# gpustack/llama-box

Measured on AMD Instinct MI355X. Metric: decode tokens/sec (batch-1) + prefill tok/s, Llama-3-8B Q4_K_M, higher is better.
Workload: dtype q4_K/q6_K weights x q8_K activations (int8 dot, f32 accumulate)

## Files before the change

### include/ggml_mi355x.h

```cpp
#ifndef GGML_MI355X_H
#define GGML_MI355X_H
#include "ggml_abi.h"

#ifdef __cplusplus
extern "C" {
#endif

#define GGML_MI355X_NAME "MI355X"
#define GGML_MI355X_MAX_DEVICES 16

ggml_backend_reg_t ggml_backend_init(void);

int ggml_backend_score(void);

ggml_backend_reg_t ggml_backend_mi355x_reg(void);


typedef void (*ggml_backend_mi355x_split_rows_t)(int64_t nrows, const float * tensor_split, int n_dev, int64_t * row0);

typedef int (*ggml_backend_mi355x_tp_init_t)(ggml_backend_t backend, int rank, int world_size, const void * unique_id, size_t unique_id_size);
typedef int (*ggml_backend_mi355x_tp_p2p_export_t)(ggml_backend_t backend, int rank, int world_size, void * handle_out, size_t handle_size);
typedef int (*ggml_backend_mi355x_tp_p2p_attach_t)(ggml_backend_t backend, const void * handles, size_t handles_size);
typedef int (*ggml_backend_mi355x_tp_all_reduce_t)(ggml_backend_t backend, float * device_ptr, size_t n);
typedef int (*ggml_backend_mi355x_tp_get_unique_id_t)(void * unique_id_out, size_t unique_id_size);
typedef ggml_backend_buffer_type_t (*ggml_backend_mi355x_tp_rowpar_buffer_type_t)(int device);

typedef int (*ggml_backend_mi355x_graph_key_probe_t)(const struct ggml_cgraph * a, const struct ggml_cgraph * b, int64_t * n_words);

typedef int64_t (*ggml_backend_mi355x_decode_copy_read_t)(ggml_backend_t backend, const struct ggml_tensor * t, void * out, size_t size);

typedef int (*ggml_backend_mi355x_set_option_t)(ggml_backend_t backend, const char * key, const char * value);
typedef int64_t (*ggml_backend_mi355x_get_stat_t)(ggml_backend_t backend, const char * key);
typedef int (*ggml_backend_mi355x_timing_report_t)(ggml_backend_t backend, char * buf, size_t size, int reset);

#ifdef __cplusplus
}
#endif
#endif
```

### llama_box_amd/csrc/backend.cpp

```cpp
#include <dlfcn.h>

#include <algorithm>
#include <chrono>
#include <mutex>
#include <thread>

#include "common.h"
#include "kernels.h"

namespace mi355x {

int log_level() {
    static int lvl = [] {
        const char * e = getenv("GGML_MI355X_LOG");
        return e ? atoi(e) : 0;
    }();
    return lvl;
}

struct device_ctx {
    int device = 0;
    std::string name, description;
    ggml_backend_buffer_type buft{};
    ggml_backend_buffer_type buft_rowpar{};
    ggml_backend_buffer_type buft_host{};
};

struct reg_ctx {
    std::vector<ggml_backend_device *> devices;
};

static ggml_backend_reg g_reg;
static reg_ctx g_reg_ctx;
static std::once_flag g_reg_once;
static ggml_guid g_guid = {0x4d, 0x49, 0x33, 0x35, 0x35, 0x58, 0x2d, 0x67, 0x67, 0x6d, 0x6c, 0x2d, 0x62, 0x6b, 0x6e, 0x64};

static device_ctx * dctx(ggml_backend_dev_t dev) { return (device_ctx *) dev->context; }
int logical_device_count() { return (int) g_reg_ctx.devices.size(); }
int logical_device_ordinal(int i) { return dctx(g_reg_ctx.devices[(size_t) i])->device; }
ggml_backend_dev_t logical_device(int i) { return g_reg_ctx.devices[(size_t) i]; }

typedef ggml_backend_buffer_t (*buffer_init_fn)(ggml_backend_buffer_type_t, struct ggml_backend_buffer_i, void *, size_t);

ggml_backend_buffer_t make_backend_buffer(ggml_backend_buffer_type_t buft, const ggml_backend_buffer_i & iface, void * context, size_t size);
static ggml_backend_buffer_t make_buffer(ggml_backend_buffer_type_t buft, const ggml_backend_buffer_i & iface, void * context, size_t size) {
    return make_backend_buffer(buft, iface, context, size);
}
ggml_backend_buffer_t make_backend_buffer(ggml_backend_buffer_type_t buft, const ggml_backend_buffer_i & iface, void * context, size_t size) {
    static buffer_init_fn host_fn = (buffer_init_fn) dlsym(RTLD_DEFAULT, "ggml_backend_buffer_init");
    if (host_fn) return host_fn(buft, iface, context, size);
    return new ggml_backend_buffer{iface, buft, context, size, GGML_BACKEND_BUFFER_USAGE_ANY};
}

static void uploader_drain(int device);
static std::atomic<uint64_t> g_decode_epoch{1};
uint64_t decode_copy_epoch() { return g_decode_epoch.load(std::memory_order_acquire); }
static void decode_copy_drop(buffer_ctx * c, size_t off, size_t n) {
    if (c->shadow == nullptr) return;
    std::lock_guard<std::mutex> lk(c->sh_mtx);
    if (c->sh_valid.empty()) return;
    bool any = false;
    for (auto it = c->sh_valid.begin(); it != c->sh_valid.end();) {
        if (it->first < off + n && off < it->first + it->second) { it = c->sh_valid.erase(it); any = true; }
        else ++it;
    }
    if (any) g_decode_epoch.fetch_add(1, std::memory_order_acq_rel);
}
static void decode_copy_drop(ggml_backend_buffer_t b, const ggml_tensor * t, size_t offset, size_t size) {
    buffer_ctx * c = (buffer_ctx *) b->context;
    if (c->shadow != nullptr && t->data != nullptr) decode_copy_drop(c, (size_t) ((const char *) t->data - (const char *) c->base) + offset, size);
}
static const uint8_t * second_copy(backend_ctx * c, const ggml_tensor * w, const bool q80_panels) {
    if (!c->opt.decode_copy || w == nullptr || w->view_src != nullptr || w->data == nullptr || w->ne[2] != 1 || w->ne[3] != 1) return nullptr;
    ggml_backend_buffer_t b = w->buffer;
    if (b == nullptr || !buffer_is_ours(b) || b->usage != GGML_BACKEND_BUFFER_USAGE_WEIGHTS || buffer_is_split(b) || buffer_is_rowpar(b)) return nullptr;
    if (q80_panels ? !repack_q80_supported(w->type, w->ne[0], w->ne[1], (int64_t) w->nb[1]) : !repack_supported(w->type, w->ne[0], (int64_t) w->nb[1])) return nullptr;
    buffer_ctx * bc = (buffer_ctx *) b->context;
    if (bc->device != c->device || bc->shadow_failed) return nullptr;
    const size_t off = (size_t) ((const char *) w->data - (const char *) bc->base), bytes = (size_t) w->nb[1] * (size_t) w->ne[1];
    if (off + bytes > bc->size) return nullptr;
    std::lock_guard<std::mutex> lk(bc->sh_mtx);
    auto it = bc->sh_valid.find(off);
    if (it != bc->sh_valid.end() && it->second == bytes) return (const uint8_t *) bc->shadow + off;
    if (c->capturing) return nullptr;
    if (bc->shadow == nullptr) {
        size_t free_b = 0, total_b = 0;
        if (hipMemGetInfo(&free_b, &total_b) != hipSuccess || free_b < bc->size + ((size_t) std::max(0, c->opt.decode_copy_headroom_gib) << 30) || hipMalloc(&bc->shadow, bc->size) != hipSuccess) {
            (void) hipGetLastError();
            bc->shadow = nullptr;
            bc->shadow_failed = true;
            MI_INFO("decode copy: no room for a second copy of a %.1f GiB weights buffer on device %d — the mat-vec kernels read the block layout", (double) bc->size / (1 << 30), bc->device);
            return nullptr;
        }
    }
    if (q80_panels) launch_repack_q80_panels(c->stream, w->data, (char *) bc->shadow + off, w->ne[0], w->ne[1], (int64_t) w->nb[1]);
    else launch_repack_planes(c->stream, w->type, w->data, (char *) bc->shadow + off, w->ne[0], (int64_t) w->nb[1], 0, w->ne[1]);
    if (hipStreamSynchronize(c->stream) != hipSuccess) { (void) hipGetLastError(); return nullptr; }
    bc->sh_valid[off] = bytes;
    c->st.decode_copy_tensors++;
    c->st.decode_copy_bytes += (int64_t) bytes;
    return (const uint8_t *) bc->shadow + off;
}
const uint8_t * decode_copy(backend_ctx * c, const ggml_tensor * w) { return second_copy(c, w, false); }
const uint8_t * q80_panel_copy(backend_ctx * c, const ggml_tensor * w) { return second_copy(c, w, true); }
static void buf_free(ggml_backend_buffer_t b) {
    buffer_ctx * c = (buffer_ctx *) b->context;
    if (ip_any()) ip_host_buffer_freed(b);
    HIP_SOFT(hipSetDevice(c->device));
    uploader_drain(c->device);
    if (c->shadow) {
        HIP_SOFT(hipDeviceSynchronize());
        HIP_NOTE(hipFree(c->shadow));
        g_decode_epoch.fetch_add(1, std::memory_order_acq_rel);
    }
    HIP_NOTE(hipFree(c->base));
    delete c;
}
static void * buf_get_base(ggml_backend_buffer_t b) { return ((buffer_ctx *) b->context)->base; }
static enum ggml_status buf_init_tensor(ggml_backend_buffer_t, ggml_tensor *) { return GGML_STATUS_SUCCESS; }
static void buf_memset_tensor(ggml_backend_buffer_t b, ggml_tensor * t, uint8_t value, size_t offset, size_t size) {
    buffer_ctx * c = (buffer_ctx *) b->context;
    if (ip_any()) ip_host_access(b, true);
    HIP_SOFT(hipSetDevice(c->device));
    decode_copy_drop(b, t, offset, size);
    uploader_drain(c->device);
    HIP_SOFT(hipMemset((char *) t->data + offset, value, size));
    HIP_SOFT(hipDeviceSynchronize());
}
struct uploader {
    std::atomic<int> device{-1};
    std::atomic<bool> failed{false};
    hipStream_t stream = nullptr;
    static constexpr int NSLOT = 3;
    char * slot[NSLOT] = {nullptr, nullptr, nullptr};
    hipEvent_t ev[NSLOT] = {nullptr, nullptr, nullptr};
    bool busy[NSLOT] = {false, false, false};
    size_t slot_bytes = 0;
    int next = 0;
    hipEvent_t last = nullptr;
    std::atomic<bool> in_flight{false};
    int n_threads = 1;
    std::mutex mtx;
    uint64_t bytes = 0;
    double seconds = 0;
};
static uploader g_uploaders[GGML_MI355X_MAX_DEVICES];
static std::atomic<int> g_staged_upload{env_int("GGML_MI355X_STAGED_UPLOAD", 0)};

static void par_memcpy(char * dst, const char * src, size_t n, int n_threads) {
    if (n_threads <= 1 || n < ((size_t) 4 << 20)) { memcpy(dst, src, n); return; }
    std::vector<std::thread> th;
    const size_t per = ((n / (size_t) n_threads) + 4095) & ~(size_t) 4095;
    for (int t = 1; t < n_threads; ++t) {
        const size_t o = (size_t) t * per;
        if (o >= n) break;
        th.emplace_back([=] { memcpy(dst + o, src + o, std::min(per, n - o)); });
    }
    memcpy(dst, src, std::min(per, n));
    for (auto & x : th) x.join();
}
static uploader * uploader_for(int device) {
    if (device < 0 || device >= GGML_MI355X_MAX_DEVICES) return nullptr;
    uploader * u = &g_uploaders[device];
    if (u->failed) return nullptr;
    if (u->device == device) return u;
    if (!g_staged_upload.load(std::memory_order_relaxed)) return nullptr;
    std::lock_guard<std::mutex> init_lock(u->mtx);
    if (u->failed) return nullptr;
    if (u->device == device) return u;
    const char * e_mb = getenv("GGML_MI355X_UPLOAD_SLOT_MIB");
    const char * e_th = getenv("GGML_MI355X_UPLOAD_THREADS");
    u->slot_bytes = (size_t) std::max(1, e_mb ? atoi(e_mb) : 32) << 20;
    u->n_threads = std::max(1, std::min(16, e_th ? atoi(e_th) : 4));
    bool ok = hipStreamCreateWithFlags(&u->stream, hipStreamNonBlocking) == hipSuccess && hipEventCreateWithFlags(&u->last, hipEventDisableTiming) == hipSuccess;
    for (int i = 0; i < uploader::NSLOT && ok; ++i)
        ok = hipHostMalloc((void **) &u->slot[i], u->slot_bytes, hipHostMallocDefault) == hipSuccess && hipEventCreateWithFlags(&u->ev[i], hipEventDisableTiming) == hipSuccess;
    if (!ok) {
        (void) hipGetLastError();
        MI_INFO("staged uploads unavailable on device %d (pinned allocation failed): set_tensor falls back to hipMemcpy", device);
        for (int i = 0; i < uploader::NSLOT; ++i) {
            if (u->slot[i]) (void) hipHostFree(u->slot[i]);
            if (u->ev[i]) (void) hipEventDestroy(u->ev[i]);
            u->slot[i] = nullptr;
            u->ev[i] = nullptr;
        }
        if (u->last) (void) hipEventDestroy(u->last);
        if (u->stream) (void) hipStreamDestroy(u->stream);
        u->failed = true;
        return nullptr;
    }
    u->device = device;
    return u;
}
static void uploader_drain(int device) {
    if (device < 0 || device >= GGML_MI355X_MAX_DEVICES) return;
    uploader * u = &g_uploaders[device];
    if (u->device != device) return;
    std::lock_guard<std::mutex> lock(u->mtx);
    if (!u->in_flight) return;
    HIP_SOFT(hipStreamSynchronize(u->stream));
    for (bool & b : u->busy) b = false;
    u->in_flight = false;
}
static void uploader_join(int device, hipStream_t s) {
    if (device < 0 || device >= GGML_MI355X_MAX_DEVICES) return;
    uploader * u = &g_uploaders[device];
    if (u->device != device || !u->in_flight) return;
    std::lock_guard<std::mutex> lock(u->mtx);
    if (!u->in_flight) return;
    if (hipEventQuery(u->last) == hipSuccess) {
        for (bool & b : u->busy) b = false;
        u->in_flight = false;
        return;
    }
    (void) hipGetLastError();
    HIP_SOFT(hipStreamWaitEvent(s, u->last, 0));
}
static bool staged_upload(int device, char * dst, const char * src, size_t size) {
    uploader * u = uploader_for(device);
    if (!u) return false;
    std::lock_guard<std::mutex> lock(u->mtx);
    const auto t0 = std::chrono::steady_clock::now();
    for (size_t o = 0; o < size; o += u->slot_bytes) {
        const size_t n = std::min(u->slot_bytes, size - o);
        const int k = u->next;
        u->next = (k + 1) % uploader::NSLOT;
        if (u->busy[k] && hipEventSynchronize(u->ev[k]) != hipSuccess) return false;
        par_memcpy(u->slot[k], src + o, n, u->n_threads);
        if (hipMemcpyAsync(dst + o, u->slot[k], n, hipMemcpyHostToDevice, u->stream) != hipSuccess || hipEventRecord(u->ev[k], u->stream) != hipSuccess) {
            (void) hipGetLastError();
            (void) hipStreamSynchronize(u->stream);
            u->failed = true;
            return false;
        }
        u->busy[k] = true;
        u->in_flight = true;
    }
    if (hipEventRecord(u->last, u->stream) != hipSuccess) { (void) hipGetLastError(); (void) hipStreamSynchronize(u->stream); }
    u->bytes += size;
    u->seconds += std::chrono::duration<double>(std::chrono::steady_clock::now() - t0).count();
    return true;
}

static std::atomic<int> g_hip_failed{0};
void note_hip_failure() { g_hip_failed.store(1, std::memory_order_relaxed); }
bool hip_failed() { return g_hip_failed.load(std::memory_order_relaxed) != 0; }
void clear_hip_failure() { g_hip_failed.store(0, std::memory_order_relaxed); }

namespace {
struct mask_entry { const void * dev = nullptr; mask_stats st; uint64_t stamp = 0; };
std::mutex g_mask_mtx;
mask_entry g_masks[8];
std::atomic<uint64_t> g_mask_clock{0};
}
void note_mask_upload(const ggml_tensor * t, const void * host, size_t offset, size_t size) {
    auto forget = [&]() {
        std::lock_guard<std::mutex> lock(g_mask_mtx);
        for (mask_entry & e : g_masks)
            if (e.dev == t->data) { e.dev = nullptr; e.stamp = 0; }
    };
    bool named = false;
    for (const char * p = t->name; *p && !named; ++p) named = (p[0] == 'm' || p[0] == 'M') && (p[1] == 'a' || p[1] == 'A') && (p[2] == 's' || p[2] == 'S') && (p[3] == 'k' || p[3] == 'K');
    const bool whole = offset == 0 && t->ne[2] == 1 && t->ne[3] == 1 && (t->type == GGML_TYPE_F16 || t->type == GGML_TYPE_F32) && t->nb[1] > 0 && size % (size_t) t->nb[1] == 0 &&
                       size <= (size_t) t->nb[1] * (size_t) t->ne[1] && t->nb[0] == (t->type == GGML_TYPE_F16 ? 2u : 4u);
    if (!named || !whole || t->ne[1] < 2 || t->ne[1] > 256 || size > ((size_t) 16 << 20)) { forget(); return; }
    const int64_t n = t->ne[0], rows = (int64_t) (size / (size_t) t->nb[1]);
    if (rows < 2) { forget(); return; }
    mask_stats st;
    int64_t total = 0;
    const int64_t dense_at = rows * n / 4 + 1;
    for (int64_t r = 0; r < rows; ++r) {
        if (total >= dense_at) {
            st.rows = (int) rows;
            st.max_visible = std::max(st.max_visible, (int) n);
            total = rows * n;
            break;
        }
        int64_t vis = 0;
        if (t->type == GGML_TYPE_F16) {
            const uint16_t * m = (const uint16_t *) ((const char *) host + r * t->nb[1]);
            for (int64_t i = 0; i < n; ++i) vis += m[i] != 0xFC00u;
        } else {
            const uint32_t * m = (const uint32_t *) ((const char *) host + r * t->nb[1]);
            for (int64_t i = 0; i < n; ++i) vis += m[i] != 0xFF800000u;
        }
        total += vis;
        st.rows += vis > 0;
        st.max_visible = std::max(st.max_visible, (int) vis);
    }
    st.density = st.rows > 0 ? (float) ((double) total / ((double) st.rows * (double) n)) : 0.0f;
    std::lock_guard<std::mutex> lock(g_mask_mtx);
    mask_entry * slot = &g_masks[0];
    for (mask_entry & e : g_masks) {
        if (e.dev == t->data) { slot = &e; break; }
        if (e.stamp < slot->stamp) slot = &e;
    }
    slot->dev = t->data;
    slot->st = st;
    slot->stamp = ++g_mask_clock;
}
void forget_mask_stats(const void * dev_ptr, size_t nbytes) {
    if (g_mask_clock.load(std::memory_order_relaxed) == 0 || !dev_ptr) return;
    std::lock_guard<std::mutex> lock(g_mask_mtx);
    for (mask_entry & e : g_masks)
        if (e.stamp != 0 && (const char *) e.dev >= (const char *) dev_ptr && (const char *) e.dev < (const char *) dev_ptr + nbytes) { e.dev = nullptr; e.stamp = 0; }
}
void copy_mask_stats(const ggml_tensor * src, const ggml_tensor * dst, size_t nbytes) {
    if (g_mask_clock.load(std::memory_order_relaxed) == 0 || !src->data || !dst->data) return;
    std::lock_guard<std::mutex> lock(g_mask_mtx);
    const mask_entry * from = nullptr;
    for (const mask_entry & e : g_masks)
        if (e.stamp != 0 && e.dev == src->data) from = &e;
    for (mask_entry & e : g_masks)
        if (e.stamp != 0 && (const char *) e.dev >= (const char *) dst->data && (const char *) e.dev < (const char *) dst->data + nbytes) { e.dev = nullptr; e.stamp = 0; }
    if (!from || src->view_src || dst->view_src || src->type != dst->type || src->ne[0] != dst->ne[0] || src->ne[1] != dst->ne[1] || src->ne[2] != dst->ne[2] || src->ne[3] != dst->ne[3] ||
        src->nb[1] != dst->nb[1])
        return;
    const mask_stats st = from->st;
    mask_entry * slot = &g_masks[0];
    for (mask_entry & e : g_masks) {
        if (e.dev == dst->data) { slot = &e; break; }
        if (e.stamp < slot->stamp) slot = &e;
    }
    if (slot == from) return;
    slot->dev = dst->data;
    slot->st = st;
    slot->stamp = ++g_mask_clock;
}
bool lookup_mask_stats(const void * dev_ptr, mask_stats * out) {
    std::lock_guard<std::mutex> lock(g_mask_mtx);
    for (const mask_entry & e : g_masks)
        if (e.dev == dev_ptr && e.stamp != 0) { *out = e.st; return true; }
    return false;
}
int mask_sparse_hint(const void * dev_ptr) {
    mask_stats st;
    return dev_ptr != nullptr && lookup_mask_stats(dev_ptr, &st) && st.rows > 0 && st.density <= 0.25f ? 1 : 0;
}

static void buf_set_tensor(ggml_backend_buffer_t b, ggml_tensor * t, const void * data, size_t offset, size_t size) {
    buffer_ctx * c = (buffer_ctx *) b->context;
    if (ip_any()) ip_host_access(b, true);
    HIP_SOFT(hipSetDevice(c->device));
    note_mask_upload(t, data, offset, size);
    decode_copy_drop(b, t, offset, size);
    if (size > ((size_t) 1 << 20) && staged_upload(c->device, (char *) t->data + offset, (const char *) data, size)) return;
    uploader_drain(c->device);
    HIP_SOFT(hipMemcpy((char *) t->data + offset, data, size, hipMemcpyHostToDevice));
}
static void buf_get_tensor(ggml_backend_buffer_t b, const ggml_tensor * t, void * data, size_t offset, size_t size) {
    buffer_ctx * c = (buffer_ctx *) b->context;
    if (ip_any()) ip_host_access(b, false);
    HIP_SOFT(hipSetDevice(c->device));
    uploader_drain(c->device);
    HIP_SOFT(hipMemcpy(data, (const char *) t->data + offset, size, hipMemcpyDeviceToHost));
}
static bool buf_cpy_tensor(ggml_backend_buffer_t b, const ggml_tensor * src, ggml_tensor * dst) {
    ggml_backend_buffer_t sb = src->view_src ? src->view_src->buffer : src->buffer;
    if (!buffer_is_ours(sb)) return false;
    buffer_ctx * sc = (buffer_ctx *) sb->context;
    buffer_ctx * dc = (buffer_ctx *) b->context;
    const size_t n = ggml_abi_nbytes(src);
    copy_mask_stats(src, dst, n);
    decode_copy_drop(b, dst, 0, n);
    if (ip_any()) { ip_host_access(sb, false); ip_host_access(b, true); }
    uploader_drain(sc->device);
    if (dc->device != sc->device) uploader_drain(dc->device);
    if (sc->device == dc->device) {
        HIP_SOFT(hipSetDevice(dc->device));
        HIP_SOFT(hipMemcpy(dst->data, src->data, n, hipMemcpyDeviceToDevice));
    } else {
        HIP_SOFT(hipMemcpyPeer(dst->data, dc->device, src->data, sc->device, n));
    }
    HIP_SOFT(hipDeviceSynchronize());
    return true;
}
static void buf_clear(ggml_backend_buffer_t b, uint8_t value) {
    buffer_ctx * c = (buffer_ctx *) b->context;
    if (ip_any()) ip_host_access(b, true);
    HIP_SOFT(hipSetDevice(c->device));
    decode_copy_drop(c, 0, c->size);
    uploader_drain(c->device);
    HIP_SOFT(hipMemset(c->base, value, c->size));
    HIP_SOFT(hipDeviceSynchronize());
}
static const ggml_backend_buffer_i k_buffer_iface = {buf_free, buf_get_base, buf_init_tensor, buf_memset_tensor, buf_set_tensor,
                                                     buf_get_tensor, buf_cpy_tensor, buf_clear, nullptr};

bool buffer_is_ours(ggml_backend_buffer_t b) { return b != nullptr && b->iface.free_buffer == buf_free; }
void make_internal_buffer(ggml_backend_buffer * out, buffer_ctx * bc, int device_ordinal, bool rowpar) {
    bc->device = device_ordinal;
    bc->base = nullptr;
    bc->size = 0;
    bc->rowpar = rowpar;
    *out = ggml_backend_buffer{k_buffer_iface, nullptr, bc, 0, GGML_BACKEND_BUFFER_USAGE_COMPUTE};
}
bool buffer_is_rowpar(ggml_backend_buffer_t b) { return buffer_is_ours(b) && ((buffer_ctx *) b->context)->rowpar; }

struct buft_ctx {
    int device;
    bool rowpar;
    std::string name;
};
static const char * buft_get_name(ggml_backend_buffer_type_t buft) { return ((buft_ctx *) buft->context)->name.c_str(); }
static ggml_backend_buffer_t buft_alloc(ggml_backend_buffer_type_t buft, size_t size) {
    buft_ctx * bc = (buft_ctx *) buft->context;
    HIP_SOFT(hipSetDevice(bc->device));
    void * p = nullptr;
    hipError_t err = hipMalloc(&p, size + 256);
    if (err != hipSuccess) {
        (void) hipGetLastError();
        MI_ERR("allocating %.2f MiB on device %d: hipMalloc failed: %s", size / 1024.0 / 1024.0, bc->device, hipGetErrorString(err));
        return nullptr;
    }
    buffer_ctx * c = new buffer_ctx{bc->device, p, size, bc->rowpar};
    return make_buffer(buft, k_buffer_iface, c, size);
}
static size_t buft_alignment(ggml_backend_buffer_type_t) { return 256; }
static size_t buft_max_size(ggml_backend_buffer_type_t buft) {
    buft_ctx * bc = (buft_ctx *) buft->context;
    hipDeviceProp_t prop{};
    if (hipGetDeviceProperties(&prop, bc->device) != hipSuccess) {
        (void) hipGetLastError();
        return SIZE_MAX;
    }
    return prop.totalGlobalMem;
}
static size_t buft_alloc_size(ggml_backend_buffer_type_t, const ggml_tensor * t) {
    return (ggml_abi_nbytes(t) + 15) / 16 * 16;
}
static bool buft_is_host(ggml_backend_buffer_type_t) { return false; }
static const ggml_backend_buffer_type_i k_buft_iface = {buft_get_name, buft_alloc, buft_alignment, buft_max_size, buft_alloc_size, buft_is_host};

static std::mutex g_pinned_mtx;
static std::vector<std::pair<const char *, size_t>> g_pinned;
static bool is_pinned_range(const void * p, size_t n) {
    std::lock_guard<std::mutex> lock(g_pinned_mtx);
    for (const auto & r : g_pinned)
        if ((const char *) p >= r.first && (const char *) p + n <= r.first + r.second) return true;
    return false;
}
static void hbuf_free(ggml_backend_buffer_t b) {
    {
        std::lock_guard<std::mutex> lock(g_pinned_mtx);
        for (size_t i = 0; i < g_pinned.size(); ++i)
            if (g_pinned[i].first == (const char *) b->context) { g_pinned.erase(g_pinned.begin() + (long) i); break; }
    }
    HIP_NOTE(hipHostFree(b->context));
}
static void * hbuf_base(ggml_backend_buffer_t b) { return b->context; }
static void hbuf_memset(ggml_backend_buffer_t, ggml_tensor * t, uint8_t v, size_t off, size_t sz) { memset((char *) t->data + off, v, sz); }
static void hbuf_set(ggml_backend_buffer_t, ggml_tensor * t, const void * d, size_t off, size_t sz) { memcpy((char *) t->data + off, d, sz); }
static void hbuf_get(ggml_backend_buffer_t, const ggml_tensor * t, void * d, size_t off, size_t sz) { memcpy(d, (const char *) t->data + off, sz); }
static void hbuf_clear(ggml_backend_buffer_t b, uint8_t v) { memset(b->context, v, b->size); }
static const char * hbuft_name(ggml_backend_buffer_type_t) { return GGML_MI355X_NAME "_Host"; }
static ggml_backend_buffer_t hbuft_alloc(ggml_backend_buffer_type_t buft, size_t size) {
    void * p = nullptr;
    hipError_t err = hipHostMalloc(&p, size > 0 ? size : 1, hipHostMallocPortable | hipHostMallocMapped);
    if (err != hipSuccess) {
        (void) hipGetLastError();
        return nullptr;
    }
    ggml_backend_buffer_i iface = {hbuf_free, hbuf_base, nullptr, hbuf_memset, hbuf_set, hbuf_get, nullptr, hbuf_clear, nullptr};
    {
        std::lock_guard<std::mutex> lock(g_pinned_mtx);
        g_pinned.emplace_back((const char *) p, size > 0 ? size : 1);
    }
    return make_buffer(buft, iface, p, size);
}
static size_t hbuft_alignment(ggml_backend_buffer_type_t) { return 64; }
static bool hbuft_is_host(ggml_backend_buffer_type_t) { return true; }

static const char * be_get_name(ggml_backend_t be) { return ((backend_ctx *) be->context)->name.c_str(); }
static void be_free(ggml_backend_t be) {
    backend_ctx * c = (backend_ctx *) be->context;
    HIP_SOFT(hipSetDevice(c->device));
    HIP_SOFT(hipStreamSynchronize(c->stream));
    free_graph_cache(c);
    ip_free(c);
    tp_free(c);
    free_split_helpers(c);
    if (c->ws) HIP_NOTE(hipFree(c->ws));
    if (c->up_ring) HIP_NOTE(hipHostFree(c->up_ring));
    if (c->fa_lists) HIP_NOTE(hipFree(c->fa_lists));
    if (c->rope_tab) HIP_NOTE(hipFree(c->rope_tab));
    if (c->act_tab) HIP_NOTE(hipFree(c->act_tab));
    if (c->fa_arrive) HIP_NOTE(hipFree(c->fa_arrive));
    if (c->ss_buf) HIP_NOTE(hipFree(c->ss_buf));
    HIP_SOFT(hipStreamDestroy(c->stream));
    delete c;
    delete be;
}
void flush_uploads(backend_ctx * c) {
    if (c->up_pending.n == 0) return;
    launch_upload_multi(c->stream, c->up_pending);
    c->up_pending.n = 0;
}
static void be_set_tensor_async(ggml_backend_t be, ggml_tensor * t, const void * data, size_t offset, size_t size) {
    backend_ctx * c = (backend_ctx *) be->context;
    if (ip_any()) ip_host_access(t->view_src ? t->view_src->buffer : t->buffer, true);
    HIP_SOFT(hipSetDevice(c->device));
    note_mask_upload(t, data, offset, size);
    {
        ggml_backend_buffer_t tb = t->view_src ? t->view_src->buffer : t->buffer;
        if (tb && buffer_is_ours(tb) && ((buffer_ctx *) tb->context)->shadow) decode_copy_drop(tb, t, offset, size);
    }
    constexpr size_t SMALL = 64 * 1024, RING = 4u << 20;
    if (size > 0 && size <= SMALL && c->opt.small_uploads) {
        if (!c->up_ring) {
            if (hipHostMalloc((void **) &c->up_ring, RING, hipHostMallocDefault) == hipSuccess) c->up_cap = RING;
            else { (void) hipGetLastError(); c->up_ring = nullptr; c->opt.small_uploads = false; }
        }
        if (c->up_ring) {
            size_t at = (c->up_head + 255) & ~(size_t) 255;
            if (at + size > c->up_cap) {
                flush_uploads(c);
                HIP_SOFT(hipStreamSynchronize(c->stream));
                at = 0;
            }
            memcpy(c->up_ring + at, data, size);
            c->up_head = at + size;
            if (c->up_pending.n == 8) flush_uploads(c);
            c->up_pending.seg[c->up_pending.n++] = {(char *) t->data + offset, c->up_ring + at, size};
            return;
        }
    }
    flush_uploads(c);
    uploader_join(c->device, c->stream);
    HIP_SOFT(hipMemcpyAsync((char *) t->data + offset, data, size, hipMemcpyHostToDevice, c->stream));
}
static void be_get_tensor_async(ggml_backend_t be, const ggml_tensor * t, void * data, size_t offset, size_t size) {
    backend_ctx * c = (backend_ctx *) be->context;
    if (ip_any()) ip_host_access(t->view_src ? t->view_src->buffer : t->buffer, false);
    HIP_SOFT(hipSetDevice(c->device));
    flush_uploads(c);
    uploader_join(c->device, c->stream);
    if (c->opt.small_downloads && size > 0 && size <= ((size_t) 8 << 20) && is_pinned_range(data, size)) {
        launch_upload_small(c->stream, data, (const char *) t->data + offset, size);
        c->st.kernel_downloads++;
        return;
    }
    HIP_SOFT(hipMemcpyAsync(data, (const char *) t->data + offset, size, hipMemcpyDeviceToHost, c->stream));
}
static bool be_is_ours(ggml_backend_t be);
static bool be_cpy_tensor_async(ggml_backend_t be_src, ggml_backend_t be_dst, const ggml_tensor * src, ggml_tensor * dst) {
    if (!be_is_ours(be_src) || !be_is_ours(be_dst)) return false;
    ggml_backend_buffer_t sb = src->view_src ? src->view_src->buffer : src->buffer;
    ggml_backend_buffer_t db = dst->view_src ? dst->view_src->buffer : dst->buffer;
    if (!buffer_is_ours(sb) || !buffer_is_ours(db)) return false;
    backend_ctx * cs = (backend_ctx *) be_src->context;
    backend_ctx * cd = (backend_ctx *) be_dst->context;
    flush_uploads(cs);
    if (cd != cs) flush_uploads(cd);
    const size_t n = ggml_abi_nbytes(src);
    copy_mask_stats(src, dst, n);
    if (((buffer_ctx *) db->context)->shadow) decode_copy_drop(db, dst, 0, n);
    if (ip_any()) { ip_host_access(sb, false); ip_host_access(db, true); }
    uploader_join(cs->device, cs->stream);
    if (cd->device != cs->device) uploader_drain(cd->device);
    if (cs->device == cd->device) {
        HIP_SOFT(hipSetDevice(cs->device));
        HIP_SOFT(hipMemcpyAsync(dst->data, src->data, n, hipMemcpyDeviceToDevice, cs->stream));
    } else {
        HIP_SOFT(hipSetDevice(cs->device));
        HIP_SOFT(hipMemcpyPeerAsync(dst->data, cd->device, src->data, cs->device, n, cs->stream));
    }
    if (be_src != be_dst) {
        hipEvent_t ev;
        HIP_NOTE(hipEventCreateWithFlags(&ev, hipEventDisableTiming));
        HIP_SOFT(hipEventRecord(ev, cs->stream));
        HIP_SOFT(hipSetDevice(cd->device));
        HIP_SOFT(hipStreamWaitEvent(cd->stream, ev, 0));
        HIP_NOTE(hipEventDestroy(ev));
    }
    return true;
}
static void be_synchronize(ggml_backend_t be) {
    backend_ctx * c = (backend_ctx *) be->context;
    HIP_SOFT(hipSetDevice(c->device));
    flush_uploads(c);
    uploader_drain(c->device);
    HIP_SOFT(hipStreamSynchronize(c->stream));
}
static enum ggml_status be_graph_compute(ggml_backend_t be, ggml_cgraph * g) {
    backend_ctx * c = (backend_ctx *) be->context;
    if (hipSetDevice(c->device) != hipSuccess) return GGML_STATUS_FAILED;
    flush_uploads(c);
    uploader_join(c->device, c->stream);
    return graph_compute(c, g);
}
static void be_event_record(ggml_backend_t be, ggml_backend_event_t ev) {
    backend_ctx * c = (backend_ctx *) be->context;
    flush_uploads(c);
    HIP_SOFT(hipEventRecord((hipEvent_t) ev->context, c->stream));
}
static void be_event_wait(ggml_backend_t be, ggml_backend_event_t ev) {
    backend_ctx * c = (backend_ctx *) be->context;
    flush_uploads(c);
    HIP_SOFT(hipStreamWaitEvent(c->stream, (hipEvent_t) ev->context, 0));
}
static const ggml_backend_i k_backend_iface = {
    be_get_name, be_free, be_set_tensor_async, be_get_tensor_async, be_cpy_tensor_async, be_synchronize,
     nullptr,  nullptr,  nullptr,  nullptr,
    be_graph_compute, be_event_record, be_event_wait,
#if GGML_ABI_HAS_GRAPH_OPTIMIZE
    nullptr,
#endif
};
static bool be_is_ours(ggml_backend_t be) { return be != nullptr && be->iface.get_name == be_get_name; }
static ggml_backend_t dev_init_backend(ggml_backend_dev_t dev, const char *);
ggml_backend_t internal_backend(int logical) {
    if (logical < 0 || logical >= logical_device_count()) return nullptr;
    return dev_init_backend(logical_device(logical), nullptr);
}

static const char * dev_get_name(ggml_backend_dev_t dev) { return dctx(dev)->name.c_str(); }
static const char * dev_get_description(ggml_backend_dev_t dev) { return dctx(dev)->description.c_str(); }
static void dev_get_memory(ggml_backend_dev_t dev, size_t * free, size_t * total) {
    *free = 0;
    *total = 0;
    HIP_NOTE(hipSetDevice(dctx(dev)->device));
    HIP_NOTE(hipMemGetInfo(free, total));
}
static enum ggml_backend_dev_type dev_get_type(ggml_backend_dev_t) { return GGML_BACKEND_DEVICE_TYPE_GPU; }
static void dev_get_props(ggml_backend_dev_t dev, ggml_backend_dev_props * props) {
    props->name = dev_get_name(dev);
    props->description = dev_get_description(dev);
    props->type = GGML_BACKEND_DEVICE_TYPE_GPU;
    dev_get_memory(dev, &props->memory_free, &props->memory_total);
    props->caps = { true,  true,  false,  true};
}
static ggml_backend_t dev_init_backend(ggml_backend_dev_t dev, const char *) {
    device_ctx * d = dctx(dev);
    if (hipSetDevice(d->device) != hipSuccess) { (void) hipGetLastError(); MI_ERR("init_backend: device %d cannot be made current", d->device); return nullptr; }
    backend_ctx * c = new backend_ctx();
    c->device = d->device;
    c->name = d->name;
    if (hipStreamCreateWithFlags(&c->stream, hipStreamNonBlocking) != hipSuccess) {
        (void) hipGetLastError();
        MI_ERR("init_backend: no stream on device %d", d->device);
        delete c;
        return nullptr;
    }
    {
        static const bool preload = env_flag("GGML_MI355X_PRELOAD", true);
        static std::mutex pre_mtx;
        static bool preloaded[64] = {false};
        std::lock_guard<std::mutex> lk(pre_mtx);
        if (preload && d->device >= 0 && d->device < 64 && !preloaded[d->device]) {
            preload_kernel_files(c->stream);
            if (hipStreamSynchronize(c->stream) != hipSuccess) { (void) hipGetLastError(); MI_ERR("init_backend: kernel preload failed on device %d", d->device); }
            preloaded[d->device] = true;
        }
    }
    c->fa_lists_bytes = (size_t) 8 << 20;
    if (hipMalloc((void **) &c->fa_lists, c->fa_lists_bytes) != hipSuccess) { (void) hipGetLastError(); c->fa_lists = nullptr; c->fa_lists_bytes = 0; }
    if (hipMalloc((void **) &c->rope_tab, backend_ctx::rope_tab_floats * sizeof(float)) != hipSuccess) { (void) hipGetLastError(); c->rope_tab = nullptr; }
    if (hipMalloc((void **) &c->fa_arrive, backend_ctx::fa_arrive_slots * sizeof(unsigned)) != hipSuccess || hipMemset(c->fa_arrive, 0, backend_ctx::fa_arrive_slots * sizeof(unsigned)) != hipSuccess) {
        (void) hipGetLastError();
        c->fa_arrive = nullptr;
    }
    options_from_env(c->opt);
    c->ssm_fuse = env_flag("GGML_MI355X_SSM_FUSE", true);
    if (hipMalloc((void **) &c->ss_buf, 256 * sizeof(double)) != hipSuccess) {
        (void) hipGetLastError();
        c->ss_buf = nullptr;
    }
    return new ggml_backend{&g_guid, k_backend_iface, dev, c};
}
static ggml_backend_buffer_type_t dev_get_buffer_type(ggml_backend_dev_t dev) { return &dctx(dev)->buft; }
static ggml_backend_buffer_type_t dev_get_host_buffer_type(ggml_backend_dev_t dev) { return &dctx(dev)->buft_host; }
static bool dev_supports_op(ggml_backend_dev_t, const ggml_tensor * op) { return supports_op(op); }
static bool dev_supports_buft(ggml_backend_dev_t dev, ggml_backend_buffer_type_t buft) {
    if (buft_is_split(buft)) return logical_device(split_buft_main_device(buft)) == dev;
    if (buft->iface.get_name != buft_get_name) return false;
    return ((buft_ctx *) buft->context)->device == dctx(dev)->device;
}
static bool dev_offload_op(ggml_backend_dev_t, const ggml_tensor * op) {
    const int64_t batch = op->op == GGML_OP_MUL_MAT ? op->ne[1] : 0;
    return batch >= 32;
}
static ggml_backend_event_t dev_event_new(ggml_backend_dev_t dev) {
    HIP_SOFT(hipSetDevice(dctx(dev)->device));
    hipEvent_t ev;
    if (hipEventCreateWithFlags(&ev, hipEventDisableTiming) != hipSuccess) {
        (void) hipGetLastError();
        return nullptr;
    }
    return new ggml_backend_event{dev, ev};
}
static void dev_event_free(ggml_backend_dev_t, ggml_backend_event_t ev) {
    HIP_NOTE(hipEventDestroy((hipEvent_t) ev->context));
    delete ev;
}
static void dev_event_synchronize(ggml_backend_dev_t, ggml_backend_event_t ev) { HIP_SOFT(hipEventSynchronize((hipEvent_t) ev->context)); }
static const ggml_backend_device_i k_device_iface = {
    dev_get_name, dev_get_description, dev_get_memory, dev_get_type, dev_get_props, dev_init_backend, dev_get_buffer_type,
    dev_get_host_buffer_type,  nullptr, dev_supports_op, dev_supports_buft, dev_offload_op,
    dev_event_new, dev_event_free, dev_event_synchronize,
};

static ggml_backend_feature g_features[] = {{"ARCH", "gfx950"}, {"WAVE", "64"}, {"GRAPHS", "1"}, {"RCCL_TP", "1"}, {nullptr, nullptr}};
static ggml_backend_feature * get_features(ggml_backend_reg_t) { return g_features; }

static int api_tp_init(ggml_backend_t be, int rank, int world, const void * uid, size_t n) {
    if (!be_is_ours(be)) return -1;
    return tp_init((backend_ctx *) be->context, rank, world, uid, n);
}
static int api_tp_get_unique_id(void * out, size_t n) { return tp_get_unique_id(out, n); }
static int api_tp_p2p_export(ggml_backend_t be, int rank, int world, void * handle_out, size_t n) {
    if (!be_is_ours(be)) return -1;
    return tp_p2p_export((backend_ctx *) be->context, rank, world, handle_out, n);
}
static int api_tp_all_reduce(ggml_backend_t be, float * device_ptr, size_t n) {
    if (!be_is_ours(be)) return -1;
    backend_ctx * c = (backend_ctx *) be->context;
    if (!tp_active(c)) return -2;
    HIP_TRY(hipSetDevice(c->device), -3);
    return tp_all_reduce(c, device_ptr, n) ? 0 : -4;
}
static int api_tp_p2p_attach(ggml_backend_t be, const void * handles, size_t n) {
    if (!be_is_ours(be)) return -1;
    return tp_p2p_attach((backend_ctx *) be->context, handles, n);
}
static ggml_backend_buffer_type_t api_split_buffer_type(int main_device, const float * tensor_split) { return split_buffer_type(main_device, tensor_split); }
static void api_split_rows(int64_t nrows, const float * tensor_split, int n_dev, int64_t * row0) { split_rows(nrows, tensor_split, n_dev, nrows % 256 == 0 ? 256 : 64, row0); }
static ggml_backend_buffer_type_t api_tp_rowpar_buft(int device) {
    if (device < 0 || device >= (int) g_reg_ctx.devices.size()) return nullptr;
    return &dctx(g_reg_ctx.devices[device])->buft_rowpar;
}
static int api_graph_key_probe(const ggml_cgraph * a, const ggml_cgraph * b, int64_t * n_words) {
    std::vector<uint64_t> key;
    graph_key_build(a, key);
    if (n_words) *n_words = (int64_t) key.size();
    return graph_key_equals(b, key) ? 1 : 0;
}
static int64_t api_decode_copy_read(ggml_backend_t be, const ggml_tensor * t, void * out, size_t size) {
    if (!be_is_ours(be) || t == nullptr) return -1;
    backend_ctx * c = (backend_ctx *) be->context;
    if (hipSetDevice(c->device) != hipSuccess) return -1;
    uploader_join(c->device, c->stream);
    const uint8_t * p = t->type == GGML_TYPE_Q8_0 ? q80_panel_copy(c, t) : decode_copy(c, t);
    if (!p) return 0;
    const size_t bytes = (size_t) t->nb[1] * (size_t) t->ne[1];
    if (out == nullptr || size < bytes) return (int64_t) bytes;
    if (hipStreamSynchronize(c->stream) != hipSuccess || hipMemcpy(out, p, bytes, hipMemcpyDeviceToHost) != hipSuccess) { (void) hipGetLastError(); return -1; }
    return (int64_t) bytes;
}
static int api_set_option(ggml_backend_t be, const char * key, const char * value) {
    if (!be_is_ours(be)) return -1;
    backend_ctx * c = (backend_ctx *) be->context;
    const std::string k = key;
    const int v = atoi(value);
    if (!options_set(c->opt, key, v)) {
        if (k == "tp_p2p") { if (!tp_p2p_enable(c, v != 0)) return -2; }
        else if (k == "tp_p2p_reset") { if (!tp_p2p_reset(c)) return -2; }
        else if (k == "clear_failure") { if (v) clear_hip_failure(); }
        else if (k == "staged_upload") g_staged_upload.store(v != 0);
        else if (k == "ssm_fuse") c->ssm_fuse = v != 0;
        else return -1;
    }
    HIP_SOFT(hipStreamSynchronize(c->stream));
    free_graph_cache(c);
    return 0;
}
static int64_t api_get_stat(ggml_backend_t be, const char * key) {
    if (!be_is_ours(be)) return -1;
    backend_ctx * c = (backend_ctx *) be->context;
    const std::string k = key;
    if (const int64_t * p = stats_find(c->st, key)) return *p;
    if (k == "graph_cache_size") return (int64_t) c->graphs.size();
    if (k == "p2p_timeouts") return tp_p2p_timeouts(c);
    if (k.rfind("ip_", 0) == 0) return ip_stat(c, key);
    if (k == "staged_upload_bytes") return (int64_t) g_uploaders[c->device].bytes;
    if (k == "staged_upload_us") return (int64_t) (g_uploaders[c->device].seconds * 1e6);
    return -1;
}
static int api_timing_report(ggml_backend_t be, char * buf, size_t size, int reset) {
    if (!be_is_ours(be) || !buf || size == 0) return -1;
    backend_ctx * c = (backend_ctx *) be->context;
    HIP_SOFT(hipStreamSynchronize(c->stream));
    for (auto & pe : c->pending_events) {
        float ms = 0;
        HIP_NOTE(hipEventElapsedTime(&ms, pe.second.first, pe.second.second));
        c->timing[pe.first].total_ms += ms;
        c->timing[pe.first].count += 1;
        HIP_NOTE(hipEventDestroy(pe.second.first));
        HIP_NOTE(hipEventDestroy(pe.second.second));
    }
    c->pending_events.clear();
    std::string out;
    for (auto & kv : c->timing) {
        if (kv.first.rfind("bytes:", 0) == 0) continue;
        auto itb = c->timing.find("bytes:" + kv.first);
        char line[256];
        snprintf(line, sizeof(line), "%s %lld %.6f %.0f\n", kv.first.c_str(), (long long) kv.second.count, kv.second.total_ms,
                 itb == c->timing.end() ? 0.0 : itb->second.total_ms);
        out += line;
    }
    snprintf(buf, size, "%s", out.c_str());
    if (reset) c->timing.clear();
    return 0;
}

static const char * reg_get_name(ggml_backend_reg_t) { return GGML_MI355X_NAME; }
static size_t reg_get_device_count(ggml_backend_reg_t) { return g_reg_ctx.devices.size(); }
static ggml_backend_dev_t reg_get_device(ggml_backend_reg_t, size_t i) { return i < g_reg_ctx.devices.size() ? g_reg_ctx.devices[i] : nullptr; }
static void * reg_get_proc_address(ggml_backend_reg_t, const char * name) {
    const std::string n = name;
    if (n == "ggml_backend_get_features") return (void *) get_features;
    if (n == "ggml_backend_mi355x_tp_init") return (void *) api_tp_init;
    if (n == "ggml_backend_mi355x_tp_get_unique_id") return (void *) api_tp_get_unique_id;
    if (n == "ggml_backend_mi355x_tp_p2p_export") return (void *) api_tp_p2p_export;
    if (n == "ggml_backend_mi355x_tp_p2p_attach") return (void *) api_tp_p2p_attach;
    if (n == "ggml_backend_mi355x_tp_all_reduce") return (void *) api_tp_all_reduce;
    if (n == "ggml_backend_mi355x_tp_rowpar_buffer_type") return (void *) api_tp_rowpar_buft;
    if (n == "ggml_backend_mi355x_set_option") return (void *) api_set_option;
    if (n == "ggml_backend_mi355x_decode_copy_read") return (void *) api_decode_copy_read;
    if (n == "ggml_backend_mi355x_get_stat") return (void *) api_get_stat;
    if (n == "ggml_backend_mi355x_timing_report") return (void *) api_timing_report;
    if (n == "ggml_backend_split_buffer_type") return (void *) api_split_buffer_type;
    if (n == "ggml_backend_mi355x_split_rows") return (void *) api_split_rows;
    if (n == "ggml_backend_mi355x_graph_key_probe") return (void *) api_graph_key_probe;
    return nullptr;
}
static const ggml_backend_reg_i k_reg_iface = {reg_get_name, reg_get_device_count, reg_get_device, reg_get_proc_address};

static int count_gfx950() {
    int n = 0;
    if (hipGetDeviceCount(&n) != hipSuccess) {
        (void) hipGetLastError();
        return 0;
    }
    int ok = 0;
    for (int i = 0; i < n; ++i) {
        hipDeviceProp_t prop;
        if (hipGetDeviceProperties(&prop, i) == hipSuccess && strncmp(prop.gcnArchName, "gfx950", 6) == 0) ok++;
    }
    return ok;
}

static void init_reg() {
    int n = 0;
    if (hipGetDeviceCount(&n) != hipSuccess) {
        (void) hipGetLastError();
        n = 0;
    }
    const int fake = std::max(1, env_int("GGML_MI355X_FAKE_DEVICES", 1));
    for (int ii = 0; ii < n * fake && (int) g_reg_ctx.devices.size() < GGML_MI355X_MAX_DEVICES; ++ii) {
        const int i = ii / fake;
        hipDeviceProp_t prop;
        if (hipGetDeviceProperties(&prop, i) != hipSuccess) continue;
        if (strncmp(prop.gcnArchName, "gfx950", 6) != 0) {
            MI_INFO("skipping HIP device %d (%s): not gfx950", i, prop.gcnArchName);
            continue;
        }
        device_ctx * d = new device_ctx();
        d->device = i;
        d->name = std::string(GGML_MI355X_NAME) + std::to_string(g_reg_ctx.devices.size());
        d->description = prop.name;
        ggml_backend_device * dev = new ggml_backend_device{k_device_iface, &g_reg, d};
        d->buft = {k_buft_iface, dev, new buft_ctx{i, false, d->name}};
        d->buft_rowpar = {k_buft_iface, dev, new buft_ctx{i, true, d->name + "_RowPar"}};
        d->buft_host = {{hbuft_name, hbuft_alloc, hbuft_alignment, nullptr, nullptr, hbuft_is_host}, dev, nullptr};
        g_reg_ctx.devices.push_back(dev);
    }
    g_reg = {GGML_BACKEND_API_VERSION, k_reg_iface, &g_reg_ctx};
}

static bool op_numbering_matches_host() {
    typedef const char * (*op_name_fn)(int);
    op_name_fn host_name = (op_name_fn) dlsym(RTLD_DEFAULT, "ggml_op_name");
    if (!host_name) {
        MI_INFO("ggml_op_name is not resolvable in this process: operator numbering of include/ggml_abi.h not verified against the host");
        return true;
    }
    static const struct { int op; const char * name; } k_expect[] = {
        {GGML_OP_NONE, "NONE"}, {GGML_OP_DUP, "DUP"}, {GGML_OP_ADD, "ADD"}, {GGML_OP_SUB, "SUB"}, {GGML_OP_MUL, "MUL"}, {GGML_OP_DIV, "DIV"},
        {GGML_OP_ARGMAX, "ARGMAX"}, {GGML_OP_NORM, "NORM"}, {GGML_OP_RMS_NORM, "RMS_NORM"}, {GGML_OP_MUL_MAT, "MUL_MAT"}, {GGML_OP_MUL_MAT_ID, "MUL_MAT_ID"}, {GGML_OP_SCALE, "SCALE"},
        {GGML_OP_CPY, "CPY"}, {GGML_OP_CONT, "CONT"}, {GGML_OP_RESHAPE, "RESHAPE"}, {GGML_OP_VIEW, "VIEW"}, {GGML_OP_PERMUTE, "PERMUTE"},
        {GGML_OP_TRANSPOSE, "TRANSPOSE"}, {GGML_OP_GET_ROWS, "GET_ROWS"}, {GGML_OP_SET_ROWS, "SET_ROWS"}, {GGML_OP_SOFT_MAX, "SOFT_MAX"},
        {GGML_OP_ROPE, "ROPE"}, {GGML_OP_FLASH_ATTN_EXT, "FLASH_ATTN_EXT"}, {GGML_OP_UNARY, "UNARY"}, {GGML_OP_GLU, "GLU"},
    };
    bool ok = true;
    for (const auto & e : k_expect) {
        const char * got = host_name(e.op);
        if (!got || strcmp(got, e.name) != 0) {
            MI_ERR("operator numbering mismatch: this library was built with %s = %d, the host calls op %d \"%s\" — rebuild against the host's ggml.h (tools/abi_dump.c prints both tables)",
                   e.name, e.op, e.op, got ? got : "(null)");
            ok = false;
        }
    }
    return ok;
}

}

extern "C" {

__attribute__((visibility("default"))) ggml_backend_reg_t ggml_backend_mi355x_reg(void) {
    std::call_once(mi355x::g_reg_once, mi355x::init_reg);
    return &mi355x::g_reg;
}

__attribute__((visibility("default"))) ggml_backend_reg_t ggml_backend_init(void) {
    ggml_backend_reg_t reg = ggml_backend_mi355x_reg();
    if (mi355x::g_reg_ctx.devices.empty()) {
        MI_ERR("no gfx950 (MI355X) device visible: backend not registered");
        return nullptr;
    }
    static const bool ops_ok = mi355x::op_numbering_matches_host();
    if (!ops_ok) return nullptr;
    return reg;
}

__attribute__((visibility("default"))) int ggml_backend_score(void) { return mi355x::count_gfx950() > 0 ? 100 : 0; }
}
```

### llama_box_amd/csrc/common.h

```cpp
#pragma once
#include <hip/hip_runtime.h>
#include <hip/hip_ext.h>

#include <cstdint>
#include <cstdio>
#include <cstdlib>
#include <cstring>
#include <atomic>
#include <map>
#include <mutex>
#include <string>
#include <unordered_map>
#include <vector>

#include "../../include/ggml_mi355x.h"
#include "options.h"

#define MI_LOG(level, ...)                                    \
    do {                                                      \
        if ((level) <= mi355x::log_level()) {                 \
            fprintf(stderr, "ggml-mi355x: " __VA_ARGS__);     \
            fprintf(stderr, "\n");                            \
        }                                                     \
    } while (0)
#define MI_ERR(...) MI_LOG(0, __VA_ARGS__)
#define MI_INFO(...) MI_LOG(1, __VA_ARGS__)
#define MI_DBG(...) MI_LOG(2, __VA_ARGS__)

#define HIP_CHECK(expr)                                                                                         \
    do {                                                                                                        \
        hipError_t err_ = (expr);                                                                               \
        if (err_ != hipSuccess) {                                                                               \
            fprintf(stderr, "ggml-mi355x: HIP error %d (%s) at %s:%d: %s\n", (int) err_, hipGetErrorString(err_), __FILE__, __LINE__, #expr); \
            abort();                                                                                            \
        }                                                                                                       \
    } while (0)

#define HIP_SOFT(expr)                                                                                          \
    do {                                                                                                        \
        hipError_t err_ = (expr);                                                                               \
        if (err_ != hipSuccess) {                                                                               \
            (void) hipGetLastError();                                                                           \
            fprintf(stderr, "ggml-mi355x: HIP error %d (%s) at %s:%d: %s — graph_compute will report failure from here on\n", (int) err_, \
                    hipGetErrorString(err_), __FILE__, __LINE__, #expr);                                        \
            mi355x::note_hip_failure();                                                                         \
        }                                                                                                       \
    } while (0)

#define HIP_NOTE(expr)                                                                                          \
    do {                                                                                                        \
        hipError_t err_ = (expr);                                                                               \
        if (err_ != hipSuccess) {                                                                               \
            (void) hipGetLastError();                                                                           \
            fprintf(stderr, "ggml-mi355x: HIP error %d (%s) at %s:%d: %s (ignored: no tensor data involved)\n", (int) err_, hipGetErrorString(err_), __FILE__, __LINE__, #expr); \
        }                                                                                                       \
    } while (0)

#define HIP_TRY(expr, ret)                                                                                      \
    do {                                                                                                        \
        hipError_t err_ = (expr);                                                                               \
        if (err_ != hipSuccess) {                                                                               \
            (void) hipGetLastError();                                                                           \
            fprintf(stderr, "ggml-mi355x: HIP error %d (%s) at %s:%d: %s\n", (int) err_, hipGetErrorString(err_), __FILE__, __LINE__, #expr); \
            return ret;                                                                                         \
        }                                                                                                       \
    } while (0)

namespace mi355x {

int log_level();
void note_hip_failure();
bool hip_failed();
void clear_hip_failure();

struct upload_seg { char * dst; const char * src; size_t n; };
struct upload_batch { upload_seg seg[8]; int n; };

struct q8k_dev {
    int8_t qs[256];
    uint16_t bsums[16];
    int16_t bs32[8];
    float d;
    float pad[3];
};
static_assert(sizeof(q8k_dev) == 320, "q8k_dev");
struct q80_dev {
    int8_t qs[32];
    float d;
};
static_assert(sizeof(q80_dev) == 36, "q80_dev");
struct q81_dev {
    int8_t qs[32];
    float d;
    float s;
};
static_assert(sizeof(q81_dev) == 40, "q81_dev");

struct backend_ctx;

struct tp_state;
struct split_helper;
struct ip_engine;

struct cached_graph {
    hipGraph_t graph = nullptr;
    hipGraphExec_t exec = nullptr;
    int seen = 0;
    uint64_t last_use = 0;
    int64_t allreduces = 0;
    int n_nodes = 0;
    int fa_form = 0;
    bool early_failed = false;
    std::vector<uint64_t> key;
};

struct timing_slot {
    double total_ms = 0;
    int64_t count = 0;
};

struct backend_ctx {
    int device = 0;
    hipStream_t stream = nullptr;
    std::string name;
    options opt;
    stats st;
    void * ws = nullptr;
    size_t ws_size = 0;
    const void * q8_src = nullptr;
    int q8_kind = 0;
    size_t q8_bytes = 0;
    uint64_t q8_epoch = 0;
    std::unordered_map<uint64_t, cached_graph> graphs;
    cached_graph * last_graph = nullptr;
    std::vector<uint64_t> key_scratch;
    uint64_t tick = 0;
    uint64_t decode_epoch = 0;
    bool capturing = false;
    bool ssm_fuse = true;
    bool mm_q5_major = false;
    tp_state * tp = nullptr;
    ip_engine * ip = nullptr;
    std::vector<split_helper *> split_helpers;
    hipEvent_t split_ready = nullptr;
    char * up_ring = nullptr;
    size_t up_cap = 0, up_head = 0;
    upload_batch up_pending{};
    double * ss_buf = nullptr;
    unsigned * fa_arrive = nullptr;
    static constexpr int fa_arrive_slots = 16384;
    float * rope_tab = nullptr;
    static constexpr int rope_tab_floats = 4096 * 256;
    uint16_t * act_tab = nullptr;
    int * fa_lists = nullptr;
    size_t fa_lists_bytes = 0;
    std::map<std::string, timing_slot> timing;
    std::vector<std::pair<std::string, std::pair<hipEvent_t, hipEvent_t>>> pending_events;
};

inline bool ensure_dyn_lds(const void * kernel, size_t bytes, std::atomic<uint32_t> & done) {
    int dev = 0;
    if (hipGetDevice(&dev) != hipSuccess || dev < 0 || dev >= 32) dev = 0;
    const uint32_t bit = 1u << dev;
    if (done.load(std::memory_order_acquire) & bit) return true;
    if (hipFuncSetAttribute(kernel, hipFuncAttributeMaxDynamicSharedMemorySize, (int) bytes) != hipSuccess) {
        (void) hipGetLastError();
        MI_ERR("hipFuncSetAttribute(MaxDynamicSharedMemorySize = %zu) failed on device %d", bytes, dev);
        return false;
    }
    done.fetch_or(bit, std::memory_order_release);
    return true;
}

void flush_uploads(backend_ctx * c);

struct buffer_ctx {
    int device = 0;
    void * base = nullptr;
    size_t size = 0;
    bool rowpar = false;
    void * shadow = nullptr;
    bool shadow_failed = false;
    std::mutex sh_mtx;
    std::unordered_map<size_t, size_t> sh_valid;
};
const uint8_t * decode_copy(backend_ctx * c, const ggml_tensor * w);
const uint8_t * q80_panel_copy(backend_ctx * c, const ggml_tensor * w);
uint64_t decode_copy_epoch();
bool buffer_is_ours(ggml_backend_buffer_t b);
bool buffer_is_rowpar(ggml_backend_buffer_t b);
ggml_backend_buffer_t make_backend_buffer(ggml_backend_buffer_type_t buft, const ggml_backend_buffer_i & iface, void * context, size_t size);
int logical_device_count();
int logical_device_ordinal(int i);
ggml_backend_dev_t logical_device(int i);

struct split_tensor_info {
    int n_dev;
    int kind;
    int64_t row0[GGML_MI355X_MAX_DEVICES + 1];
    void * slice[GGML_MI355X_MAX_DEVICES];
    size_t row_bytes;
    size_t slice_row_bytes[GGML_MI355X_MAX_DEVICES];
};
void split_rows(int64_t nrows, const float * tensor_split, int n_dev, int64_t granule, int64_t * row0);
ggml_backend_buffer_type_t split_buffer_type(int main_device, const float * tensor_split);
bool buft_is_split(ggml_backend_buffer_type_t buft);
int split_buft_main_device(ggml_backend_buffer_type_t buft);
bool buffer_is_split(ggml_backend_buffer_t b);
const split_tensor_info * split_info(const ggml_tensor * t);
bool split_mul_mat_supported(const ggml_tensor * op);
bool run_split_mul_mat(backend_ctx * c, const ggml_tensor * w, const ggml_tensor * b, ggml_tensor * dst);
bool run_split_rowpar(backend_ctx * c, const ggml_tensor * w, const ggml_tensor * b, ggml_tensor * dst, const ggml_tensor * add);
bool split_ffn_applies(const ggml_tensor * wg, const ggml_tensor * wu, const ggml_tensor * wd);
bool run_split_ffn(backend_ctx * c, const ggml_tensor * wg, const ggml_tensor * wu, const ggml_tensor * wd, const ggml_tensor * x, ggml_tensor * dst, const ggml_tensor * add);
void free_split_helpers(backend_ctx * c);

bool supports_op(const ggml_tensor * op);
enum ggml_status graph_compute(backend_ctx * ctx, ggml_cgraph * g);
void free_graph_cache(backend_ctx * ctx);
bool graph_key_equals(const ggml_cgraph * g, const std::vector<uint64_t> & key);
void graph_key_build(const ggml_cgraph * g, std::vector<uint64_t> & key);

struct ip_engine;
enum ggml_status ip_graph_compute(backend_ctx * ctx, ggml_cgraph * g, bool * handled);
void ip_free(backend_ctx * ctx);
int64_t ip_stat(const backend_ctx * ctx, const char * key);
void ip_host_access(ggml_backend_buffer_t b, bool write);
void ip_host_buffer_freed(ggml_backend_buffer_t b);
bool ip_any();

struct buffer_ctx;
void make_internal_buffer(ggml_backend_buffer * out, buffer_ctx * bc, int device_ordinal, bool rowpar);
ggml_backend_t internal_backend(int logical_device);

struct mask_stats {
    int rows = 0;
    int max_visible = 0;
    float density = 1.0f;
};
void note_mask_upload(const ggml_tensor * t, const void * host, size_t offset, size_t size);
bool lookup_mask_stats(const void * dev_ptr, mask_stats * out);
void forget_mask_stats(const void * dev_ptr, size_t nbytes);
void copy_mask_stats(const ggml_tensor * src, const ggml_tensor * dst, size_t nbytes);
int mask_sparse_hint(const void * dev_ptr);

int tp_init(backend_ctx * ctx, int rank, int world, const void * uid, size_t uid_size);
int tp_get_unique_id(void * out, size_t size);
bool tp_active(const backend_ctx * ctx);
int tp_p2p_export(backend_ctx * ctx, int rank, int world, void * handle_out, size_t size);
int tp_p2p_attach(backend_ctx * ctx, const void * handles, size_t size);
int64_t tp_p2p_timeouts(backend_ctx * ctx);
int tp_attach_local(backend_ctx * const * ctxs, int n);
bool tp_p2p_enable(backend_ctx * ctx, bool on);
bool tp_p2p_reset(backend_ctx * ctx);
bool tp_check(backend_ctx * ctx);
bool tp_all_reduce(backend_ctx * ctx, float * ptr, size_t n);
bool tp_all_reduce_fused(backend_ctx * ctx, float * ptr, size_t n, const float * add, float * out, double * ss_out, int * ss_n);
void tp_free(backend_ctx * ctx);

}
```

### llama_box_amd/csrc/graph.cpp

```cpp
#include <algorithm>
#include <chrono>
#include <cmath>

#include "kernels.h"

namespace mi355x {

static bool is_kq23_type(int t) { return t == GGML_TYPE_Q2_K || t == GGML_TYPE_Q3_K; }
static bool is_iq4xs_type(int t) { return t == GGML_TYPE_IQ4_XS; }
struct wtype_info {
    int type;
    const char * tag;
    int act;
    int align;
    bool prologue;
};
static const wtype_info k_wtypes[] = {
    {GGML_TYPE_Q4_K, "q4_K", GGML_TYPE_Q8_K, 0, true},
    {GGML_TYPE_Q5_K, "q5_K", GGML_TYPE_Q8_K, 0, true},
    {GGML_TYPE_Q6_K, "q6_K", GGML_TYPE_Q8_K, 0, true},
    {GGML_TYPE_Q8_0, "q8_0", GGML_TYPE_Q8_0, 0, true},
    {GGML_TYPE_Q4_0, "q4_0", GGML_TYPE_Q8_0, 2, false},
    {GGML_TYPE_Q4_1, "q4_1", GGML_TYPE_Q8_1, 4, false},
    {GGML_TYPE_Q5_0, "q5_0", GGML_TYPE_Q8_0, 2, false},
// ... 2019 lines not shown
                    }
                    return 1;
                }
            }
            timed_scope ts(c, "get_rows", (double) ggml_abi_nbytes(n));
            launch_get_rows(s, TD(a), TD(b), TD(n));
            c->st.kernel_launches++;
            return 1;
        }
        case GGML_OP_SET_ROWS: {
            timed_scope ts(c, "set_rows", (double) ggml_abi_nbytes(a));
            if (n->type == GGML_TYPE_Q8_0) launch_set_rows_q8_0(s, TD(a), TD(b), TD(n));
            else if (kv_store_type(n->type)) {
                int j = i + 1;
                while (j < g->n_nodes && (st.done[j] || is_view_op(g->nodes[j]))) ++j;
                const ggml_tensor * n2 = j < g->n_nodes ? g->nodes[j] : nullptr;
                if (fuse && n2 && n2->op == GGML_OP_SET_ROWS && kv_store_type(n2->type) && n2->src[0]->type == GGML_TYPE_F32 && n2->src[1]->type == GGML_TYPE_I64 &&
                    n2->src[0] != n && !ranges_overlap(n2->src[0], n) && !ranges_overlap(n2, n) && supports_op(n2)) {
                    launch_set_rows_kv_pair(s, TD(a), TD(b), TD(n), TD(n2->src[0]), TD(n2->src[1]), TD(n2));
                    mark_done(st, j);
                    c->st.fused_nodes++;
                } else {
                    launch_set_rows_kv(s, TD(a), TD(b), TD(n));
                }
            }
            else launch_set_rows(s, TD(a), TD(b), TD(n));
            c->st.kernel_launches++;
            return 1;
        }
        case GGML_OP_SOFT_MAX: {
            const tdesc md = b ? TD(b) : TD(a);
            if (fuse && c->opt.softmax_mm && n->ne[1] == 1 && !n->src[2] && ggml_abi_op_param_f32(n, 1) == 0.0f && a->type == GGML_TYPE_F32 && ggml_abi_is_contiguous(a) &&
                single_use(st, n)) {
                int j = -1;
                for (int k = i + 1; k < std::min(g->n_nodes, i + 8) && j < 0; ++k) {
                    if (st.done[k]) continue;
                    const ggml_tensor * t = g->nodes[k];
                    if (t->op == GGML_OP_MUL_MAT && t->src[1] == n) j = k;
                    else if (!is_view_op(t)) break;
                }
                if (j >= 0) {
                    const ggml_tensor * mm = g->nodes[j];
                    const ggml_tensor * v = mm->src[0];
                    if (v->type == GGML_TYPE_F16 && !buffer_is_split(v->buffer) && ggml_abi_is_contiguous(mm) && !ranges_overlap(mm, a) && !(b && ranges_overlap(mm, b))) {
                        int cont_at = -1;
                        const ggml_tensor * cont = nullptr;
                        static const bool elide_on = env_flag("GGML_MI355X_ELIDE_CONT", true);
                        if (elide_on && use_count(st, mm) == 1 && !(mm->flags & GGML_TENSOR_FLAG_OUTPUT)) {
                            const ggml_tensor * cur = mm;
                            for (int k = j + 1; k < std::min(g->n_nodes, j + 6); ++k) {
                                const ggml_tensor * t = g->nodes[k];
                                if (st.done[k]) continue;
                                if (is_view_op(t) && t->src[0] == cur && t->data == mm->data && use_count(st, t) == 1 && !(t->flags & GGML_TENSOR_FLAG_OUTPUT)) { cur = t; continue; }
                                if ((t->op == GGML_OP_CONT || t->op == GGML_OP_CPY || t->op == GGML_OP_DUP) && t->src[0] == cur && cur != mm && t->type == mm->type && ggml_abi_is_contiguous(cur) &&
                                    ggml_abi_is_contiguous(t) && ggml_abi_nelements(t) == ggml_abi_nelements(mm) && !ranges_overlap(t, a) && !ranges_overlap(t, v) && !(b && ranges_overlap(t, b)) &&
                                    !ranges_overlap(t, mm)) {
                                    cont = t;
                                    cont_at = k;
                                }
                                break;
                            }
                        }
                        tdesc out = TD(mm);
                        if (cont) out.data = (char *) cont->data;
                        timed_scope ts(c, "soft_max_mul_mat_f", (double) ggml_abi_nbytes(v) + (double) ggml_abi_nbytes(n));
                        if (launch_soft_max_mul_mat_f16(s, TD(v), TD(a), b ? &md : nullptr, out, ggml_abi_op_param_f32(n, 0))) {
                            mark_done(st, j);
                            if (cont) { mark_done(st, cont_at); c->st.fused_nodes++; c->st.elided_conts++; }
                            c->st.kernel_launches++;
                            c->st.fused_nodes++;
                            return 1;
                        }
                    }
                }
            }
            timed_scope ts(c, "soft_max", (double) ggml_abi_nbytes(n) * 2);
            launch_soft_max(s, TD(a), b ? &md : nullptr, n->src[2] ? (const float *) n->src[2]->data : nullptr, TD(n), ggml_abi_op_param_f32(n, 0), ggml_abi_op_param_f32(n, 1));
            c->st.kernel_launches++;
            return 1;
        }
        case GGML_OP_ROPE: {
            if (fuse && try_fuse_rope_store(st, i)) return 1;
            const rope_params p = rope_params_of(n, true);
            timed_scope ts(c, "rope", (double) ggml_abi_nbytes(n) * 2);
            launch_rope(s, TD(a), TD(b), n->src[2] ? (const float *) n->src[2]->data : nullptr, TD(n), p);
            c->st.kernel_launches++;
            return 1;
        }
        case GGML_OP_FLASH_ATTN_EXT: {
            const ggml_tensor * k = n->src[1];
            const ggml_tensor * v = n->src[2];
            const ggml_tensor * m = n->src[3];
            fattn_params p;
            p.scale = ggml_abi_op_param_f32(n, 0);
            p.max_bias = ggml_abi_op_param_f32(n, 1);
            p.logit_softcap = ggml_abi_op_param_f32(n, 2);
            const tdesc qd = TD(a);
            tdesc kd = TD(k), vd = TD(v);
            bool imaged = fa_route(n) == 3;
            bool native_kv = false;
            if (imaged) {
                fattn_params probe{};
                probe.logit_softcap = ggml_abi_op_param_f32(n, 2);
                probe.max_bias = ggml_abi_op_param_f32(n, 1);
                probe.n_splits = 1;
                native_kv = fattn_native_kv_ok(qd, kd, vd, probe);
                if (native_kv) {
                    imaged = false;
                    c->st.kv_native_nodes++;
                }
            }
            if (imaged) {
                char * img = (char *) c->ws + st.aux_off + fa_image_offset(qd, kd, vd);
                timed_scope ts(c, "kv_image_f16", (double) (ggml_abi_nbytes(k) + ggml_abi_nbytes(v)));
                launch_kv_images_f16(s, kd, vd, img);
                c->st.kernel_launches++;
                c->st.kv_image_nodes++;
            }
            const tdesc md0 = m ? TD(m) : qd;
            p.mask_sparse = fa_mask_hint(n);
            p.n_splits = std::min(64, c->opt.fa_splits > 0 ? c->opt.fa_splits : fattn_pick_splits(qd, kd, m ? &md0 : nullptr, p.mask_sparse));
            p.kv_type = (imaged || native_kv) ? (int) GGML_TYPE_F16 : (int) k->type;
            p.dq = native_kv ? 1 : 0;
            if (c->opt.fa_self_merge && c->fa_arrive) {
                p.arrive = c->fa_arrive;
                p.arrive_slots = backend_ctx::fa_arrive_slots;
            }
            const tdesc md = m ? TD(m) : qd;
            timed_scope ts(c, "flash_attn", (double) (k->ne[1] * k->ne[2] * k->ne[0] * 2 * 2));
            if (c->fa_lists) {
                const int tile = fattn_list_tile(qd, kd, m ? &md : nullptr, p, c->fa_lists_bytes);
                if (tile > 0) {
                    if (st.fa_list_mask != m->data || st.fa_list_tile != tile) {
                        launch_fattn_tile_scan(s, md, (int) a->ne[1], (int) k->ne[1], tile, c->fa_lists);
                        c->st.kernel_launches++;
                        st.fa_list_mask = m->data;
                        st.fa_list_tile = tile;
                    }
                    p.lists = c->fa_lists;
                    c->st.fa_list_launches++;
                } else if (m && a->ne[1] >= fattn_mma_min_q() && a->ne[3] == 1 && m->ne[3] == 1 && m->type == GGML_TYPE_F16 && (m->nb[1] % 8) == 0 && !(((uintptr_t) m->data) & 7) &&
                           (k->ne[1] % 4) == 0 && fattn_vis_bytes(qd, kd) <= c->fa_lists_bytes && flash_attn_mma_applies(qd, kd, &md, n->src[4] ? (const float *) n->src[4]->data : nullptr, TD(n), p)) {
                    if (st.fa_list_mask != m->data || st.fa_list_tile != -1) {
                        launch_fattn_vis_scan(s, md, (int) a->ne[1], (int) k->ne[1], (uint8_t *) c->fa_lists);
                        c->st.kernel_launches++;
                        st.fa_list_mask = m->data;
                        st.fa_list_tile = -1;
                    }
                    p.tile_vis = (const uint8_t *) c->fa_lists;
                }
            }
            if (fuse && c->opt.fa_wo && !native_kv && c->opt.prologue && c->opt.fa_splits == 0 && a->ne[1] == 1 && a->ne[3] == 1 && !p.lists && !p.tile_vis && use_count(st, n) == 1 &&
                !(n->flags & GGML_TENSOR_FLAG_OUTPUT) && ggml_abi_is_contiguous(n) && (((uintptr_t) n->data) & 15) == 0) {
                const int S = fattn_fat_splits(qd, kd, m ? &md : nullptr, n->src[4] ? (const float *) n->src[4]->data : nullptr, p);
                int j = i + 1;
                const ggml_tensor * view = nullptr;
                while (j < g->n_nodes && (st.done[j] || is_view_op(g->nodes[j]))) {
                    if (!st.done[j] && g->nodes[j]->src[0] == (view ? view : n) && g->nodes[j]->data == n->data) view = g->nodes[j];
                    ++j;
                }
                const ggml_tensor * mm = j < g->n_nodes ? g->nodes[j] : nullptr;
                const ggml_tensor * w = mm ? mm->src[0] : nullptr;
                const bool kq = w && (w->type == GGML_TYPE_Q4_K || w->type == GGML_TYPE_Q5_K || w->type == GGML_TYPE_Q6_K || w->type == GGML_TYPE_Q8_0) && w->ne[2] == 1 && w->ne[3] == 1 &&
                                rows_contig(w) && (w->ne[0] % 256) == 0 && !buffer_is_split(w->buffer);
                if (S > 0 && view && mm && mm->op == GGML_OP_MUL_MAT && mm->src[1] == view && kq && w->ne[0] == n->ne[0] * n->ne[1] && ggml_abi_nelements(view) == w->ne[0] &&
                    use_count(st, view) == 1 && !(view->flags & GGML_TENSOR_FLAG_OUTPUT) && ggml_abi_is_contiguous(mm) && mm->type == GGML_TYPE_F32 &&
                    !(tp_active(c) && weight_is_rowpar(w))) {
                    p.n_splits = S;
                    p.fat = 1;
                    timed_scope ts(c, "flash_attn_fat", (double) (k->ne[1] * k->ne[2] * k->ne[0] * 2 * 2));
                    g_fa_form = 0;
                    launch_flash_attn(s, qd, kd, vd, m ? &md : nullptr, nullptr, TD(n), p, (char *) c->ws + st.aux_off);
                    c->st.fa_form = g_fa_form;
                    st.fa_wo.b = view;
                    st.fa_wo.fa = n;
                    st.fa_wo.part = (const float *) ((char *) c->ws + st.aux_off);
                    st.fa_wo.splits = S;
                    c->st.kernel_launches++;
                    c->st.fused_nodes++;
                    return 1;
                }
            }
            const ggml_tensor * q8_reader = nullptr;
            if (fuse && c->opt.prologue && a->ne[1] > 1 &&
                (a->ne[1] <= 128 || (p.n_splits >= 2 && fattn_combine_rows_applies((int) k->ne[0], a->ne[1], a->ne[2], a->ne[3], p.n_splits, n->src[4] ? (const float *) n->src[4]->data : nullptr))) &&
                use_count(st, n) == 1 && !(n->flags & GGML_TENSOR_FLAG_OUTPUT) && ggml_abi_is_contiguous(n)) {
                for (int k = i + 1; k < std::min(g->n_nodes, i + 4) && !q8_reader; ++k) {
                    const ggml_tensor * t = g->nodes[k];
                    if ((t->op == GGML_OP_RESHAPE || t->op == GGML_OP_VIEW) && t->src[0] == n && t->data == n->data && ggml_abi_is_contiguous(t) && t->ne[0] == n->ne[0] * n->ne[1] &&
                        t->ne[1] == n->ne[2] && quant_consumers_only(st, k, t) &&
                        fattn_q8_out_ok(qd, kd, m ? &md : nullptr, n->src[4] ? (const float *) n->src[4]->data : nullptr, TD(n), p))
                        q8_reader = t;
                }
            }
            if (q8_reader) p.q8_out = (char *) c->ws + st.act_off;
            g_fa_form = 0;
            launch_flash_attn(s, qd, kd, vd, m ? &md : nullptr, n->src[4] ? (const float *) n->src[4]->data : nullptr, TD(n), p, (char *) c->ws + st.aux_off);
            c->st.fa_form = g_fa_form;
            if (q8_reader) {
                mark_q8_cache(st, q8_reader);
                c->st.fused_nodes++;
            }
            c->st.kernel_launches += p.n_splits > 1 ? 2 : 1;
            return 1;
        }
        case GGML_OP_ARGMAX:
            launch_argmax(s, TD(a), TD(n));
            c->st.kernel_launches++;
            return 1;
        case GGML_OP_CONCAT: {
            timed_scope ts(c, "concat", (double) ggml_abi_nbytes(n) * 2);
            if (!launch_concat(s, TD(a), TD(b), TD(n), n->op_params[0])) return -1;
            c->st.kernel_launches++;
            return 1;
        }
        case GGML_OP_SSM_CONV: {
            const ssm_conv_act f = (fuse && c->ssm_fuse) ? find_ssm_conv_act(st, i) : ssm_conv_act{nullptr, n, 0};
            timed_scope ts(c, f.absorbed ? "ssm_conv_bias_silu" : "ssm_conv", (double) ggml_abi_nbytes(a) + (double) ggml_abi_nbytes(n));
            if (!launch_ssm_conv(s, TD(a), TD(b), TD(f.out), f.bias ? (const float *) f.bias->data : nullptr)) return -1;
            c->st.kernel_launches++;
            c->st.fused_nodes += f.absorbed;
            return 1 + f.absorbed;
        }
        case GGML_OP_SSM_SCAN: {
            timed_scope ts(c, "ssm_scan", (double) (ggml_abi_nelements(n) - ggml_abi_nelements(b)) * 8);
            if (!launch_ssm_scan(s, TD(a), TD(b), TD(n->src[2]), TD(n->src[3]), TD(n->src[4]), TD(n->src[5]), TD(n->src[6]), TD(n))) return -1;
            c->st.kernel_launches++;
            return 1;
        }
        default:
            MI_ERR("graph_compute: unsupported op %d (node %d '%s')", (int) n->op, i, n->name);
            return -1;
    }
}

static bool run_nodes(backend_ctx * c, ggml_cgraph * g, const ws_plan & wp) {
    exec_state st{};
    st.c = c;
    st.g = g;
    st.aux_off = wp.act_bytes;
    st.uses.reserve((size_t) g->n_nodes * 2);
    for (int i = 0; i < g->n_nodes; ++i)
        for (int s = 0; s < GGML_MAX_SRC; ++s)
            if (g->nodes[i]->src[s]) st.uses[g->nodes[i]->src[s]]++;
    c->q8_src = nullptr;
    st.done.assign((size_t) g->n_nodes, 0);
    for (int i = 0; i < g->n_nodes;) {
        ggml_tensor * n = g->nodes[i];
        if (ggml_abi_nelements(n) == 0 || st.done[i]) { i++; continue; }
        st.ooo.clear();
        const int used = run_node(st, i);
        if (used < 0) return false;
        for (int k = 0; k < used; ++k)
            if (!is_view_op(g->nodes[i + k]) && g->nodes[i + k]->data) forget_mask_stats(g->nodes[i + k]->data, ggml_abi_nbytes(g->nodes[i + k]));
        if (!st.q8_fresh && c->q8_src) {
            const char * q0 = (const char *) c->q8_src, * q1 = q0 + c->q8_bytes;
            auto hits = [&](const ggml_tensor * t) {
                if (is_view_op(t) || !t->data) return false;
                const char * t0 = (const char *) t->data;
                return t0 < q1 && q0 < t0 + ggml_abi_nbytes(t);
            };
            bool hit = false;
            for (int k = 0; k < used && !hit; ++k) hit = hits(g->nodes[i + k]);
            for (size_t k = 0; k < st.ooo.size() && !hit; ++k) hit = hits(g->nodes[st.ooo[k]]);
            if (hit) c->q8_src = nullptr;
        }
        st.q8_fresh = false;
        i += used;
    }
    return hipGetLastError() == hipSuccess;
}

static_assert(offsetof(ggml_tensor, ne) == offsetof(ggml_tensor, buffer) + 8 && offsetof(ggml_tensor, nb) == offsetof(ggml_tensor, ne) + 32 &&
              offsetof(ggml_tensor, op) == offsetof(ggml_tensor, nb) + 32 && offsetof(ggml_tensor, op_params) == offsetof(ggml_tensor, op) + 4 &&
              offsetof(ggml_tensor, flags) == offsetof(ggml_tensor, op_params) + 64 && offsetof(ggml_tensor, src) == offsetof(ggml_tensor, flags) + 4 &&
              offsetof(ggml_tensor, buffer) % 8 == 0 && offsetof(ggml_tensor, src) % 8 == 0,
              "graph key: {buffer, ne, nb, op, op_params, flags} must be one padding-free run of ggml_tensor");
static constexpr size_t KEY_NODE_RUN = (offsetof(ggml_tensor, src) - offsetof(ggml_tensor, buffer)) / 8;
static constexpr size_t KEY_SRC_RUN = (offsetof(ggml_tensor, op) - offsetof(ggml_tensor, buffer)) / 8;

template <class Put>
static inline bool walk_key(const ggml_cgraph * g, Put && put) {
    uint64_t w[2];
    w[0] = (uint64_t) (uint32_t) g->n_nodes;
    if (!put(w, 1)) return false;
    for (int i = 0; i < g->n_nodes; ++i) {
        const ggml_tensor * n = g->nodes[i];
        uint32_t present = 0;
        for (int s = 0; s < GGML_MAX_SRC; ++s) present |= n->src[s] ? 1u << s : 0u;
        const bool hinted = n->op == GGML_OP_FLASH_ATTN_EXT || n->op == GGML_OP_SOFT_MAX;
        w[0] = (uint64_t) (uint32_t) n->type | (uint64_t) present << 32 | (uint64_t) (hinted ? fa_mask_hint(n) : 0) << 48;
        w[1] = (uint64_t) (uintptr_t) n->data;
        if (!put(w, 2) || !put(&n->buffer, KEY_NODE_RUN)) return false;
        for (int s = 0; s < GGML_MAX_SRC; ++s) {
            const ggml_tensor * t = n->src[s];
            if (!t) continue;
            w[0] = (uint64_t) (uint32_t) t->type;
            w[1] = (uint64_t) (uintptr_t) t->data;
            if (!put(w, 2) || !put(&t->buffer, KEY_SRC_RUN)) return false;
        }
    }
    return true;
}
static bool key_equals(const ggml_cgraph * g, const std::vector<uint64_t> & key) {
    const uint64_t * at = key.data(), * const end = at + key.size();
    const bool same = walk_key(g, [&](const void * p, size_t n) {
        if ((size_t) (end - at) < n || memcmp(at, p, n * 8) != 0) return false;
        at += n;
        return true;
    });
    return same && at == end;
}
static void key_build(const ggml_cgraph * g, std::vector<uint64_t> & key) {
    key.clear();
    key.reserve((size_t) g->n_nodes * 48);
    walk_key(g, [&](const void * p, size_t n) {
        const size_t at = key.size();
        key.resize(at + n);
        memcpy(key.data() + at, p, n * 8);
        return true;
    });
}
bool graph_key_equals(const ggml_cgraph * g, const std::vector<uint64_t> & key) { return key_equals(g, key); }
void graph_key_build(const ggml_cgraph * g, std::vector<uint64_t> & key) { key_build(g, key); }
static uint64_t key_hash(const std::vector<uint64_t> & key) {
    uint64_t h[4] = {0x9E3779B97F4A7C15ull, 0xC2B2AE3D27D4EB4Full, 0x165667B19E3779F9ull, 0x27D4EB2F165667C5ull};
    auto fold = [](uint64_t a, uint64_t v) {
        const unsigned __int128 m = (unsigned __int128) (a ^ v) * 0xD6E8FEB86659FD93ull;
        return (uint64_t) m ^ (uint64_t) (m >> 64);
    };
    size_t i = 0;
    for (; i + 4 <= key.size(); i += 4)
        for (int l = 0; l < 4; ++l) h[l] = fold(h[l], key[i + l]);
    for (; i < key.size(); ++i) h[0] = fold(h[0], key[i]);
    return fold(fold(fold(h[0], h[1]), h[2]), h[3] ^ key.size());
}

void free_graph_cache(backend_ctx * c) {
    for (auto & kv : c->graphs) {
        if (kv.second.exec) (void) hipGraphExecDestroy(kv.second.exec);
        if (kv.second.graph) (void) hipGraphDestroy(kv.second.graph);
    }
    c->graphs.clear();
    c->last_graph = nullptr;
}

enum ggml_status graph_compute(backend_ctx * c, ggml_cgraph * g) {
    if (g->n_nodes == 0) return GGML_STATUS_SUCCESS;
    if (hip_failed()) {
        MI_ERR("graph_compute: refused — an earlier HIP call of the data path failed (see the log above)");
        return GGML_STATUS_FAILED;
    }
    if (!tp_check(c)) return GGML_STATUS_FAILED;
    const auto t_enter = std::chrono::steady_clock::now();
    struct host_clock {
        backend_ctx * c;
        std::chrono::steady_clock::time_point t0;
        ~host_clock() { c->st.graph_compute_host_ns += std::chrono::duration_cast<std::chrono::nanoseconds>(std::chrono::steady_clock::now() - t0).count(); }
    } clock{c, t_enter};
    c->tick++;
    c->st.fa_form = 0;
    {
        const uint64_t ep = decode_copy_epoch();
        if (ep != c->decode_epoch) {
            if (!c->graphs.empty()) {
                (void) hipStreamSynchronize(c->stream);
                free_graph_cache(c);
            }
            c->decode_epoch = ep;
        }
    }
    auto replay = [&](cached_graph & cg) {
        cg.last_use = c->tick;
        cg.seen++;
        const auto t0 = std::chrono::steady_clock::now();
        c->st.graph_key_host_ns += std::chrono::duration_cast<std::chrono::nanoseconds>(t0 - t_enter).count();
        if (hipGraphLaunch(cg.exec, c->stream) != hipSuccess) {
            (void) hipGetLastError();
            return GGML_STATUS_FAILED;
        }
        c->st.graph_launch_host_ns += std::chrono::duration_cast<std::chrono::nanoseconds>(std::chrono::steady_clock::now() - t0).count();
        c->st.graph_launches++;
        c->st.allreduces += cg.allreduces;
        c->st.fa_form = cg.fa_form;
        return GGML_STATUS_SUCCESS;
    };
    const bool may_replay = c->opt.graphs && !c->opt.timing && g->n_nodes >= 8;
    if (may_replay && c->last_graph && c->last_graph->exec && key_equals(g, c->last_graph->key)) {
        c->st.graph_key_fast_hits++;
        return replay(*c->last_graph);
    }
    {
        bool handled = false;
        const enum ggml_status st_ip = ip_graph_compute(c, g, &handled);
        if (handled) return st_ip;
    }
    const ws_plan wp = plan_ws(c, g);
    if (!ensure_ws(c, wp.act_bytes + wp.aux_bytes + 256)) return GGML_STATUS_ALLOC_FAILED;
    if (!ensure_act_tables(c, g)) return GGML_STATUS_ALLOC_FAILED;
    bool has_split = false;
    for (int i = 0; i < g->n_nodes && !has_split; ++i) has_split = g->nodes[i]->op == GGML_OP_MUL_MAT && buffer_is_split(g->nodes[i]->src[0]->buffer);
    static const bool split_graphs = env_flag("GGML_MI355X_SPLIT_GRAPHS", false);
    const bool want_graph = may_replay && (!has_split || split_graphs);
    if (!want_graph) {
        c->st.eager_graphs++;
        return run_nodes(c, g, wp) ? GGML_STATUS_SUCCESS : GGML_STATUS_FAILED;
    }
    key_build(g, c->key_scratch);
    uint64_t fp = key_hash(c->key_scratch);
    auto it = c->graphs.find(fp);
    while (it != c->graphs.end() && it->second.key != c->key_scratch) {
        c->st.graph_key_collisions++;
        fp = fp * 0x9E3779B97F4A7C15ull + 1;
        it = c->graphs.find(fp);
    }
    if (it == c->graphs.end()) {
        if (c->graphs.size() > 64) {
            for (auto jt = c->graphs.begin(); jt != c->graphs.end();) {
                if (jt->second.last_use + 256 < c->tick) {
                    if (jt->second.exec) (void) hipGraphExecDestroy(jt->second.exec);
                    if (jt->second.graph) (void) hipGraphDestroy(jt->second.graph);
                    if (c->last_graph == &jt->second) c->last_graph = nullptr;
                    jt = c->graphs.erase(jt);
                    c->st.graph_evictions++;
                } else {
                    ++jt;
                }
            }
        }
        it = c->graphs.emplace(fp, cached_graph()).first;
        it->second.key = c->key_scratch;
        it->second.last_use = c->tick;
    }
    cached_graph & cg = it->second;
    static const bool early_on = env_flag("GGML_MI355X_EARLY_CAPTURE", true);
    const bool early = early_on && cg.seen == 0 && !cg.early_failed && c->last_graph && c->last_graph != &cg && c->last_graph->exec && c->last_graph->n_nodes == g->n_nodes &&
                       c->last_graph->last_use + 1 == c->tick && !has_split && !tp_active(c);
    cached_graph * const prev = early ? c->last_graph : nullptr;
    cg.n_nodes = g->n_nodes;
    c->last_graph = &cg;
    if (cg.exec) return replay(cg);
    cg.last_use = c->tick;
    cg.seen++;
    if (!early && (cg.seen < 2 || cg.seen > 1000000)) {
        c->st.eager_graphs++;
        return run_nodes(c, g, wp) ? GGML_STATUS_SUCCESS : GGML_STATUS_FAILED;
    }
    const bool shadow = early && c->opt.shadow_capture != 0;
    auto now_ns = [] { return std::chrono::duration_cast<std::chrono::nanoseconds>(std::chrono::steady_clock::now().time_since_epoch()).count(); };
    int64_t t_mark = now_ns();
    if (shadow && !run_nodes(c, g, wp)) return GGML_STATUS_FAILED;
    if (shadow) c->st.graph_shadow_eager_ns += now_ns() - t_mark;
    const stats st_step = c->st;
    struct shadow_stats {
        backend_ctx * c; const stats & keep; bool on;
        ~shadow_stats() {
            if (!on) return;
            stats s = keep;
            s.graph_captures = c->st.graph_captures; s.graph_early_captures = c->st.graph_early_captures; s.graph_shadow_captures = c->st.graph_shadow_captures;
            s.graph_exec_updates = c->st.graph_exec_updates; s.graph_exec_update_failures = c->st.graph_exec_update_failures; s.graph_evictions = c->st.graph_evictions;
            s.graph_capture_walk_ns = c->st.graph_capture_walk_ns; s.graph_exec_update_ns = c->st.graph_exec_update_ns;
            c->st = s;
        }
    } shadow_guard{c, st_step, shadow};
    t_mark = now_ns();
    if (hipStreamBeginCapture(c->stream, hipStreamCaptureModeRelaxed) != hipSuccess) {
        (void) hipGetLastError();
        if (shadow) { cg.early_failed = true; return GGML_STATUS_SUCCESS; }
        c->st.eager_graphs++;
        return run_nodes(c, g, wp) ? GGML_STATUS_SUCCESS : GGML_STATUS_FAILED;
    }
    c->capturing = true;
    const int64_t red0 = c->st.allreduces;
    const bool ok = run_nodes(c, g, wp);
    c->capturing = false;
    cg.fa_form = (int) c->st.fa_form;
    const int64_t red_captured = c->st.allreduces - red0;
    hipGraph_t graph = nullptr;
    const hipError_t e_end = hipStreamEndCapture(c->stream, &graph);
    c->st.graph_capture_walk_ns += now_ns() - t_mark;
    t_mark = now_ns();
    if (!ok || e_end != hipSuccess || graph == nullptr) {
        (void) hipGetLastError();
        if (graph) (void) hipGraphDestroy(graph);
        if (shadow) { cg.early_failed = true; return GGML_STATUS_SUCCESS; }
        if (early) {
            cg.early_failed = true;
            c->st.eager_graphs++;
            return run_nodes(c, g, wp) ? GGML_STATUS_SUCCESS : GGML_STATUS_FAILED;
        }
        MI_INFO("hipGraph capture failed (ok=%d, err=%d); running this topology eagerly from now on", (int) ok, (int) e_end);
        cg.seen = 1000001;
        c->st.eager_graphs++;
        return run_nodes(c, g, wp) ? GGML_STATUS_SUCCESS : GGML_STATUS_FAILED;
    }
    hipGraphExec_t exec = nullptr;
    if (early && c->opt.exec_update && prev && prev->exec) {
        hipGraphNode_t err_node = nullptr;
        hipGraphExecUpdateResult res = hipGraphExecUpdateError;
        const bool updated = hipGraphExecUpdate(prev->exec, graph, &err_node, &res) == hipSuccess && res == hipGraphExecUpdateSuccess && c->opt.exec_update != 2;
        if (updated) {
            exec = prev->exec;
            c->st.graph_exec_updates++;
        } else {
            (void) hipGetLastError();
            (void) hipGraphExecDestroy(prev->exec);
            c->st.graph_exec_update_failures++;
        }
        prev->exec = nullptr;
        if (prev->graph) (void) hipGraphDestroy(prev->graph);
        prev->graph = nullptr;
        prev->seen = 1;
    }
    if (exec == nullptr && (hipGraphInstantiate(&exec, graph, nullptr, nullptr, 0) != hipSuccess || exec == nullptr)) {
        (void) hipGetLastError();
        (void) hipGraphDestroy(graph);
        cg.seen = 1000001;
        if (shadow) return GGML_STATUS_SUCCESS;
        c->st.eager_graphs++;
        return run_nodes(c, g, wp) ? GGML_STATUS_SUCCESS : GGML_STATUS_FAILED;
    }
    c->st.graph_exec_update_ns += now_ns() - t_mark;
    cg.graph = graph;
    cg.exec = exec;
    cg.allreduces = red_captured;
    c->st.graph_captures++;
    c->st.graph_early_captures += early ? 1 : 0;
    if (shadow) {
        c->st.graph_shadow_captures++;
        return GGML_STATUS_SUCCESS;
    }
    if (hipGraphLaunch(cg.exec, c->stream) != hipSuccess) {
        (void) hipGetLastError();
        return GGML_STATUS_FAILED;
    }
    c->st.graph_launches++;
    return GGML_STATUS_SUCCESS;
}

}
```

### llama_box_amd/csrc/kernels.h

```cpp
#pragma once
#include "common.h"

namespace mi355x {

struct tdesc {
    char * data;
    int64_t ne[4];
    int64_t nb[4];
    int type;
};
inline tdesc TD(const ggml_tensor * t) {
    tdesc d;
    d.data = (char *) t->data;
    for (int i = 0; i < 4; ++i) {
        d.ne[i] = t->ne[i];
        d.nb[i] = (int64_t) t->nb[i];
    }
    d.type = (int) t->type;
    return d;
}

size_t quantized_act_bytes(int kind, int64_t K, int64_t rows);
void launch_quantize_act(hipStream_t s, int kind, const tdesc & src, void * dst);
#define MI_ACT_Q80_PANEL 1008
void launch_quantize_q80_panel(hipStream_t s, const tdesc & src, void * dst);
#define MI_ACT_Q81_PANEL 1009
bool rms_norm_q80_panel_ok(const tdesc & src, const float * w);
void launch_rms_norm_mul_q80_panel(hipStream_t s, const tdesc & src, float eps, const float * w, void * q80_panel);
bool swiglu_q80_panel_ok(const tdesc & a, const tdesc * b, int64_t nc, int swapped);
void launch_swiglu_q80_panel(hipStream_t s, const tdesc & a, const tdesc * b, int64_t nc, int swapped, void * q80_panel);

struct mmvq_args {
    const uint8_t * W;
    const uint8_t * W2;
    int64_t w_nb1;
    int type;
    int K, N;
    int ncols;
    const void * act;
    float * dst;
    int64_t dst_stride;
    const float * add;
    int64_t add_stride;
    const float * add2;
    int64_t add2_stride;
    const float * x;
    const float * norm_w;
    float eps;
    const float * fa_part;
    int fa_splits;
    float * x_out;
    float * norm_out;
    int balance_tail;
    double * ss_out;
    const double * ss_in;
    int ss_n;
    const uint8_t * Wp;
    const uint8_t * W2p;
};
int launch_mmvq_ss_count(const mmvq_args & a);
#define FA_REC 132
void launch_mmvq(hipStream_t s, const mmvq_args & a, int rows_per_wave);
struct launch_probe {
    hipEvent_t e0 = nullptr, e1 = nullptr;
    bool armed = false, used = false;
};
extern thread_local launch_probe g_launch_probe;
#define MI_LAUNCH_PROBED(kernel, grid, block, lds, stream, ...)                                                                  \
    do {                                                                                                                         \
        if (g_launch_probe.armed && !g_launch_probe.used) {                                                                      \
            hipExtLaunchKernelGGL(kernel, grid, block, lds, stream, g_launch_probe.e0, g_launch_probe.e1, 0, __VA_ARGS__);       \
            g_launch_probe.used = true;                                                                                          \
        } else {                                                                                                                 \
            hipLaunchKernelGGL(kernel, grid, block, lds, stream, __VA_ARGS__);                                                   \
        }                                                                                                                        \
    } while (0)

struct mmid_args {
    const uint8_t * W;
    int64_t w_nb1, w_nb2;
    int type;
    int K, N, n_expert;
    const char * ids;
    int64_t ids_nb1;
    int n_used, n_tokens;
    int b_rows;
    const void * act;
    const char * x;
    int64_t x_nb1, x_nb2;
    float * dst;
    int64_t dst_nb1, dst_nb2;
};
void launch_mmid(hipStream_t s, const mmid_args & a);

struct qkv_seg {
    const uint8_t * W;
    int64_t w_nb1;
    int N;
    uint8_t alt;
    uint8_t rope;
    uint8_t store;
    uint8_t kvt;
    const float * bias;
    char * out;
    int64_t row_stride;
};
struct qkv_args {
    qkv_seg seg[3];
    int nseg, K;
    const float * x;
    const float * norm_w;
    float eps;
    float * norm_out;
    int head_dim, neox;
    const int32_t * pos;
    const float * freq_factors;
    float theta_scale, freq_scale, ext_factor, attn_factor, corr0, corr1;
    const int64_t * slot;
    const float * rope_tab;
    int wg_a;
    int wv_a;
    int planes;
    const double * ss_in;
    int ss_n;
};
#define P2P_SLOT_FLOATS 65536
#define P2P_MAX_BLOCKS 32
#define P2P_MAX_RANKS 16
struct p2p_args {
    float * data;
    int n;
    int rank, world;
    char * mbox[P2P_MAX_RANKS];
    unsigned * state;
    unsigned max_spins;
    unsigned * err_host;
    const float * add;
    float * out;
    double * ss_out;
};
void launch_p2p_all_reduce(hipStream_t s, const p2p_args & a);
int p2p_all_reduce_blocks(int n);
bool qkv_types_supported(int type_a, int type_b);
void launch_qkv(hipStream_t s, const qkv_args & a, int type_a, int type_b);

void launch_mul_mat_f(hipStream_t s, const tdesc & src0, const tdesc & src1, const tdesc & dst, float * ws = nullptr, size_t ws_bytes = 0);
size_t mul_mat_f_workspace_bytes(const tdesc & src0, const tdesc & src1);
enum { MI_BF16_DOT = 0, MI_BF16_MMV = 1, MI_BF16_MMV_COLS = 2, MI_BF16_MMA16 = 3, MI_BF16_MMA = 4 };
int mul_mat_bf16_form(const tdesc & src0, const tdesc & src1, const tdesc & dst, int force, int max_cols);
const char * mul_mat_bf16_class(int form, int64_t n_cols);
int mul_mat_bf16_launches(int form, const tdesc & src0, const tdesc & src1);
void launch_mul_mat_bf16(hipStream_t s, const tdesc & src0, const tdesc & src1, const tdesc & dst, int form = -1, bool nt = MI_BF16_NT != 0, void * ws = nullptr, size_t ws_bytes = 0);
size_t mul_mat_bf16_workspace_bytes(const tdesc & src0, const tdesc & src1);
size_t attn_nf_list_scratch_bytes(const tdesc & q, const tdesc & k, int * dq_out);
bool launch_attn_nf_list(hipStream_t s, const tdesc & q, const tdesc & k, const tdesc & v, const tdesc & mask, const tdesc & dst, const int * lists, int list_stride,
                         float * scratch, size_t scratch_bytes, float scale, void * q8_out = nullptr );
bool launch_soft_max_mul_mat_f16(hipStream_t s, const tdesc & a, const tdesc & kq, const tdesc * mask, const tdesc & d, float scale);

bool mmq_supported(int type, int64_t K, int64_t N, int64_t M);
size_t mmq_workspace_bytes(int type, int64_t K, int64_t N, int64_t M, bool skinny);
bool mmq_skinny_mix_ok(const int * types, const int64_t * N, const int64_t * w_nb1, int n, int64_t K, int64_t M);
struct mmq_mat_desc { const uint8_t * W; int64_t w_nb1; int N; float * dst; int64_t dst_stride; const float * add; int64_t add_stride;
                      int type = 0; };
struct mmq_epi {
    int kind[3];
    char * out[3];
    int64_t nb1[3], nb2[3];
    const int32_t * pos;
    const float * ff;
    const int64_t * idx;
    const int64_t * v_idx;
    const float * tab;
    float theta_scale, freq_scale, ext_factor, attn_factor, corr0, corr1;
    int head_dim, n_dims;
};
int launch_mmq_i8_multi(hipStream_t s, int type, int n_mat, const mmq_mat_desc * mats, int K, int M, const void * act_q8k, int force_bn, int ksplit, float * part, bool reduce = true, bool skinny = false,
                        const mmq_epi * epi = nullptr );
void launch_splitk_reduce_mats(hipStream_t s, int n_mat, const mmq_mat_desc * mats, const float * part, int ks, int M);
bool mmq_i8_supported(int type, int64_t K, int64_t N, int64_t M);
int mmq_pick_ksplit(int64_t K, int64_t N, int64_t M, bool skinny, int type);
void launch_splitk_reduce(hipStream_t s, const float * part, int ks, int M, int N, float * dst, int64_t dst_stride, const float * add, int64_t add_stride);
int launch_mmq_i8(hipStream_t s, int type, const uint8_t * W, int64_t w_nb1, int K, int N, int M, const void * act_q8k, float * dst, int64_t dst_stride, int force_bn,
                   int ksplit, float * part, const float * add , int64_t add_stride, bool reduce = true, bool skinny = false, const mmq_epi * epi = nullptr);
bool mmq_skinny_supported(int type, int64_t K, int64_t N, int64_t M, int64_t w_nb1);
int mmq_skinny_ksplit(int64_t K, int64_t n_total);
bool mmq_q80_supported(int type, int64_t K, int64_t N, int64_t M);
void launch_mmq_q80(hipStream_t s, const uint8_t * W, const uint8_t * W_panels, int64_t w_nb1, int K, int N, int M, const void * act_q80, float * dst, int64_t dst_stride, const float * add, int64_t add_stride);
bool mmq_q80_skinny_supported(int type, int64_t K, int64_t N, int64_t M);
struct mmq80s_desc { const uint8_t * W; const uint8_t * W_panels; int64_t w_nb1; int N; float * dst; int64_t dst_stride; const float * add; int64_t add_stride; };
void launch_mmq_q80_skinny_multi(hipStream_t s, int n, const mmq80s_desc * mats, int K, int M, const void * act_q80_panel);
void launch_mmq_q80_skinny(hipStream_t s, const uint8_t * W, const uint8_t * W_panels, int64_t w_nb1, int K, int N, int M, const void * act_q80_panel, float * dst, int64_t dst_stride, const float * add, int64_t add_stride);
inline bool is_l32_type(int t) { return t == GGML_TYPE_Q4_0 || t == GGML_TYPE_Q4_1 || t == GGML_TYPE_Q5_0 || t == GGML_TYPE_Q5_1 || t == GGML_TYPE_IQ4_NL; }
int mmq_l32_form(int type, int64_t K, int64_t N, int64_t M);
void launch_mmq_l32(hipStream_t s, int type, int form, const uint8_t * W, int64_t w_nb1, int K, int N, int M, const void * act, float * dst, int64_t dst_stride, const float * add, int64_t add_stride);
void launch_mmq(hipStream_t s, int type, const uint8_t * W, int64_t w_nb1, int K, int N, int M, const void * act_q8k, float * dst, int64_t dst_stride, int ksplit, float * part);

void launch_rms_norm(hipStream_t s, const tdesc & src, const tdesc & dst, float eps, const tdesc * mul_w );
void launch_binary(hipStream_t s, int op, const tdesc & a, const tdesc & b, const tdesc & dst);
void launch_scale(hipStream_t s, const tdesc & src, const tdesc & dst, float scale, float bias);
void launch_unary(hipStream_t s, int uop, const tdesc & src, const tdesc & dst);
void launch_swiglu(hipStream_t s, const tdesc & a, const tdesc * b, const tdesc & dst, int swapped);
struct splitk_src { const float * part; int ks; int64_t mn; const float * add; int64_t add_stride; float * out; int64_t out_stride; };
void launch_splitk_rms_norm_mul_quantize(hipStream_t s, const splitk_src & sk, int rows, int K, const float * w, float eps, void * dst);
void launch_rms_norm_mul_quantize(hipStream_t s, const tdesc & x, const float * w, float eps, void * dst_q8k);
void launch_swiglu_quantize(hipStream_t s, const tdesc & a, const tdesc * b, int64_t nc, int swapped, void * dst_q8k);
void launch_cpy(hipStream_t s, const tdesc & src, const tdesc & dst);
void launch_get_rows(hipStream_t s, const tdesc & src, const tdesc & idx, const tdesc & dst);
void launch_set_rows(hipStream_t s, const tdesc & src, const tdesc & idx, const tdesc & dst);
void launch_cpy_q8_0(hipStream_t s, const void * src, void * dst, int64_t n_values, bool to_q8);
void launch_set_rows_q8_0(hipStream_t s, const tdesc & src, const tdesc & idx, const tdesc & dst);
bool kv_type_is_block(int type);
bool kv_store_type(int type);
bool kv_image_type(int type);
void launch_set_rows_kv(hipStream_t s, const tdesc & src, const tdesc & idx, const tdesc & dst);
void launch_set_rows_kv_pair(hipStream_t s, const tdesc & a0, const tdesc & i0, const tdesc & d0, const tdesc & a1, const tdesc & i1, const tdesc & d1);
void launch_cpy_kv(hipStream_t s, int type, const void * src, void * dst, int64_t n_values, bool to_type);
size_t kv_image_bytes(const tdesc & t);
tdesc kv_image_desc(const tdesc & t, void * image);
void launch_kv_images_f16(hipStream_t s, tdesc & k, tdesc & v, void * image);
void launch_argmax(hipStream_t s, const tdesc & src, const tdesc & dst);
#define MI_ARGSORT_MAX_COLS 1024
void launch_argsort(hipStream_t s, const tdesc & src, const tdesc & dst, int descending);
void launch_sum_rows(hipStream_t s, const tdesc & src, const tdesc & dst);
void launch_clamp(hipStream_t s, const tdesc & src, const tdesc & dst, float lo, float hi);
void launch_upload_multi(hipStream_t s, const upload_batch & b);
void launch_upload_small(hipStream_t s, void * dst, const void * pinned_src, size_t n);
void launch_copy2d(hipStream_t s, void * dst, size_t dpitch, const void * src, size_t spitch, size_t width, size_t height);
void launch_rebase_row_index(hipStream_t s, int64_t * dst, const int64_t * src, int64_t n_tok, int64_t full, int64_t ext, int64_t o0, int64_t n_ctx);
struct reduce_parts { const float * part[GGML_MI355X_MAX_DEVICES]; int n; };
void launch_reduce_parts(hipStream_t s, const reduce_parts & p, const float * add, float * dst, int64_t n);
void launch_norm(hipStream_t s, const tdesc & src, const tdesc & dst, float eps, const float * mul_w, const float * add_b);
bool launch_gelu(hipStream_t s, int unary_op, const tdesc & src, const tdesc & dst, const uint16_t * act_tab);
bool launch_glu(hipStream_t s, int glu_op, const tdesc & a, const tdesc * b, const tdesc & d, int swapped, const uint16_t * act_tab);


struct rope_params {
    int n_dims, mode, n_ctx_orig;
    float freq_base, freq_scale, ext_factor, attn_factor, beta_fast, beta_slow;
    int sections[4];
};
void rope_host_consts(const rope_params & p, float & theta_scale, float & corr0, float & corr1);
void launch_rope_table(hipStream_t s, const int32_t * pos, const float * ff, const rope_params & p, int n_tok, float * tab);
void launch_step_head(hipStream_t s, const tdesc * a, const tdesc * idx, const tdesc * d, const float * cp_src, void * cp_dst, int64_t cp_n,
                      const int32_t * pos, const float * ff, const rope_params * p, int n_tok, float * tab);
struct rope_store_args {
    const char * q_src; char * q_dst; const char * k_src; const char * v_src;
    int64_t q_nb1, q_nb2, qd_nb1, qd_nb2, k_nb1, k_nb2, v_nb1, v_nb2;
    char * k_cache; char * v_cache;
    int64_t kc_nb1, vc_nb1;
    const int64_t * idx;
    const int64_t * v_idx;
    const int32_t * pos;
    const float * ff;
    rope_params p;
    float theta_scale, corr0, corr1;
    int nh, nkv, head_dim;
    struct { const float * part; int64_t mn; const float * bias; int n; } sk[3];
    int ks;
};
void launch_rope_qk_store(hipStream_t s, rope_store_args a, int n_tokens);
bool rope_qk_store_vec_ok(const rope_store_args & a, int n_tokens);
void launch_rope_qk_store_vec(hipStream_t s, const rope_store_args & a, int n_tokens, const float * tab);
void launch_rope(hipStream_t s, const tdesc & src, const tdesc & pos, const float * freq_factors, const tdesc & dst, const rope_params & p);
void launch_soft_max(hipStream_t s, const tdesc & src, const tdesc * mask, const float * sinks, const tdesc & dst, float scale, float max_bias);

struct fattn_params {
    float scale, max_bias, logit_softcap;
    int n_splits;
    int fat = 0;
    int kv_type;
    int dq = 0;
    const int * lists = nullptr;
    void * q8_out = nullptr;
    unsigned * arrive = nullptr;
    int arrive_slots = 0;
    const uint8_t * tile_vis = nullptr;
    int mask_sparse = 0;
};
bool attn_nf_mma_applies(const tdesc & q, const tdesc & k, const tdesc & vt, const tdesc & mask);
size_t attn_nf_mma_ws_bytes(const tdesc & q, int n_splits);
void launch_attn_nf_mma(hipStream_t s, const tdesc & q, const tdesc & k, const tdesc & vt, const tdesc & mask, const tdesc & dst, float scale, int n_splits, const uint8_t * tile_vis, void * workspace,
                        void * q8_out = nullptr);
bool fattn_native_kv_ok(const tdesc & q, const tdesc & k, const tdesc & v, const fattn_params & p);
bool fattn_combine_rows_applies(int D, int64_t n_q, int64_t n_head, int64_t n_batch, int n_splits, const float * sinks);
size_t fattn_vis_bytes(const tdesc & q, const tdesc & k);
void launch_fattn_vis_scan(hipStream_t s, const tdesc & mask, int n_q, int n_kv, uint8_t * vis);
int fattn_list_tile(const tdesc & q, const tdesc & k, const tdesc * mask, const fattn_params & p, size_t lists_bytes);
void launch_fattn_tile_scan(hipStream_t s, const tdesc & mask, int n_q, int n_kv, int tile, int * lists);
size_t fattn_workspace_bytes(const tdesc & q, const tdesc & k, const tdesc & v, int n_splits, int kv_type);
int fattn_mma_min_q();
bool flash_attn_mma_applies(const tdesc & q, const tdesc & k, const tdesc * mask, const float * sinks, const tdesc & dst, const fattn_params & p);
int fattn_pick_splits(const tdesc & q, const tdesc & k, const tdesc * mask = nullptr, int mask_sparse = 0);
bool fattn_prefers_lists(const tdesc & q, const tdesc * mask, int mask_sparse);
int fattn_fat_splits(const tdesc & q, const tdesc & k, const tdesc * mask, const float * sinks, const fattn_params & p);
bool fattn_q8_out_ok(const tdesc & q, const tdesc & k, const tdesc * mask, const float * sinks, const tdesc & dst, const fattn_params & p);
void launch_flash_attn(hipStream_t s, const tdesc & q, const tdesc & k, const tdesc & v, const tdesc * mask, const float * sinks,
                       const tdesc & dst, const fattn_params & p, void * workspace);
bool launch_flash_attn_mma(hipStream_t s, const tdesc & q, const tdesc & k, const tdesc & v, const tdesc * mask, const float * sinks, const tdesc & dst,
                           const fattn_params & p, void * workspace);
int fattn_mma_pick_splits(const tdesc & q, const tdesc & k);
void launch_flash_attn_combine(hipStream_t s, int D, const float * ws, const float * sinks, const tdesc & dst, int n_q, int n_head, int n_batch, int n_splits, void * q8_out = nullptr);
enum {
    FA_FORM_K_SPLIT = 1, FA_FORM_K_DEC = 2, FA_FORM_K_MMA = 3,
    FA_FORM_MODE_PLAIN = 0, FA_FORM_MODE_SKIP = 1, FA_FORM_MODE_LIST = 2,
    FA_FORM_KV_F16 = 0, FA_FORM_KV_Q8_0 = 1, FA_FORM_KV_BLOCK = 2, FA_FORM_KV_Q8_IMAGE = 3,
    FA_FORM_TAIL_NONE = 0, FA_FORM_TAIL_COMBINE = 1, FA_FORM_TAIL_COMBINE_ROWS = 2, FA_FORM_TAIL_SELF_MERGE = 3, FA_FORM_TAIL_MERGE2 = 4, FA_FORM_TAIL_FAT = 5,
    FA_FORM_D256_BIT = 16,
};
static inline int fa_form_code(int kernel, int mode, int waves, int kv, int D, int tail) {
    if (D == 256) kernel |= 1 << FA_FORM_D256_BIT;
    return kernel | (mode << 4) | (waves << 6) | (kv << 10) | ((D == 128 ? 1 : 0) << 12) | (tail << 13);
}
extern thread_local int g_fa_form;

bool repack_supported(int type, int64_t K, int64_t nb1);
void launch_repack_planes(hipStream_t s, int type, const void * src, void * dst, int64_t K, int64_t nb1, int64_t r0, int64_t n_rows);
bool repack_q80_supported(int type, int64_t K, int64_t N, int64_t nb1);
void launch_repack_q80_panels(hipStream_t s, const void * src, void * dst, int64_t K, int64_t N, int64_t nb1);

bool launch_concat(hipStream_t s, const tdesc & a, const tdesc & b, const tdesc & dst, int dim);
bool launch_ssm_conv(hipStream_t s, const tdesc & sx, const tdesc & c, const tdesc & dst, const float * bias);
bool launch_ssm_scan(hipStream_t s, const tdesc & st, const tdesc & x, const tdesc & dt, const tdesc & A, const tdesc & B, const tdesc & C, const tdesc & ids, const tdesc & dst);

#define MI_TU_TOUCH(name) \
    __global__ void k_tu_touch_##name() {} \
    void tu_touch_##name(hipStream_t s) { hipLaunchKernelGGL(k_tu_touch_##name, dim3(1), dim3(64), 0, s); }
void tu_touch_quantize(hipStream_t s);
void tu_touch_mmvq(hipStream_t s);
void tu_touch_qkv(hipStream_t s);
void tu_touch_mmf(hipStream_t s);
void tu_touch_mmbf(hipStream_t s);
void tu_touch_attn_nf(hipStream_t s);
void tu_touch_mmq(hipStream_t s);
void tu_touch_mmq_i8(hipStream_t s);
void tu_touch_mmq_skinny(hipStream_t s);
void tu_touch_mmq_q80(hipStream_t s);
void tu_touch_ops(hipStream_t s);
void tu_touch_ops_act(hipStream_t s);
void tu_touch_fattn(hipStream_t s);
void tu_touch_fattn_mma(hipStream_t s);
void tu_touch_tp_p2p(hipStream_t s);
void tu_touch_kv_types(hipStream_t s);
void tu_touch_repack(hipStream_t s);
void tu_touch_mmid(hipStream_t s);
void tu_touch_ssm(hipStream_t s);
inline void preload_kernel_files(hipStream_t s) {
    tu_touch_kv_types(s);
    tu_touch_repack(s);
    tu_touch_quantize(s);
    tu_touch_mmvq(s);
    tu_touch_mmid(s);
    tu_touch_qkv(s);
    tu_touch_mmf(s);
    tu_touch_mmbf(s);
    tu_touch_attn_nf(s);
    tu_touch_mmq(s);
    tu_touch_mmq_i8(s);
    tu_touch_mmq_skinny(s);
    tu_touch_mmq_q80(s);
    tu_touch_ops(s);
    tu_touch_ops_act(s);
    tu_touch_fattn(s);
    tu_touch_fattn_mma(s);
    tu_touch_tp_p2p(s);
    tu_touch_ssm(s);
}

}
```

### llama_box_amd/csrc/ops.hip

```cpp
#include <algorithm>

#include "dev_util.h"
#include "kernels.h"
#include "kv_dequant.h"

namespace mi355x {

__device__ __forceinline__ double block_sum_d(double v, double * sh) {
    v = wave_sum_d(v);
    const int lane = threadIdx.x & 63, wave = threadIdx.x >> 6;
    __syncthreads();
    if (lane == 0) sh[wave] = v;
    __syncthreads();
    double t = 0.0;
    const int nw = blockDim.x >> 6;
    for (int i = 0; i < nw; ++i) t += sh[i];
    return t;
}
__device__ __forceinline__ float block_max_f(float v, float * sh) {
    v = wave_max(v);
    const int lane = threadIdx.x & 63, wave = threadIdx.x >> 6;
    __syncthreads();
    if (lane == 0) sh[wave] = v;
    __syncthreads();
// ... 664 lines not shown
        if (slot < a.nh) {
            const float * src = (const float *) (a.q_src + slot * a.q_nb1 + t * a.q_nb2);
            float * dst = (float *) (a.q_dst + slot * a.qd_nb1 + t * a.qd_nb2);
            for (int i0 = a.p.n_dims + lane; i0 < a.head_dim; i0 += 64) dst[i0] = ld(0, src, slot, i0);
        } else if (slot < a.nh + a.nkv) {
            const int h = slot - a.nh;
            const float * src = (const float *) (a.k_src + h * a.k_nb1 + t * a.k_nb2);
            uint16_t * dst = (uint16_t *) (a.k_cache + row * a.kc_nb1) + (int64_t) h * a.head_dim;
            for (int i0 = a.p.n_dims + lane; i0 < a.head_dim; i0 += 64) dst[i0] = f2h(ld(1, src, h, i0));
        } else {
            const int h = slot - a.nh - a.nkv;
            const float * src = (const float *) (a.v_src + h * a.v_nb1 + t * a.v_nb2);
            if (a.v_idx) {
                const int64_t * ix = a.v_idx + ((int64_t) t * a.nkv + h) * a.head_dim;
                for (int i0 = lane; i0 < a.head_dim; i0 += 64) ((uint16_t *) a.v_cache)[ix[i0]] = f2h(ld(2, src, h, i0));
            } else {
                uint16_t * dst = (uint16_t *) (a.v_cache + row * a.vc_nb1) + (int64_t) h * a.head_dim;
                for (int i0 = lane; i0 < a.head_dim; i0 += 64) dst[i0] = f2h(ld(2, src, h, i0));
            }
        }
    }
}
template <bool NEOX>
__global__ void __launch_bounds__(256) k_rope_qk_store_vec(const rope_store_args a, const float * __restrict__ tab) {
    const int64_t t = blockIdx.x;
    const int tid = threadIdx.x, hd = a.head_dim, half = hd >> 1;
    const int64_t row = a.idx[t];
    const int cph = NEOX ? hd / 8 : hd / 4;
    const int n_rot = (a.nh + a.nkv) * cph, n_v = a.nkv * (hd / 4);
    constexpr int MAXC = 6;
    for (int c0 = 0; c0 < n_rot + n_v; c0 += 256 * MAXC) {
        float4 lo[MAXC], hi[MAXC], cs[MAXC], cs2[MAXC];
#pragma unroll
        for (int k = 0; k < MAXC; ++k) {
            const int c = c0 + tid + 256 * k;
            if (c < n_rot) {
                const int slot = c / cph, j = c - slot * cph;
                const float * src = slot < a.nh ? (const float *) (a.q_src + (int64_t) slot * a.q_nb1 + t * a.q_nb2) : (const float *) (a.k_src + (int64_t) (slot - a.nh) * a.k_nb1 + t * a.k_nb2);
                lo[k] = *(const float4 *) (src + 4 * j);
                if (NEOX) {
                    hi[k] = *(const float4 *) (src + half + 4 * j);
                    cs[k] = *(const float4 *) (tab + ((size_t) t * half + 4 * j) * 2);
                    cs2[k] = *(const float4 *) (tab + ((size_t) t * half + 4 * j + 2) * 2);
                } else {
                    cs[k] = *(const float4 *) (tab + ((size_t) t * half + 2 * j) * 2);
                }
            } else if (c < n_rot + n_v) {
                const int cv = c - n_rot, h = cv / (hd / 4), j = cv - h * (hd / 4);
                lo[k] = *(const float4 *) ((const float *) (a.v_src + (int64_t) h * a.v_nb1 + t * a.v_nb2) + 4 * j);
            }
        }
#pragma unroll
        for (int k = 0; k < MAXC; ++k) {
            const int c = c0 + tid + 256 * k;
            if (c < n_rot) {
                const int slot = c / cph, j = c - slot * cph;
                float4 o0, o1;
                if (NEOX) {
                    o0 = make_float4(lo[k].x * cs[k].x - hi[k].x * cs[k].y, lo[k].y * cs[k].z - hi[k].y * cs[k].w, lo[k].z * cs2[k].x - hi[k].z * cs2[k].y, lo[k].w * cs2[k].z - hi[k].w * cs2[k].w);
                    o1 = make_float4(lo[k].x * cs[k].y + hi[k].x * cs[k].x, lo[k].y * cs[k].w + hi[k].y * cs[k].z, lo[k].z * cs2[k].y + hi[k].z * cs2[k].x, lo[k].w * cs2[k].w + hi[k].w * cs2[k].z);
                } else {
                    o0 = make_float4(lo[k].x * cs[k].x - lo[k].y * cs[k].y, lo[k].x * cs[k].y + lo[k].y * cs[k].x, lo[k].z * cs[k].z - lo[k].w * cs[k].w, lo[k].z * cs[k].w + lo[k].w * cs[k].z);
                    o1 = o0;
                }
                if (slot < a.nh) {
                    float * dst = (float *) (a.q_dst + (int64_t) slot * a.qd_nb1 + t * a.qd_nb2);
                    *(float4 *) (dst + 4 * j) = o0;
                    if (NEOX) *(float4 *) (dst + half + 4 * j) = o1;
                } else {
                    uint16_t * dst = (uint16_t *) (a.k_cache + row * a.kc_nb1) + (int64_t) (slot - a.nh) * hd;
                    *(uint2 *) (dst + 4 * j) = make_uint2((uint32_t) f2h(o0.x) | ((uint32_t) f2h(o0.y) << 16), (uint32_t) f2h(o0.z) | ((uint32_t) f2h(o0.w) << 16));
                    if (NEOX) *(uint2 *) (dst + half + 4 * j) = make_uint2((uint32_t) f2h(o1.x) | ((uint32_t) f2h(o1.y) << 16), (uint32_t) f2h(o1.z) | ((uint32_t) f2h(o1.w) << 16));
                }
            } else if (c < n_rot + n_v) {
                const int cv = c - n_rot, h = cv / (hd / 4), j = cv - h * (hd / 4);
                if (a.v_idx) {
                    const int64_t * ix = a.v_idx + ((int64_t) t * a.nkv + h) * hd + 4 * j;
                    const int64_t i0 = ix[0], i1 = ix[1], i2 = ix[2], i3 = ix[3];
                    uint16_t * vc = (uint16_t *) a.v_cache;
                    vc[i0] = f2h(lo[k].x);
                    vc[i1] = f2h(lo[k].y);
                    vc[i2] = f2h(lo[k].z);
                    vc[i3] = f2h(lo[k].w);
                } else {
                    uint16_t * dst = (uint16_t *) (a.v_cache + row * a.vc_nb1) + (int64_t) h * hd;
                    *(uint2 *) (dst + 4 * j) = make_uint2((uint32_t) f2h(lo[k].x) | ((uint32_t) f2h(lo[k].y) << 16), (uint32_t) f2h(lo[k].z) | ((uint32_t) f2h(lo[k].w) << 16));
                }
            }
        }
    }
}
bool rope_qk_store_vec_ok(const rope_store_args & a, int n_tokens) {
    static const bool on = env_flag("GGML_MI355X_ROPE_VEC", true);
    if (!on || n_tokens < 33 || a.ks > 1 || a.sk[0].part || a.sk[1].part || a.sk[2].part) return false;
    if ((a.p.mode & ~GGML_ROPE_TYPE_NEOX) != 0 || a.p.n_dims != a.head_dim || (a.head_dim % 8) != 0) return false;
    auto al16 = [](const void * p) { return (((uintptr_t) p) & 15) == 0; };
    if (!al16(a.q_src) || !al16(a.q_dst) || !al16(a.k_src) || !al16(a.v_src) || !al16(a.k_cache) || !al16(a.v_cache)) return false;
    for (int64_t v : {a.q_nb1, a.q_nb2, a.qd_nb1, a.qd_nb2, a.k_nb1, a.k_nb2, a.v_nb1, a.v_nb2})
        if (v % 16) return false;
    return (a.kc_nb1 % 8) == 0 && (a.v_idx != nullptr || (a.vc_nb1 % 8) == 0);
}
void launch_rope_qk_store_vec(hipStream_t s, const rope_store_args & a, int n_tokens, const float * tab) {
    if (a.p.mode & GGML_ROPE_TYPE_NEOX) hipLaunchKernelGGL(k_rope_qk_store_vec<true>, dim3((unsigned) n_tokens), dim3(256), 0, s, a, tab);
    else hipLaunchKernelGGL(k_rope_qk_store_vec<false>, dim3((unsigned) n_tokens), dim3(256), 0, s, a, tab);
}
void launch_rope_qk_store(hipStream_t s, rope_store_args a, int n_tokens) {
    rope_host_consts(a.p, a.theta_scale, a.corr0, a.corr1);
    const int n_all = a.nh + 2 * a.nkv;
    const int shares = n_tokens >= 256 ? 1 : std::max(1, std::min((n_all + 3) / 4, 1024 / std::max(1, n_tokens)));
    hipLaunchKernelGGL(k_rope_qk_store, dim3((unsigned) n_tokens, (unsigned) shares), dim3(256), 0, s, a);
}
void launch_rope(hipStream_t s, const tdesc & a, const tdesc & pos, const float * ff, const tdesc & d, const rope_params & p) {
    float theta_scale, c0, c1;
    rope_host_consts(p, theta_scale, c0, c1);
    dim3 grid((unsigned) a.ne[1], (unsigned) a.ne[2], (unsigned) a.ne[3]);
    if (p.mode & GGML_ROPE_TYPE_MROPE) {
        if (a.type == GGML_TYPE_F16) hipLaunchKernelGGL(k_rope_multi<true>, grid, dim3(64), 0, s, a, (const int32_t *) pos.data, ff, d, p, theta_scale, c0, c1);
        else hipLaunchKernelGGL(k_rope_multi<false>, grid, dim3(64), 0, s, a, (const int32_t *) pos.data, ff, d, p, theta_scale, c0, c1);
        return;
    }
    if (a.type == GGML_TYPE_F16) hipLaunchKernelGGL(k_rope<true>, grid, dim3(64), 0, s, a, pos, ff, d, p, theta_scale, c0, c1);
    else hipLaunchKernelGGL(k_rope<false>, grid, dim3(64), 0, s, a, pos, ff, d, p, theta_scale, c0, c1);
}

__global__ void __launch_bounds__(256) k_soft_max(const tdesc a, const tdesc m, const int has_mask, const float * __restrict__ sinks, const tdesc d,
                                                  const float scale, const float max_bias, const float m0, const float m1, const uint32_t n_head_log2) {
    __shared__ double shd[4];
    __shared__ float shf[4];
    const int64_t row = blockIdx.x;
    const int64_t i1 = row % a.ne[1], i2 = (row / a.ne[1]) % a.ne[2], i3 = row / (a.ne[1] * a.ne[2]);
    const float * x = (const float *) (a.data + i1 * a.nb[1] + i2 * a.nb[2] + i3 * a.nb[3]);
    float * y = (float *) (d.data + i1 * d.nb[1] + i2 * d.nb[2] + i3 * d.nb[3]);
    const char * mp = has_mask ? m.data + i1 * m.nb[1] + (i2 % m.ne[2]) * m.nb[2] + (i3 % m.ne[3]) * m.nb[3] : nullptr;
    const uint32_t h = (uint32_t) i2;
    const float slope = max_bias > 0.0f ? (h < n_head_log2 ? powf(m0, (float) (h + 1)) : powf(m1, (float) (2 * (h - n_head_log2) + 1))) : 1.0f;
    const int64_t n = a.ne[0];
    float mx = -INFINITY;
    for (int64_t i = threadIdx.x; i < n; i += blockDim.x) {
        float w = x[i] * scale;
        if (mp) {
            const float mv = m.type == GGML_TYPE_F16 ? h2f(((const uint16_t *) mp)[i]) : ((const float *) mp)[i];
            w += slope * mv;
        }
        y[i] = w;
        mx = fmaxf(mx, w);
    }
    mx = block_max_f(mx, shf);
    if (sinks) mx = fmaxf(mx, sinks[i2]);
    double sum = 0.0;
    for (int64_t i = threadIdx.x; i < n; i += blockDim.x) {
        const float v = expf(y[i] - mx);
        y[i] = v;
        sum += (double) v;
    }
    sum = block_sum_d(sum, shd);
    if (sinks) sum += (double) expf(sinks[i2] - mx);
    if (isnan(sum) || sum == 0.0) sum = -INFINITY;
    const float inv = (float) (1.0 / sum);
    for (int64_t i = threadIdx.x; i < n; i += blockDim.x) y[i] *= inv;
}
template <int NR>
__global__ void __launch_bounds__(256) k_soft_max_reg(const tdesc a, const tdesc m, const int has_mask, const float * __restrict__ sinks, const tdesc d,
                                                      const float scale, const float max_bias, const float m0, const float m1, const uint32_t n_head_log2) {
    __shared__ double shd[4];
    __shared__ float shf[4];
    const int64_t row = blockIdx.x;
    const int64_t i1 = row % a.ne[1], i2 = (row / a.ne[1]) % a.ne[2], i3 = row / (a.ne[1] * a.ne[2]);
    const float * x = (const float *) (a.data + i1 * a.nb[1] + i2 * a.nb[2] + i3 * a.nb[3]);
    float * y = (float *) (d.data + i1 * d.nb[1] + i2 * d.nb[2] + i3 * d.nb[3]);
    const char * mp = has_mask ? m.data + i1 * m.nb[1] + (i2 % m.ne[2]) * m.nb[2] + (i3 % m.ne[3]) * m.nb[3] : nullptr;
    const uint32_t h = (uint32_t) i2;
    const float slope = max_bias > 0.0f ? (h < n_head_log2 ? powf(m0, (float) (h + 1)) : powf(m1, (float) (2 * (h - n_head_log2) + 1))) : 1.0f;
    const int n = (int) a.ne[0];
    const bool m16 = m.type == GGML_TYPE_F16;
    float w[NR];
    float mx = -INFINITY;
#pragma unroll
    for (int j = 0; j < NR; ++j) {
        const int i = threadIdx.x + 256 * j;
        w[j] = -INFINITY;
        if (i < n) {
            float v = x[i] * scale;
            if (mp) v += slope * (m16 ? h2f(((const uint16_t *) mp)[i]) : ((const float *) mp)[i]);
            w[j] = v;
            mx = fmaxf(mx, v);
        }
    }
    mx = block_max_f(mx, shf);
    if (sinks) mx = fmaxf(mx, sinks[i2]);
    double sum = 0.0;
#pragma unroll
    for (int j = 0; j < NR; ++j) {
        if ((int) threadIdx.x + 256 * j < n) {
            w[j] = expf(w[j] - mx);
            sum += (double) w[j];
        }
    }
    sum = block_sum_d(sum, shd);
    if (sinks) sum += (double) expf(sinks[i2] - mx);
    if (isnan(sum) || sum == 0.0) sum = -INFINITY;
    const float inv = (float) (1.0 / sum);
#pragma unroll
    for (int j = 0; j < NR; ++j) {
        const int i = threadIdx.x + 256 * j;
        if (i < n) y[i] = w[j] * inv;
    }
}
void launch_soft_max(hipStream_t s, const tdesc & a, const tdesc * mask, const float * sinks, const tdesc & d, float scale, float max_bias) {
    const uint32_t n_head = (uint32_t) a.ne[2];
    const uint32_t n_head_log2 = 1u << (uint32_t) floor(log2((double) n_head));
    const float m0 = powf(2.0f, -(max_bias) / (float) n_head_log2);
    const float m1 = powf(2.0f, -(max_bias / 2.0f) / (float) n_head_log2);
    const int64_t rows = a.ne[1] * a.ne[2] * a.ne[3];
    tdesc dummy = a;
#define SM_REG(NR) hipLaunchKernelGGL(k_soft_max_reg<NR>, dim3((unsigned) rows), dim3(256), 0, s, a, mask ? *mask : dummy, mask ? 1 : 0, sinks, d, scale, max_bias, m0, m1, n_head_log2)
    if (a.nb[0] == 4 && d.nb[0] == 4 && a.ne[0] <= 256 * 32) {
        if (a.ne[0] <= 256 * 4) SM_REG(4);
        else if (a.ne[0] <= 256 * 12) SM_REG(12);
        else SM_REG(32);
        return;
    }
#undef SM_REG
    hipLaunchKernelGGL(k_soft_max, dim3((unsigned) rows), dim3(256), 0, s, a, mask ? *mask : dummy, mask ? 1 : 0, sinks, d, scale, max_bias, m0, m1, n_head_log2);
}

__global__ void __launch_bounds__(64) k_set_rows_q8_0(const tdesc a, const tdesc idx, const tdesc d) {
    const int lane = threadIdx.x;
    const int64_t chunks = (a.ne[0] + 255) / 256;
    const int64_t gid = blockIdx.x;
    const int64_t row = gid / chunks, ch = gid - row * chunks;
    const int64_t i01 = row % a.ne[1], i02 = (row / a.ne[1]) % a.ne[2], i03 = row / (a.ne[1] * a.ne[2]);
    const int64_t i12 = i03 % idx.ne[2], i11 = i02 % idx.ne[1];
    const int64_t r = *(const int64_t *) (idx.data + i01 * idx.nb[0] + i11 * idx.nb[1] + i12 * idx.nb[2]);
    const bool live = ch * 256 + lane * 4 < a.ne[0];
    const float4 x = live ? ((const float4 *) (a.data + i01 * a.nb[1] + i02 * a.nb[2] + i03 * a.nb[3]))[ch * 64 + lane] : make_float4(0.f, 0.f, 0.f, 0.f);
    const float v[4] = {x.x, x.y, x.z, x.w};
    float amax = fmaxf(fmaxf(fabsf(v[0]), fabsf(v[1])), fmaxf(fabsf(v[2]), fabsf(v[3])));
    amax = fmaxf(amax, dpp_f32<MI_DPP_QUAD_XOR1>(amax));
    amax = fmaxf(amax, dpp_f32<MI_DPP_QUAD_XOR2>(amax));
    amax = fmaxf(amax, dpp_f32<MI_DPP_HALF_MIRROR>(amax));
    const float dd = amax / 127.0f;
    const float id = dd != 0.0f ? 1.0f / dd : 0.0f;
    uint32_t packed = 0;
#pragma unroll
    for (int k = 0; k < 4; ++k) packed |= (uint32_t) ((int) roundf(v[k] * id) & 0xFF) << (8 * k);
    char * blk = d.data + r * d.nb[1] + i02 * d.nb[2] + i03 * d.nb[3] + (ch * 8 + (lane >> 3)) * 34;
    if (!live) return;
    uint16_t * qs = (uint16_t *) (blk + 2 + 4 * (lane & 7));
    qs[0] = (uint16_t) (packed & 0xFFFF);
    qs[1] = (uint16_t) (packed >> 16);
    if ((lane & 7) == 0) *(uint16_t *) blk = f2h(dd);
}
void launch_set_rows_q8_0(hipStream_t s, const tdesc & a, const tdesc & idx, const tdesc & d) {
    const int64_t blocks = ((a.ne[0] + 255) / 256) * a.ne[1] * a.ne[2] * a.ne[3];
    hipLaunchKernelGGL(k_set_rows_q8_0, dim3((unsigned) blocks), dim3(64), 0, s, a, idx, d);
}

__global__ void __launch_bounds__(256) k_cpy_q8_0_f32(const char * __restrict__ src, float * __restrict__ dst, const int64_t n4) {
    const int64_t i = (int64_t) blockIdx.x * 256 + threadIdx.x;
    if (i >= n4) return;
    const char * blk = src + (i >> 3) * 34;
    const float d = h2f(ld16(blk));
    const uint32_t qs = ld32_a2(blk + 2 + 4 * (i & 7));
    ((float4 *) dst)[i] = make_float4(d * (float) (int8_t) qs, d * (float) (int8_t) (qs >> 8), d * (float) (int8_t) (qs >> 16), d * (float) (int8_t) (qs >> 24));
}
__global__ void __launch_bounds__(256) k_cpy_f32_q8_0(const float * __restrict__ src, char * __restrict__ dst, const int64_t n4) {
    const int64_t i = (int64_t) blockIdx.x * 256 + threadIdx.x;
    const bool live = i < n4;
    const float4 x = live ? ((const float4 *) src)[i] : make_float4(0.f, 0.f, 0.f, 0.f);
    const float v[4] = {x.x, x.y, x.z, x.w};
    float amax = fmaxf(fmaxf(fabsf(v[0]), fabsf(v[1])), fmaxf(fabsf(v[2]), fabsf(v[3])));
    amax = fmaxf(amax, dpp_f32<MI_DPP_QUAD_XOR1>(amax));
    amax = fmaxf(amax, dpp_f32<MI_DPP_QUAD_XOR2>(amax));
    amax = fmaxf(amax, dpp_f32<MI_DPP_HALF_MIRROR>(amax));
    const float dd = amax / 127.0f;
    const float id = dd != 0.0f ? 1.0f / dd : 0.0f;
    uint32_t packed = 0;
#pragma unroll
    for (int k = 0; k < 4; ++k) packed |= (uint32_t) ((int) roundf(v[k] * id) & 0xFF) << (8 * k);
    if (!live) return;
    char * blk = dst + (i >> 3) * 34;
    uint16_t * qs = (uint16_t *) (blk + 2 + 4 * (i & 7));
    qs[0] = (uint16_t) (packed & 0xFFFF);
    qs[1] = (uint16_t) (packed >> 16);
    if ((i & 7) == 0) *(uint16_t *) blk = f2h(dd);
}
void launch_cpy_q8_0(hipStream_t s, const void * src, void * dst, int64_t n, bool to_q8) {
    const int64_t n4 = n / 4;
    const unsigned grid = (unsigned) ((n4 + 255) / 256);
    if (to_q8) hipLaunchKernelGGL(k_cpy_f32_q8_0, dim3(grid), dim3(256), 0, s, (const float *) src, (char *) dst, n4);
    else hipLaunchKernelGGL(k_cpy_q8_0_f32, dim3(grid), dim3(256), 0, s, (const char *) src, (float *) dst, n4);
}

__global__ void __launch_bounds__(256) k_upload_small(char * __restrict__ dst, const char * __restrict__ src, const size_t n, const int vec) {
    const size_t i = (size_t) blockIdx.x * 256 + threadIdx.x;
    if (vec == 16) {
        if (i * 16 < n) ((uint4 *) dst)[i] = ((const uint4 *) src)[i];
    } else if (vec == 4) {
        if (i * 4 < n) ((uint32_t *) dst)[i] = ((const uint32_t *) src)[i];
    } else {
        if (i < n) dst[i] = src[i];
    }
}
void launch_upload_small(hipStream_t s, void * dst, const void * pinned_src, size_t n) {
    const uintptr_t al = (uintptr_t) dst | (uintptr_t) pinned_src | (uintptr_t) n;
    const int vec = (al & 15) == 0 ? 16 : ((al & 3) == 0 ? 4 : 1);
    const size_t items = (n + vec - 1) / vec;
    hipLaunchKernelGGL(k_upload_small, dim3((unsigned) ((items + 255) / 256)), dim3(256), 0, s, (char *) dst, (const char *) pinned_src, n, vec);
}

__global__ void __launch_bounds__(256) k_upload_multi(const upload_batch b) {
    const upload_seg sg = b.seg[blockIdx.y];
    const uintptr_t al = (uintptr_t) sg.dst | (uintptr_t) sg.src | (uintptr_t) sg.n;
    for (size_t i = (size_t) blockIdx.x * 256 + threadIdx.x;; i += (size_t) gridDim.x * 256) {
        if ((al & 15) == 0) {
            if (i * 16 >= sg.n) break;
            ((uint4 *) sg.dst)[i] = ((const uint4 *) sg.src)[i];
        } else if ((al & 3) == 0) {
            if (i * 4 >= sg.n) break;
            ((uint32_t *) sg.dst)[i] = ((const uint32_t *) sg.src)[i];
        } else {
            if (i >= sg.n) break;
            sg.dst[i] = sg.src[i];
        }
    }
}
void launch_upload_multi(hipStream_t s, const upload_batch & b) {
    size_t most = 0;
    for (int i = 0; i < b.n; ++i) most = std::max(most, b.seg[i].n);
    const unsigned gx = (unsigned) std::min<size_t>(16, (most / 16 + 255) / 256 + 1);
    hipLaunchKernelGGL(k_upload_multi, dim3(gx, (unsigned) b.n), dim3(256), 0, s, b);
}

__global__ void __launch_bounds__(256) k_copy2d(char * __restrict__ dst, const size_t dpitch, const char * __restrict__ src, const size_t spitch, const size_t width, const int vec) {
    const size_t row = blockIdx.y;
    char * d = dst + row * dpitch;
    const char * s = src + row * spitch;
    for (size_t i = (size_t) blockIdx.x * 256 + threadIdx.x;; i += (size_t) gridDim.x * 256) {
        if (vec == 16) {
            if (i * 16 >= width) break;
            ((uint4 *) d)[i] = ((const uint4 *) s)[i];
        } else if (vec == 2) {
            if (i * 2 >= width) break;
            ((uint16_t *) d)[i] = ((const uint16_t *) s)[i];
        } else {
            if (i >= width) break;
            d[i] = s[i];
        }
    }
}
void launch_copy2d(hipStream_t s, void * dst, size_t dpitch, const void * src, size_t spitch, size_t width, size_t height) {
    if (width == 0 || height == 0) return;
    const uintptr_t al = (uintptr_t) dst | (uintptr_t) src | (uintptr_t) dpitch | (uintptr_t) spitch | (uintptr_t) width;
    const int vec = (al & 15) == 0 ? 16 : ((al & 1) == 0 ? 2 : 1);
    const size_t items = (width + vec - 1) / vec;
    const unsigned gx = (unsigned) std::min<size_t>(64, (items + 255) / 256);
    for (size_t r0 = 0; r0 < height; r0 += 65535) {
        const size_t h = std::min<size_t>(65535, height - r0);
        hipLaunchKernelGGL(k_copy2d, dim3(gx, (unsigned) h), dim3(256), 0, s, (char *) dst + r0 * dpitch, dpitch, (const char *) src + r0 * spitch, spitch, width, vec);
    }
}

__global__ void __launch_bounds__(256) k_rebase_row_index(int64_t * __restrict__ dst, const int64_t * __restrict__ src, const int64_t n_tok, const int64_t full, const int64_t ext,
                                                         const int64_t o0, const int64_t n_ctx) {
    const int64_t e = (int64_t) blockIdx.x * 256 + threadIdx.x;
    if (e >= n_tok * ext) return;
    const int64_t i = e / ext, j = e - i * ext;
    dst[e] = src[i * full + o0 + j] - o0 * n_ctx;
}
void launch_rebase_row_index(hipStream_t s, int64_t * dst, const int64_t * src, int64_t n_tok, int64_t full, int64_t ext, int64_t o0, int64_t n_ctx) {
    const int64_t n = n_tok * ext;
    if (n <= 0) return;
    hipLaunchKernelGGL(k_rebase_row_index, dim3((unsigned) ((n + 255) / 256)), dim3(256), 0, s, dst, src, n_tok, full, ext, o0, n_ctx);
}

template <bool DESC> __device__ __forceinline__ bool argsort_before(const float va, const int ia, const float vb, const int ib, const int n) {
    const bool pa = ia >= n, pb = ib >= n;
    if (pa || pb) return pa == pb ? ia < ib : pb;
    if (va != vb) return DESC ? va > vb : va < vb;
    return ia < ib;
}
template <bool DESC> __global__ void __launch_bounds__(256) k_argsort(const tdesc a, const tdesc d, const int npad) {
    __shared__ float sv[MI_ARGSORT_MAX_COLS];
    __shared__ int si[MI_ARGSORT_MAX_COLS];
    const int n = (int) a.ne[0];
    const int64_t r = blockIdx.x;
    const int64_t i1 = r % a.ne[1], i2 = (r / a.ne[1]) % a.ne[2], i3 = r / (a.ne[1] * a.ne[2]);
    const float * x = (const float *) (a.data + i1 * a.nb[1] + i2 * a.nb[2] + i3 * a.nb[3]);
    int32_t * y = (int32_t *) (d.data + i1 * d.nb[1] + i2 * d.nb[2] + i3 * d.nb[3]);
    for (int i = threadIdx.x; i < npad; i += 256) {
        sv[i] = i < n ? x[i] : 0.0f;
        si[i] = i;
    }
    __syncthreads();
    for (int k = 2; k <= npad; k <<= 1) {
        for (int j = k >> 1; j > 0; j >>= 1) {
            for (int t = threadIdx.x; t < (npad >> 1); t += 256) {
                const int lo = ((t & ~(j - 1)) << 1) | (t & (j - 1)), hi = lo | j;
                const float vl = sv[lo], vh = sv[hi];
                const int il = si[lo], ih = si[hi];
                const bool up = (lo & k) == 0;
                if (argsort_before<DESC>(vh, ih, vl, il, n) == up) {
                    sv[lo] = vh; sv[hi] = vl;
                    si[lo] = ih; si[hi] = il;
                }
            }
            __syncthreads();
        }
    }
    for (int i = threadIdx.x; i < n; i += 256) y[i] = si[i];
}
void launch_argsort(hipStream_t s, const tdesc & a, const tdesc & d, int descending) {
    const int64_t rows = a.ne[1] * a.ne[2] * a.ne[3];
    if (a.ne[0] < 1 || a.ne[0] > MI_ARGSORT_MAX_COLS) { MI_ERR("launch_argsort: rows of %lld values", (long long) a.ne[0]); abort(); }
    int npad = 1;
    while (npad < a.ne[0]) npad <<= 1;
    if (descending) hipLaunchKernelGGL(k_argsort<true>, dim3((unsigned) rows), dim3(256), 0, s, a, d, npad);
    else hipLaunchKernelGGL(k_argsort<false>, dim3((unsigned) rows), dim3(256), 0, s, a, d, npad);
}

__global__ void __launch_bounds__(256) k_sum_rows(const tdesc a, const tdesc d, const int64_t rows) {
    const int lane = threadIdx.x & 63;
    const int64_t r = (int64_t) blockIdx.x * 4 + (threadIdx.x >> 6);
    if (r >= rows) return;
    const int64_t i1 = r % a.ne[1], i2 = (r / a.ne[1]) % a.ne[2], i3 = r / (a.ne[1] * a.ne[2]);
    const float * x = (const float *) (a.data + i1 * a.nb[1] + i2 * a.nb[2] + i3 * a.nb[3]);
    double sum = 0.0;
    for (int64_t i = lane; i < a.ne[0]; i += 64) sum += (double) x[i];
    sum = wave_sum_d(sum);
    if (lane == 0) *(float *) (d.data + i1 * d.nb[1] + i2 * d.nb[2] + i3 * d.nb[3]) = (float) sum;
}
void launch_sum_rows(hipStream_t s, const tdesc & a, const tdesc & d) {
    const int64_t rows = a.ne[1] * a.ne[2] * a.ne[3];
    hipLaunchKernelGGL(k_sum_rows, dim3((unsigned) ((rows + 3) / 4)), dim3(256), 0, s, a, d, rows);
}

__global__ void __launch_bounds__(256) k_clamp(const float * x, float * y, const int64_t n, const float lo, const float hi) {
    for (int64_t i = (int64_t) blockIdx.x * blockDim.x + threadIdx.x; i < n; i += (int64_t) gridDim.x * blockDim.x) {
        const float v = x[i];
        const float m = v < hi ? v : hi;
        y[i] = m > lo ? m : lo;
    }
}
void launch_clamp(hipStream_t s, const tdesc & a, const tdesc & d, float lo, float hi) {
    const int64_t n = a.ne[0] * a.ne[1] * a.ne[2] * a.ne[3];
    const unsigned grid = (unsigned) std::min<int64_t>((n + 255) / 256, 2048);
    hipLaunchKernelGGL(k_clamp, dim3(grid), dim3(256), 0, s, (const float *) a.data, (float *) d.data, n, lo, hi);
}

MI_TU_TOUCH(ops)

}
```

### llama_box_amd/csrc/tp_inproc.cpp

```cpp
#include <algorithm>
#include <condition_variable>
#include <deque>
#include <list>
#include <mutex>
#include <thread>
#include <unordered_map>

#include "common.h"
#include "kernels.h"

namespace mi355x {

static constexpr int MAXD = GGML_MI355X_MAX_DEVICES;

struct sdesc {
    int kind = 0;
    int dim = 0;
    int64_t off[MAXD + 1] = {0};
};
static bool same_off(const sdesc & a, const sdesc & b, int n) {
    for (int i = 0; i <= n; ++i)
        if (a.off[i] != b.off[i]) return false;
    return true;
}
// ... 658 lines not shown
        }
        case GGML_OP_GET_ROWS: case GGML_OP_RMS_NORM: case GGML_OP_SCALE: case GGML_OP_UNARY: case GGML_OP_CPY: case GGML_OP_DUP: case GGML_OP_ARGMAX:
            return all_replicated();
        default:
            return A.fail("an op the engine has no rule for", t);
    }
}

struct rewriter {
    ip_engine * E;
    ip_plan * P;
    analysis * A;
    int dev;
    std::unordered_map<const ggml_tensor *, ggml_tensor *> done;
    std::unordered_map<const ggml_tensor *, ggml_tensor *> vidx_done;
    bool ok = true;
};
static void contiguous_strides(ggml_tensor * c) {
    c->nb[0] = ggml_abi_type_size(c->type);
    c->nb[1] = c->nb[0] * (size_t) (c->ne[0] / ggml_abi_blck_size(c->type));
    c->nb[2] = c->nb[1] * (size_t) c->ne[1];
    c->nb[3] = c->nb[2] * (size_t) c->ne[2];
}
static char * mirror_addr(rewriter & R, const ggml_tensor * t, bool kv) {
    const int mi = mirror_of(R.E, root_buffer(t));
    if (mi < 0 || !mirror_ready(R.E, mi, kv)) { R.ok = false; return nullptr; }
    const ip_mirror & m = R.E->mirrors[(size_t) mi];
    return m.base[R.dev] + ((char *) t->data - m.host_base);
}
static ggml_tensor * clone_of(rewriter & R, const ggml_tensor * t);
static ggml_tensor * new_clone(rewriter & R, const ggml_tensor * t) {
    R.P->store[R.dev].push_back(*t);
    ggml_tensor * c = &R.P->store[R.dev].back();
    c->extra = nullptr;
    c->buffer = &R.E->buf_plain[R.dev];
    for (int s = 0; s < GGML_MAX_SRC; ++s) c->src[s] = nullptr;
    c->view_src = nullptr;
    return c;
}
static ggml_tensor * clone_leaf(rewriter & R, const ggml_tensor * t) {
    const sdesc & sd = R.A->d[t];
    ggml_tensor * c = new_clone(R, t);
    const int d = R.dev;
    if (buffer_is_split(t->buffer)) {
        const split_tensor_info * info = split_info(t);
        const int64_t ext = sd.off[d + 1] - sd.off[d];
        if (info->kind == 0) {
            c->ne[1] = ext;
            c->nb[1] = info->row_bytes;
        } else {
            c->ne[0] = ext;
            c->nb[1] = info->slice_row_bytes[d];
            c->buffer = &R.E->buf_rowpar[d];
        }
        c->nb[2] = c->nb[1] * (size_t) c->ne[1];
        c->nb[3] = c->nb[2];
        c->data = info->slice[d];
        return c;
    }
    if (sd.kind == 1) {
        const int64_t ext = sd.off[d + 1] - sd.off[d];
        c->ne[sd.dim] = ext;
        contiguous_strides(c);
        c->data = mirror_addr(R, t, true);
        return c;
    }
    if (is_weight(t)) {
        c->data = replica_of(R.E, d, t);
        if (!c->data) R.ok = false;
        return c;
    }
    c->data = mirror_addr(R, t, false);
    return c;
}
static ggml_tensor * clone_of(rewriter & R, const ggml_tensor * t) {
    auto it = R.done.find(t);
    if (it != R.done.end()) return it->second;
    ggml_tensor * c = nullptr;
    if (t->op == GGML_OP_NONE) {
        c = clone_leaf(R, t);
        R.done[t] = c;
        return c;
    }
    const sdesc & sd = R.A->d[t];
    const int d = R.dev;
    c = new_clone(R, t);
    R.done[t] = c;
    for (int s = 0; s < GGML_MAX_SRC; ++s)
        if (t->src[s]) c->src[s] = clone_of(R, t->src[s]);
    if (t->view_src) c->view_src = clone_of(R, t->view_src);
    const int64_t ext = sd.kind == 1 ? sd.off[d + 1] - sd.off[d] : 0;
    switch (t->op) {
        case GGML_OP_RESHAPE:
            if (sd.kind == 1) { c->ne[sd.dim] = ext; contiguous_strides(c); }
            c->data = c->src[0]->data;
            break;
        case GGML_OP_PERMUTE:
            for (int i = 0; i < 4; ++i) { c->ne[t->op_params[i]] = c->src[0]->ne[i]; c->nb[t->op_params[i]] = c->src[0]->nb[i]; }
            c->data = c->src[0]->data;
            break;
        case GGML_OP_TRANSPOSE:
            c->ne[0] = c->src[0]->ne[1]; c->ne[1] = c->src[0]->ne[0]; c->nb[0] = c->src[0]->nb[1]; c->nb[1] = c->src[0]->nb[0];
            c->ne[2] = c->src[0]->ne[2]; c->ne[3] = c->src[0]->ne[3]; c->nb[2] = c->src[0]->nb[2]; c->nb[3] = c->src[0]->nb[3];
            c->data = c->src[0]->data;
            break;
        case GGML_OP_VIEW:
            if (sd.kind == 1) {
                c->ne[2] = ext;
                c->nb[1] = c->src[0]->nb[1];
                c->nb[3] = c->nb[2] * (size_t) c->ne[2];
            }
            c->data = (char *) (c->view_src ? c->view_src->data : c->src[0]->data) + t->view_offs;
            break;
        case GGML_OP_SET_ROWS:
            if (t->ne[0] == 1 && sd.kind == 1) {
                c->ne[1] = ext;
                contiguous_strides(c);
                auto vi = R.A->vidx.find(t->src[1]);
                if (vi != R.A->vidx.end()) {
                    ggml_tensor *& ix = R.vidx_done[t->src[1]];
                    if (!ix) {
                        ix = new_clone(R, t->src[1]);
                        ix->ne[0] = vi->second.n_tok * (vi->second.off[d + 1] - vi->second.off[d]);
                        ix->ne[1] = ix->ne[2] = ix->ne[3] = 1;
                        contiguous_strides(ix);
                        ix->data = nullptr;
                    }
                    c->src[1] = ix;
                }
            } else {
                for (int i = 0; i < 4; ++i) { c->ne[i] = c->view_src->ne[i]; c->nb[i] = c->view_src->nb[i]; }
            }
            c->data = c->view_src->data;
            break;
        default:
            if (sd.kind == 1) { c->ne[sd.dim] = ext; contiguous_strides(c); }
            c->data = mirror_addr(R, t, false);
            break;
    }
    if ((t->op == GGML_OP_ADD || t->op == GGML_OP_SUB || t->op == GGML_OP_MUL || t->op == GGML_OP_DIV) && sd.kind == 1 && R.A->d[t->src[1]].kind == 0) {
        ggml_tensor * b = new_clone(R, t->src[1]);
        b->ne[0] = ext;
        contiguous_strides(b);
        b->data = (char *) c->src[1]->data + (size_t) sd.off[d] * sizeof(float);
        c->src[1] = b;
    }
    return c;
}

static ip_plan * build_plan(ip_engine * E, const ggml_cgraph * g) {
    E->plans.emplace_back();
    ip_plan * P = &E->plans.back();
    graph_key_build(g, P->key);
    E->plans_built++;
    analysis A;
    A.E = E;
    A.g = g;
    A.n = E->n_dev;
    bool any_split = false;
    for (int i = 0; i < g->n_nodes; ++i) {
        const ggml_tensor * t = g->nodes[i];
        if (!analyse_node(A, t)) {
            MI_INFO("in-process tensor parallel declines a graph of %d nodes: %s (node %d '%s'); it runs node by node on the main device", g->n_nodes, A.why, i, A.where ? A.where->name : "?");
            P->declined = true;
            return P;
        }
        any_split = any_split || (t->op == GGML_OP_MUL_MAT && buffer_is_split(t->src[0]->buffer));
    }
    if (!any_split) { P->declined = true; return P; }
    for (auto & kv : A.d) {
        const ggml_tensor * t = kv.first;
        if (t->op != GGML_OP_NONE || kv.second.kind != 1 || buffer_is_split(t->buffer)) continue;
        bool known = false;
        for (const ip_kv_tensor & k : E->kv) known = known || k.host_ptr == (char *) t->data;
        if (known) continue;
        const int mi = mirror_of(E, root_buffer(t));
        if (mi < 0) { P->declined = true; return P; }
        ip_kv_tensor k;
        k.host_ptr = (char *) t->data;
        k.dim = kv.second.dim;
        k.type = t->type;
        k.ne0 = t->ne[0];
        k.rows = t->ne[1];
        k.host_row_bytes = t->nb[1];
        for (int i = 0; i <= E->n_dev; ++i) k.off[i] = kv.second.off[i];
        k.mirror = mi;
        E->kv.push_back(k);
        if (E->mirrors[(size_t) mi].kv && E->mirrors[(size_t) mi].state == 0) E->mirrors[(size_t) mi].state = 2;
    }
    for (int d = 0; d < E->n_dev; ++d) {
        rewriter R;
        R.E = E;
        R.P = P;
        R.A = &A;
        R.dev = d;
        for (int i = 0; i < g->n_nodes && R.ok; ++i) P->nodes[d].push_back(clone_of(R, g->nodes[i]));
        if (!R.ok) {
            MI_ERR("in-process tensor parallel: building device %d's graph failed (memory for a mirror or a replica?)", E->ordinal[d]);
            P->declined = true;
            return P;
        }
        for (auto & vd : R.vidx_done) {
            const analysis::vidx_t & v = A.vidx[vd.first];
            ip_rebase * rb = nullptr;
            const int mi = mirror_of(E, root_buffer(vd.first));
            if (mi < 0) { P->declined = true; return P; }
            const size_t moff = (size_t) ((char *) vd.first->data - E->mirrors[(size_t) mi].host_base);
            for (ip_rebase & x : P->rebases)
                if (x.mirror == mi && x.moff == moff) rb = &x;
            if (!rb) {
                P->rebases.emplace_back();
                rb = &P->rebases.back();
                rb->mirror = mi;
                rb->moff = moff;
                rb->n_tok = v.n_tok;
                rb->full = v.full;
                rb->n_ctx = v.n_ctx;
                for (int k = 0; k <= E->n_dev; ++k) rb->off[k] = v.off[k];
                int64_t widest = 0;
                for (int k = 0; k < E->n_dev; ++k) widest = std::max(widest, v.off[k + 1] - v.off[k]);
                rb->stage_off = P->stage_bytes;
                P->stage_bytes += ((size_t) (v.n_tok * widest) * 8 + 255) & ~(size_t) 255;
            }
            rb->clones[d].push_back(vd.second);
        }
        ggml_cgraph & cg = P->graph[d];
        memset(&cg, 0, sizeof(cg));
        cg.size = (int) P->nodes[d].size();
        cg.n_nodes = (int) P->nodes[d].size();
        cg.nodes = P->nodes[d].data();
        if (d != 0) continue;
        for (auto & kv : R.done) {
            const ggml_tensor * t = kv.first;
            if (t->op != GGML_OP_NONE || buffer_is_split(t->buffer) || is_weight(t) || A.d[t].kind != 0) continue;
            const int mi = mirror_of(E, root_buffer(t));
            if (mi < 0 || E->mirrors[(size_t) mi].kv) continue;
            P->inputs.push_back({mi, (size_t) ((char *) t->data - E->mirrors[(size_t) mi].host_base), ggml_abi_nbytes(t)});
        }
    }
    for (int i = 0; i < g->n_nodes; ++i) {
        const ggml_tensor * t = g->nodes[i];
        const sdesc & sd = A.d[t];
        if (!(t->flags & GGML_TENSOR_FLAG_OUTPUT) || sd.kind == 0) continue;
        if (sd.dim != 0 || t->type != GGML_TYPE_F32 || !ggml_abi_is_contiguous(t)) { P->declined = true; return P; }
        ip_output o;
        o.node = i;
        o.host_ptr = (char *) t->data;
        o.ne0 = t->ne[0];
        o.cols = ggml_abi_nelements(t) / t->ne[0];
        for (int k = 0; k <= E->n_dev; ++k) o.off[k] = sd.off[k];
        o.stage_off = P->stage_bytes;
        int64_t widest = 0;
        for (int k = 0; k < E->n_dev; ++k) widest = std::max(widest, sd.off[k + 1] - sd.off[k]);
        P->stage_bytes += ((size_t) widest * (size_t) o.cols * 4 + 255) & ~(size_t) 255;
        P->outputs.push_back(o);
        for (int d = 0; d < E->n_dev; ++d) P->nodes[d][(size_t) i]->data = nullptr;
    }
    return P;
}

static bool ensure_stage(ip_engine * E, size_t need) {
    if (need <= E->stage_size) return true;
    for (int d = 0; d < E->n_dev; ++d) {
        if (hipSetDevice(E->ordinal[d]) != hipSuccess) { (void) hipGetLastError(); return false; }
        (void) hipStreamSynchronize(E->ctx[d]->stream);
        if (E->stage[d]) (void) hipFree(E->stage[d]);
        E->stage[d] = nullptr;
        if (hipMalloc((void **) &E->stage[d], need + (1u << 20)) != hipSuccess) { (void) hipGetLastError(); (void) hipSetDevice(E->main->device); return false; }
        free_graph_cache(E->ctx[d]);
    }
    E->stage_size = need + (1u << 20);
    (void) hipSetDevice(E->main->device);
    return true;
}

static enum ggml_status prepare_device(ip_engine * E, ip_plan * P, int d) {
    backend_ctx * w = E->ctx[d];
    HIP_TRY(hipSetDevice(E->ordinal[d]), GGML_STATUS_FAILED);
    if (d != E->main_dev) {
        HIP_TRY(hipStreamWaitEvent(w->stream, E->ev_in, 0), GGML_STATUS_FAILED);
        for (const ip_input & in : P->inputs) {
            const ip_mirror & m = E->mirrors[(size_t) in.mirror];
            launch_copy2d(w->stream, m.base[d] + in.off, in.bytes, m.host_base + in.off, in.bytes, in.bytes, 1);
        }
    }
    for (const ip_rebase & rb : P->rebases) {
        const ip_mirror & m = E->mirrors[(size_t) rb.mirror];
        launch_rebase_row_index(w->stream, (int64_t *) (E->stage[d] + rb.stage_off), (const int64_t *) (m.base[d] + rb.moff), rb.n_tok, rb.full, rb.off[d + 1] - rb.off[d], rb.off[d], rb.n_ctx);
    }
    return hipGetLastError() == hipSuccess ? GGML_STATUS_SUCCESS : GGML_STATUS_FAILED;
}
static enum ggml_status launch_device(ip_engine * E, ip_plan * P, int d) {
    backend_ctx * w = E->ctx[d];
    HIP_TRY(hipSetDevice(E->ordinal[d]), GGML_STATUS_FAILED);
    static const bool graphs_ok = env_flag("GGML_MI355X_SPLIT_GRAPHS", true);
    const bool graphs_was = w->opt.graphs;
    w->opt.graphs = graphs_was && graphs_ok;
    static const char * dbg_order = getenv("GGML_MI355X_DBG_SUBMIT_ORDER");
    if (dbg_order && E->threaded) {
        const int my = dbg_order[0] == 'd' ? E->n_dev - 1 - d : (dbg_order[0] == 'm' ? (d == E->main_dev ? 0 : E->n_dev - d) : d);
        std::unique_lock<std::mutex> lk(E->turn_m);
        E->turn_cv.wait(lk, [&] { return E->turn == my; });
    }
    const enum ggml_status st = graph_compute(w, &P->graph[d]);
    if (dbg_order && E->threaded) {
        std::lock_guard<std::mutex> lk(E->turn_m);
        E->turn++;
        E->turn_cv.notify_all();
    }
    w->opt.graphs = graphs_was;
    return st;
}
static void worker_main(ip_engine * E, int d) {
    ip_worker * W = E->workers[d];
    std::unique_lock<std::mutex> lk(W->m);
    for (;;) {
        W->cv.wait(lk, [&] { return W->job != nullptr || W->quit; });
        if (W->quit) return;
        ip_plan * P = W->job;
        lk.unlock();
        enum ggml_status st = prepare_device(E, P, d);
        W->prepared.store(E->epoch, std::memory_order_release);
        if (st == GGML_STATUS_SUCCESS) st = launch_device(E, P, d);
        lk.lock();
        W->result = st;
        W->job = nullptr;
        W->cv.notify_all();
    }
}

static enum ggml_status run_plan(ip_engine * E, ip_plan * P, const ggml_cgraph * g) {
    backend_ctx * c = E->main;
    struct guard { int dev; ~guard() { if (hipSetDevice(dev) != hipSuccess) (void) hipGetLastError(); } } restore{c->device};
    if (!(E->opt_seen == c->opt)) {
        for (int d = 0; d < E->n_dev; ++d) {
            if (d == E->main_dev) continue;
            if (hipSetDevice(E->ordinal[d]) == hipSuccess) (void) hipStreamSynchronize(E->ctx[d]->stream);
            E->ctx[d]->opt = c->opt;
            free_graph_cache(E->ctx[d]);
        }
        E->opt_seen = c->opt;
        (void) hipSetDevice(c->device);
    }
    if (!ensure_stage(E, P->stage_bytes)) return GGML_STATUS_ALLOC_FAILED;
    (void) g;
    for (const ip_output & o : P->outputs)
        for (int d = 0; d < E->n_dev; ++d) P->nodes[d][(size_t) o.node]->data = E->stage[d] + o.stage_off;
    for (const ip_rebase & rb : P->rebases)
        for (int d = 0; d < E->n_dev; ++d)
            for (ggml_tensor * ix : rb.clones[d]) ix->data = E->stage[d] + rb.stage_off;
    for (size_t mi = 0; mi < E->mirrors.size(); ++mi) {
        ip_mirror & m = E->mirrors[mi];
        if (!m.kv) continue;
        if (m.state == 2) {
            HIP_TRY(hipStreamSynchronize(c->stream), GGML_STATUS_FAILED);
            if (!kv_move(E, (int) mi, false)) return GGML_STATUS_FAILED;
        }
        m.state = 1;
    }
    HIP_TRY(hipSetDevice(c->device), GGML_STATUS_FAILED);
    HIP_TRY(hipEventRecord(E->ev_in, c->stream), GGML_STATUS_FAILED);
    enum ggml_status st = GGML_STATUS_SUCCESS;
    E->epoch++;
    E->input_copies += (int64_t) P->inputs.size() * (E->n_dev - 1);
    E->turn = 0;
    if (E->threaded) {
        for (int d = 0; d < E->n_dev; ++d) {
            if (d == E->main_dev) continue;
            ip_worker * W = E->workers[d];
            std::lock_guard<std::mutex> lk(W->m);
            W->job = P;
            W->cv.notify_all();
        }
    }
    for (int d = 0; d < E->n_dev; ++d) {
        if (d == E->main_dev) continue;
        if (E->threaded) {
            while (E->workers[d]->prepared.load(std::memory_order_acquire) != E->epoch) std::this_thread::yield();
        } else if (st == GGML_STATUS_SUCCESS) {
            st = prepare_device(E, P, d);
        }
    }
    if (st == GGML_STATUS_SUCCESS) st = prepare_device(E, P, E->main_dev);
    if (st == GGML_STATUS_SUCCESS) {
        E->running = true;
        st = launch_device(E, P, E->main_dev);
        E->running = false;
    }
    if (st == GGML_STATUS_SUCCESS) HIP_TRY(hipEventRecord(E->ev_done[E->main_dev], c->stream), GGML_STATUS_FAILED);
    for (int d = 0; d < E->n_dev; ++d) {
        if (d == E->main_dev) continue;
        if (E->threaded) {
            ip_worker * W = E->workers[d];
            std::unique_lock<std::mutex> lk(W->m);
            W->cv.wait(lk, [&] { return W->job == nullptr; });
            if (W->result != GGML_STATUS_SUCCESS) st = W->result;
        } else if (st == GGML_STATUS_SUCCESS) {
            st = launch_device(E, P, d);
        }
    }
    for (int d = 0; d < E->n_dev && st == GGML_STATUS_SUCCESS; ++d) {
        backend_ctx * w = E->ctx[d];
        HIP_TRY(hipSetDevice(E->ordinal[d]), GGML_STATUS_FAILED);
        if (!P->outputs.empty() && d != E->main_dev) HIP_TRY(hipStreamWaitEvent(w->stream, E->ev_done[E->main_dev], 0), GGML_STATUS_FAILED);
        for (const ip_output & o : P->outputs) {
            const int64_t ext = o.off[d + 1] - o.off[d];
            launch_copy2d(w->stream, o.host_ptr + (size_t) o.off[d] * 4, (size_t) o.ne0 * 4, E->stage[d] + o.stage_off, (size_t) ext * 4, (size_t) ext * 4, (size_t) o.cols);
            E->output_copies++;
        }
        if (d != E->main_dev) HIP_TRY(hipEventRecord(E->ev_done[d], w->stream), GGML_STATUS_FAILED);
    }
    HIP_TRY(hipSetDevice(c->device), GGML_STATUS_FAILED);
    if (st == GGML_STATUS_SUCCESS)
        for (int d = 0; d < E->n_dev; ++d)
            if (d != E->main_dev) HIP_TRY(hipStreamWaitEvent(c->stream, E->ev_done[d], 0), GGML_STATUS_FAILED);
    if (st != GGML_STATUS_SUCCESS) {
        for (int d = 0; d < E->n_dev; ++d)
            if (hipSetDevice(E->ordinal[d]) == hipSuccess) (void) hipStreamSynchronize(E->ctx[d]->stream);
        (void) hipGetLastError();
    }
    E->graphs++;
    return st;
}

enum ggml_status ip_graph_compute(backend_ctx * c, ggml_cgraph * g, bool * handled) {
    *handled = false;
    static const bool on = env_flag("GGML_MI355X_SPLIT_TP", true);
    if (!on || c->capturing) return GGML_STATUS_SUCCESS;
    ip_engine * E = c->ip;
    if (E && (E->dead || E->running)) return GGML_STATUS_SUCCESS;
    ip_plan * P = nullptr;
    if (E && E->last && graph_key_equals(g, E->last->key)) {
        P = E->last;
    } else {
        const ggml_tensor * w = nullptr;
        for (int i = 0; i < g->n_nodes && !w; ++i)
            if (g->nodes[i]->op == GGML_OP_MUL_MAT && buffer_is_split(g->nodes[i]->src[0]->buffer)) w = g->nodes[i]->src[0];
        if (!w) {
            if (E) {
                for (int i = 0; i < g->n_nodes; ++i) {
                    const ggml_tensor * t = g->nodes[i];
                    if (root_buffer(t)) ip_host_access(root_buffer(t), true);
                    for (int s = 0; s < GGML_MAX_SRC; ++s)
                        if (t->src[s] && root_buffer(t->src[s])) ip_host_access(root_buffer(t->src[s]), false);
                }
            }
            return GGML_STATUS_SUCCESS;
        }
        if (!E) {
            const split_tensor_info * info = split_info(w);
            const int main_dev = split_buft_main_device(w->buffer->buft);
            if (!info || main_dev < 0 || main_dev >= info->n_dev || logical_device_ordinal(main_dev) != c->device) return GGML_STATUS_SUCCESS;
            E = c->ip = engine_new(c, info->n_dev, main_dev);
            if (!E || E->dead) return GGML_STATUS_SUCCESS;
        }
        std::vector<uint64_t> key;
        graph_key_build(g, key);
        for (ip_plan & p : E->plans)
            if (p.key == key) { P = &p; break; }
        if (!P) {
            if (E->plans.size() > 48) {
                for (auto it = E->plans.begin(); it != E->plans.end();) {
                    if (&*it != E->last && it->last_use + 64 < E->tick) it = E->plans.erase(it);
                    else ++it;
                }
            }
            P = build_plan(E, g);
        }
    }
    E->tick++;
    P->last_use = E->tick;
    if (P->declined) {
        E->declined++;
        for (size_t mi = 0; mi < E->mirrors.size(); ++mi)
            if (E->mirrors[mi].kv) ip_host_access(E->mirrors[mi].host, true);
        return GGML_STATUS_SUCCESS;
    }
    E->last = P;
    *handled = true;
    return run_plan(E, P, g);
}

}
```

Baseline: 590.0.

## Park graph replay and fuse the logits download into a tail-copy graph

Result: no change. 593.4 (median of 6 runs) (+0.6%).

```diff
diff --git a/include/ggml_mi355x.h b/include/ggml_mi355x.h
--- a/include/ggml_mi355x.h
+++ b/include/ggml_mi355x.h
@@ -26,6 +26,9 @@
 typedef ggml_backend_buffer_type_t (*ggml_backend_mi355x_tp_rowpar_buffer_type_t)(int device);
 
 typedef int (*ggml_backend_mi355x_graph_key_probe_t)(const struct ggml_cgraph * a, const struct ggml_cgraph * b, int64_t * n_words);
+typedef int64_t (*ggml_backend_mi355x_graph_key_build_t)(const struct ggml_cgraph * g, uint64_t * out, int64_t cap);
+typedef int (*ggml_backend_mi355x_graph_key_equals_t)(const struct ggml_cgraph * g, const uint64_t * key, int64_t n);
+typedef int64_t (*ggml_backend_mi355x_graph_key_time_t)(const struct ggml_cgraph * g, int iters, int rounds, int inline_cmp);
 
 typedef int64_t (*ggml_backend_mi355x_decode_copy_read_t)(ggml_backend_t backend, const struct ggml_tensor * t, void * out, size_t size);
 
diff --git a/llama_box_amd/csrc/backend.cpp b/llama_box_amd/csrc/backend.cpp
--- a/llama_box_amd/csrc/backend.cpp
+++ b/llama_box_amd/csrc/backend.cpp
@@ -53,6 +53,18 @@
 }
 
 static void uploader_drain(int device);
+std::atomic<int> g_parked_count{0};
+static std::mutex g_backends_mtx;
+static std::vector<backend_ctx *> g_backends;
+static void parked_flush_all() {
+    if (g_parked_count.load(std::memory_order_acquire) <= 0) return;
+    std::lock_guard<std::mutex> lock(g_backends_mtx);
+    for (backend_ctx * c : g_backends)
+        if (c->parked.load(std::memory_order_acquire)) {
+            HIP_SOFT(hipSetDevice(c->device));
+            graph_launch_parked(c, nullptr);
+        }
+}
 static std::atomic<uint64_t> g_decode_epoch{1};
 uint64_t decode_copy_epoch() { return g_decode_epoch.load(std::memory_order_acquire); }
 static void decode_copy_drop(buffer_ctx * c, size_t off, size_t n) {
@@ -193,6 +205,7 @@
     return u;
 }
 static void uploader_drain(int device) {
+    parked_flush_all();
     if (device < 0 || device >= GGML_MI355X_MAX_DEVICES) return;
     uploader * u = &g_uploaders[device];
     if (u->device != device) return;
@@ -201,6 +214,11 @@
     HIP_SOFT(hipStreamSynchronize(u->stream));
     for (bool & b : u->busy) b = false;
     u->in_flight = false;
+}
+static bool uploader_busy(int device) {
+    if (device < 0 || device >= GGML_MI355X_MAX_DEVICES) return false;
+    const uploader * u = &g_uploaders[device];
+    return u->device == device && u->in_flight;
 }
 static void uploader_join(int device, hipStream_t s) {
     if (device < 0 || device >= GGML_MI355X_MAX_DEVICES) return;
@@ -344,6 +362,7 @@
     HIP_SOFT(hipSetDevice(c->device));
     note_mask_upload(t, data, offset, size);
     decode_copy_drop(b, t, offset, size);
+    parked_flush_all();
     if (size > ((size_t) 1 << 20) && staged_upload(c->device, (char *) t->data + offset, (const char *) data, size)) return;
     uploader_drain(c->device);
     HIP_SOFT(hipMemcpy((char *) t->data + offset, data, size, hipMemcpyHostToDevice));
@@ -441,6 +460,7 @@
     return false;
 }
 static void hbuf_free(ggml_backend_buffer_t b) {
+    parked_flush_all();
     {
         std::lock_guard<std::mutex> lock(g_pinned_mtx);
         for (size_t i = 0; i < g_pinned.size(); ++i)
@@ -475,8 +495,13 @@
 static void be_free(ggml_backend_t be) {
     backend_ctx * c = (backend_ctx *) be->context;
     HIP_SOFT(hipSetDevice(c->device));
+    flush_uploads(c);
     HIP_SOFT(hipStreamSynchronize(c->stream));
     free_graph_cache(c);
+    {
+        std::lock_guard<std::mutex> lock(g_backends_mtx);
+        g_backends.erase(std::remove(g_backends.begin(), g_backends.end(), c), g_backends.end());
+    }
     ip_free(c);
     tp_free(c);
     free_split_helpers(c);
@@ -492,6 +517,8 @@
     delete be;
 }
 void flush_uploads(backend_ctx * c) {
+    if (c->parked.load(std::memory_order_relaxed)) graph_launch_parked(c, nullptr);
+    c->follow = nullptr;
     if (c->up_pending.n == 0) return;
     launch_upload_multi(c->stream, c->up_pending);
     c->up_pending.n = 0;
@@ -533,11 +560,18 @@
     backend_ctx * c = (backend_ctx *) be->context;
     if (ip_any()) ip_host_access(t->view_src ? t->view_src->buffer : t->buffer, false);
     HIP_SOFT(hipSetDevice(c->device));
+    const bool by_kernel = c->opt.small_downloads && size > 0 && size <= ((size_t) 8 << 20) && is_pinned_range(data, size);
+    if (by_kernel && c->parked.load(std::memory_order_relaxed) && c->up_pending.n == 0 && !uploader_busy(c->device)) {
+        const tail_copy cp = {data, (const char *) t->data + offset, size};
+        if (graph_launch_parked(c, &cp)) return;
+    }
+    cached_graph * const followed = c->up_pending.n == 0 ? c->follow : nullptr;
     flush_uploads(c);
     uploader_join(c->device, c->stream);
-    if (c->opt.small_downloads && size > 0 && size <= ((size_t) 8 << 20) && is_pinned_range(data, size)) {
+    if (by_kernel) {
         launch_upload_small(c->stream, data, (const char *) t->data + offset, size);
         c->st.kernel_downloads++;
+        graph_note_download(followed, tail_copy{data, (const char *) t->data + offset, size});
         return;
     }
     HIP_SOFT(hipMemcpyAsync(data, (const char *) t->data + offset, size, hipMemcpyDeviceToHost, c->stream));
@@ -662,6 +696,11 @@
     }
     options_from_env(c->opt);
     c->ssm_fuse = env_flag("GGML_MI355X_SSM_FUSE", true);
+    c->step_tail = env_flag("GGML_MI355X_STEP_TAIL", false);
+    {
+        std::lock_guard<std::mutex> lock(g_backends_mtx);
+        g_backends.push_back(c);
+    }
     if (hipMalloc((void **) &c->ss_buf, 256 * sizeof(double)) != hipSuccess) {
         (void) hipGetLastError();
         c->ss_buf = nullptr;
@@ -717,6 +756,7 @@
     backend_ctx * c = (backend_ctx *) be->context;
     if (!tp_active(c)) return -2;
     HIP_TRY(hipSetDevice(c->device), -3);
+    flush_uploads(c);
     return tp_all_reduce(c, device_ptr, n) ? 0 : -4;
 }
 static int api_tp_p2p_attach(ggml_backend_t be, const void * handles, size_t n) {
@@ -735,10 +775,34 @@
     if (n_words) *n_words = (int64_t) key.size();
     return graph_key_equals(b, key) ? 1 : 0;
 }
+static int64_t api_graph_key_build(const ggml_cgraph * g, uint64_t * out, int64_t cap) {
+    std::vector<uint64_t> key;
+    graph_key_build(g, key);
+    if (out && cap >= (int64_t) key.size()) memcpy(out, key.data(), key.size() * 8);
+    return (int64_t) key.size();
+}
+static int api_graph_key_equals(const ggml_cgraph * g, const uint64_t * key, int64_t n) {
+    const std::vector<uint64_t> k(key, key + (n > 0 ? n : 0));
+    return graph_key_equals(g, k) ? 1 : 0;
+}
+static int64_t api_graph_key_time(const ggml_cgraph * g, int iters, int rounds, int inline_cmp) {
+    std::vector<uint64_t> key;
+    graph_key_build(g, key);
+    graph_key_set_inline(inline_cmp != 0);
+    int64_t best = INT64_MAX;
+    for (int r = 0; r < std::max(1, rounds); ++r) {
+        const auto t0 = std::chrono::steady_clock::now();
+        for (int i = 0; i < std::max(1, iters); ++i)
+            if (!graph_key_equals(g, key)) return -1;
+        best = std::min<int64_t>(best, std::chrono::duration_cast<std::chrono::nanoseconds>(std::chrono::steady_clock::now() - t0).count() / std::max(1, iters));
+    }
+    return best;
+}
 static int64_t api_decode_copy_read(ggml_backend_t be, const ggml_tensor * t, void * out, size_t size) {
     if (!be_is_ours(be) || t == nullptr) return -1;
     backend_ctx * c = (backend_ctx *) be->context;
     if (hipSetDevice(c->device) != hipSuccess) return -1;
+    flush_uploads(c);
     uploader_join(c->device, c->stream);
     const uint8_t * p = t->type == GGML_TYPE_Q8_0 ? q80_panel_copy(c, t) : decode_copy(c, t);
     if (!p) return 0;
@@ -752,12 +816,16 @@
     backend_ctx * c = (backend_ctx *) be->context;
     const std::string k = key;
     const int v = atoi(value);
+    HIP_SOFT(hipSetDevice(c->device));
+    flush_uploads(c);
     if (!options_set(c->opt, key, v)) {
         if (k == "tp_p2p") { if (!tp_p2p_enable(c, v != 0)) return -2; }
         else if (k == "tp_p2p_reset") { if (!tp_p2p_reset(c)) return -2; }
         else if (k == "clear_failure") { if (v) clear_hip_failure(); }
         else if (k == "staged_upload") g_staged_upload.store(v != 0);
         else if (k == "ssm_fuse") c->ssm_fuse = v != 0;
+        else if (k == "step_tail") c->step_tail = v != 0;
+        else if (k == "key_inline") graph_key_set_inline(v != 0);
         else return -1;
     }
     HIP_SOFT(hipStreamSynchronize(c->stream));
@@ -770,6 +838,7 @@
     const std::string k = key;
     if (const int64_t * p = stats_find(c->st, key)) return *p;
     if (k == "graph_cache_size") return (int64_t) c->graphs.size();
+    if (k == "graph_tail_copies") return c->tail_copies;
     if (k == "p2p_timeouts") return tp_p2p_timeouts(c);
     if (k.rfind("ip_", 0) == 0) return ip_stat(c, key);
     if (k == "staged_upload_bytes") return (int64_t) g_uploaders[c->device].bytes;
@@ -779,6 +848,7 @@
 static int api_timing_report(ggml_backend_t be, char * buf, size_t size, int reset) {
     if (!be_is_ours(be) || !buf || size == 0) return -1;
     backend_ctx * c = (backend_ctx *) be->context;
+    flush_uploads(c);
     HIP_SOFT(hipStreamSynchronize(c->stream));
     for (auto & pe : c->pending_events) {
         float ms = 0;
@@ -822,6 +892,9 @@
     if (n == "ggml_backend_split_buffer_type") return (void *) api_split_buffer_type;
     if (n == "ggml_backend_mi355x_split_rows") return (void *) api_split_rows;
     if (n == "ggml_backend_mi355x_graph_key_probe") return (void *) api_graph_key_probe;
+    if (n == "ggml_backend_mi355x_graph_key_build") return (void *) api_graph_key_build;
+    if (n == "ggml_backend_mi355x_graph_key_equals") return (void *) api_graph_key_equals;
+    if (n == "ggml_backend_mi355x_graph_key_time") return (void *) api_graph_key_time;
     return nullptr;
 }
 static const ggml_backend_reg_i k_reg_iface = {reg_get_name, reg_get_device_count, reg_get_device, reg_get_proc_address};
diff --git a/llama_box_amd/csrc/common.h b/llama_box_amd/csrc/common.h
--- a/llama_box_amd/csrc/common.h
+++ b/llama_box_amd/csrc/common.h
@@ -112,6 +112,17 @@
     int fa_form = 0;
     bool early_failed = false;
     std::vector<uint64_t> key;
+    bool tail_ok = false;
+    bool tail_failed = false;
+    hipGraph_t tail_graph = nullptr;
+    hipGraphExec_t tail_exec = nullptr;
+    hipGraphNode_t tail_node = nullptr;
+    void * tail_dst = nullptr;
+    const void * tail_src = nullptr;
+    size_t tail_size = 0;
+    void * want_dst = nullptr;
+    const void * want_src = nullptr;
+    size_t want_size = 0;
 };
 
 struct timing_slot {
@@ -137,6 +148,10 @@
     uint64_t tick = 0;
     uint64_t decode_epoch = 0;
     bool capturing = false;
+    bool step_tail = false;
+    int64_t tail_copies = 0;
+    cached_graph * follow = nullptr;
+    std::atomic<cached_graph *> parked{nullptr};
     bool ssm_fuse = true;
     bool mm_q5_major = false;
     tp_state * tp = nullptr;
@@ -220,6 +235,11 @@
 void free_graph_cache(backend_ctx * ctx);
 bool graph_key_equals(const ggml_cgraph * g, const std::vector<uint64_t> & key);
 void graph_key_build(const ggml_cgraph * g, std::vector<uint64_t> & key);
+void graph_key_set_inline(bool on);
+struct tail_copy { void * dst; const void * src; size_t size; };
+extern std::atomic<int> g_parked_count;
+bool graph_launch_parked(backend_ctx * ctx, const tail_copy * with_copy);
+void graph_note_download(cached_graph * followed, const tail_copy & cp);
 
 struct ip_engine;
 enum ggml_status ip_graph_compute(backend_ctx * ctx, ggml_cgraph * g, bool * handled);
diff --git a/llama_box_amd/csrc/graph.cpp b/llama_box_amd/csrc/graph.cpp
--- a/llama_box_amd/csrc/graph.cpp
+++ b/llama_box_amd/csrc/graph.cpp
@@ -2345,7 +2345,7 @@
     }
     return true;
 }
-static bool key_equals(const ggml_cgraph * g, const std::vector<uint64_t> & key) {
+static bool key_equals_memcmp(const ggml_cgraph * g, const std::vector<uint64_t> & key) {
     const uint64_t * at = key.data(), * const end = at + key.size();
     const bool same = walk_key(g, [&](const void * p, size_t n) {
         if ((size_t) (end - at) < n || memcmp(at, p, n * 8) != 0) return false;
@@ -2353,6 +2353,61 @@
         return true;
     });
     return same && at == end;
+}
+typedef uint64_t __attribute__((may_alias)) key_word;
+template <size_t N>
+static inline bool run_equals(const uint64_t * at, const void * field) {
+    typedef uint64_t word2 __attribute__((vector_size(16)));
+    const key_word * p = (const key_word *) field;
+    word2 d0 = {0, 0}, d1 = {0, 0};
+    size_t i = 0;
+    for (; i + 4 <= N; i += 4) {
+        word2 a0, b0, a1, b1;
+        __builtin_memcpy(&a0, at + i, 16); __builtin_memcpy(&b0, p + i, 16);
+        __builtin_memcpy(&a1, at + i + 2, 16); __builtin_memcpy(&b1, p + i + 2, 16);
+        d0 |= a0 ^ b0;
+        d1 |= a1 ^ b1;
+    }
+    d0 |= d1;
+    uint64_t d = d0[0] | d0[1];
+    for (; i < N; ++i) d |= at[i] ^ p[i];
+    return d == 0;
+}
+static inline void key_prefetch(const ggml_tensor * t, bool with_src) {
+    const char * p = (const char *) t;
+    __builtin_prefetch(p);
+    __builtin_prefetch(p + 64);
+    __builtin_prefetch(p + 128);
+    if (with_src) __builtin_prefetch(p + offsetof(ggml_tensor, src));
+    __builtin_prefetch(p + offsetof(ggml_tensor, data));
+}
+static std::atomic<bool> g_key_inline{env_flag("GGML_MI355X_KEY_INLINE", true)};
+void graph_key_set_inline(bool on) { g_key_inline.store(on, std::memory_order_relaxed); }
+static bool key_equals(const ggml_cgraph * g, const std::vector<uint64_t> & key) {
+    if (!g_key_inline.load(std::memory_order_relaxed)) return key_equals_memcmp(g, key);
+    const uint64_t * at = key.data(), * const end = at + key.size();
+    if (at == end || at[0] != (uint64_t) (uint32_t) g->n_nodes) return false;
+    at += 1;
+    for (int i = 0; i < g->n_nodes; ++i) {
+        const ggml_tensor * n = g->nodes[i];
+        if (i + 2 < g->n_nodes) key_prefetch(g->nodes[i + 2], true);
+        if (i + 1 < g->n_nodes) {
+            const ggml_tensor * nx = g->nodes[i + 1];
+            for (int s = 0; s < 3; ++s) if (nx->src[s]) key_prefetch(nx->src[s], false);
+        }
+        uint32_t present = 0;
+        for (int s = 0; s < GGML_MAX_SRC; ++s) present |= n->src[s] ? 1u << s : 0u;
+        const bool hinted = n->op == GGML_OP_FLASH_ATTN_EXT || n->op == GGML_OP_SOFT_MAX;
+        const uint64_t w0 = (uint64_t) (uint32_t) n->type | (uint64_t) present << 32 | (uint64_t) (hinted ? fa_mask_hint(n) : 0) << 48;
+        if ((size_t) (end - at) < 2 + KEY_NODE_RUN || at[0] != w0 || at[1] != (uint64_t) (uintptr_t) n->data || !run_equals<KEY_NODE_RUN>(at + 2, &n->buffer)) return false;
+        at += 2 + KEY_NODE_RUN;
+        for (; present; present &= present - 1) {
+            const ggml_tensor * t = n->src[__builtin_ctz(present)];
+            if ((size_t) (end - at) < 2 + KEY_SRC_RUN || at[0] != (uint64_t) (uint32_t) t->type || at[1] != (uint64_t) (uintptr_t) t->data || !run_equals<KEY_SRC_RUN>(at + 2, &t->buffer)) return false;
+            at += 2 + KEY_SRC_RUN;
+        }
+    }
+    return at == end;
 }
 static void key_build(const ggml_cgraph * g, std::vector<uint64_t> & key) {
     key.clear();
@@ -2379,13 +2434,114 @@
     return fold(fold(fold(h[0], h[1]), h[2]), h[3] ^ key.size());
 }
 
+static void drop_tail(cached_graph & cg) {
+    if (cg.tail_exec) (void) hipGraphExecDestroy(cg.tail_exec);
+    if (cg.tail_graph) (void) hipGraphDestroy(cg.tail_graph);
+    cg.tail_exec = nullptr;
+    cg.tail_graph = nullptr;
+    cg.tail_node = nullptr;
+    cg.tail_dst = nullptr; cg.tail_src = nullptr; cg.tail_size = 0;
+    cg.want_dst = nullptr; cg.want_src = nullptr; cg.want_size = 0;
+}
+static bool key_holds_range(const std::vector<uint64_t> & key, const void * src, size_t size) {
+    if (key.empty()) return false;
+    const uintptr_t p = (uintptr_t) src;
+    size_t at = 1;
+    for (uint64_t i = 0; i < key[0]; ++i) {
+        if (at + 2 + KEY_NODE_RUN > key.size()) return false;
+        const uint64_t w0 = key[at], data = key[at + 1];
+        const uint64_t * ne = &key[at + 2 + 1], * nb = ne + 4;
+        uint64_t extent = 0;
+        for (int d = 0; d < 4; ++d) extent = std::max(extent, ne[d] * nb[d]);
+        if (data != 0 && p >= data && p + size <= data + extent) return true;
+        at += 2 + KEY_NODE_RUN + (size_t) __builtin_popcountll((w0 >> 32) & 0xffff) * (2 + KEY_SRC_RUN);
+    }
+    return false;
+}
+static bool build_tail(cached_graph & cg, const tail_copy & cp) {
+    drop_tail(cg);
+    hipGraph_t g2 = nullptr;
+    if (cg.graph == nullptr || hipGraphClone(&g2, cg.graph) != hipSuccess || g2 == nullptr) { (void) hipGetLastError(); return false; }
+    size_t n_nodes = 0, n_edges = 0;
+    std::vector<hipGraphNode_t> nodes, from, to, leaves;
+    bool ok = hipGraphGetNodes(g2, nullptr, &n_nodes) == hipSuccess && n_nodes > 0;
+    if (ok) { nodes.resize(n_nodes); ok = hipGraphGetNodes(g2, nodes.data(), &n_nodes) == hipSuccess; }
+    if (ok) ok = hipGraphGetEdges(g2, nullptr, nullptr, &n_edges) == hipSuccess;
+    if (ok && n_edges > 0) { from.resize(n_edges); to.resize(n_edges); ok = hipGraphGetEdges(g2, from.data(), to.data(), &n_edges) == hipSuccess; }
+    if (ok) {
+        std::unordered_map<hipGraphNode_t, int> has_reader;
+        for (size_t e = 0; e < n_edges; ++e) has_reader[from[e]] = 1;
+        for (size_t k = 0; k < n_nodes; ++k) if (!has_reader.count(nodes[k])) leaves.push_back(nodes[k]);
+        ok = !leaves.empty();
+    }
+    upload_small_node nd;
+    upload_small_node_params(nd, cp.dst, cp.src, cp.size);
+    hipGraphNode_t tail = nullptr;
+    hipGraphExec_t exec = nullptr;
+    ok = ok && hipGraphAddKernelNode(&tail, g2, leaves.data(), leaves.size(), &nd.p) == hipSuccess && tail != nullptr;
+    ok = ok && hipGraphInstantiate(&exec, g2, nullptr, nullptr, 0) == hipSuccess && exec != nullptr;
+    if (!ok) {
+        (void) hipGetLastError();
+        if (exec) (void) hipGraphExecDestroy(exec);
+        (void) hipGraphDestroy(g2);
+        return false;
+    }
+    cg.tail_graph = g2; cg.tail_exec = exec; cg.tail_node = tail;
+    cg.tail_dst = cp.dst; cg.tail_src = cp.src; cg.tail_size = cp.size;
+    return true;
+}
+static hipGraphExec_t tail_exec_for(cached_graph & cg, const tail_copy & cp) {
+    if (cg.tail_failed) return nullptr;
+    if (cg.tail_exec && cg.tail_size == cp.size && cg.tail_src == cp.src) {
+        if (cg.tail_dst == cp.dst) return cg.tail_exec;
+        upload_small_node nd;
+        upload_small_node_params(nd, cp.dst, cp.src, cp.size);
+        if (hipGraphExecKernelNodeSetParams(cg.tail_exec, cg.tail_node, &nd.p) != hipSuccess) {
+            (void) hipGetLastError();
+            drop_tail(cg);
+            cg.tail_failed = true;
+            return nullptr;
+        }
+        cg.tail_dst = cp.dst; cg.tail_src = cp.src;
+        return cg.tail_exec;
+    }
+    const bool again = cg.want_dst == cp.dst && cg.want_src == cp.src && cg.want_size == cp.size;
+    graph_note_download(&cg, cp);
+    if (!again || !key_holds_range(cg.key, cp.src, cp.size)) return nullptr;
+    if (!build_tail(cg, cp)) { cg.tail_failed = true; return nullptr; }
+    return cg.tail_exec;
+}
+void graph_note_download(cached_graph * cg, const tail_copy & cp) {
+    if (cg == nullptr) return;
+    cg->want_dst = cp.dst; cg->want_src = cp.src; cg->want_size = cp.size;
+}
+bool graph_launch_parked(backend_ctx * c, const tail_copy * with_copy) {
+    cached_graph * cg = c->parked.exchange(nullptr, std::memory_order_acq_rel);
+    if (cg == nullptr) return false;
+    g_parked_count.fetch_sub(1, std::memory_order_release);
+    hipGraphExec_t tail = with_copy ? tail_exec_for(*cg, *with_copy) : nullptr;
+    const auto t0 = std::chrono::steady_clock::now();
+    HIP_SOFT(hipGraphLaunch(tail ? tail : cg->exec, c->stream));
+    c->st.graph_launch_host_ns += std::chrono::duration_cast<std::chrono::nanoseconds>(std::chrono::steady_clock::now() - t0).count();
+    c->st.graph_launches++;
+    c->st.allreduces += cg->allreduces;
+    if (tail) c->tail_copies++;
+    return tail != nullptr;
+}
+
 void free_graph_cache(backend_ctx * c) {
+    if (c->parked.load(std::memory_order_acquire)) {
+        graph_launch_parked(c, nullptr);
+        (void) hipStreamSynchronize(c->stream);
+    }
     for (auto & kv : c->graphs) {
+        drop_tail(kv.second);
         if (kv.second.exec) (void) hipGraphExecDestroy(kv.second.exec);
         if (kv.second.graph) (void) hipGraphDestroy(kv.second.graph);
     }
     c->graphs.clear();
     c->last_graph = nullptr;
+    c->follow = nullptr;
 }
 
 enum ggml_status graph_compute(backend_ctx * c, ggml_cgraph * g) {
@@ -2431,7 +2587,18 @@
     const bool may_replay = c->opt.graphs && !c->opt.timing && g->n_nodes >= 8;
     if (may_replay && c->last_graph && c->last_graph->exec && key_equals(g, c->last_graph->key)) {
         c->st.graph_key_fast_hits++;
-        return replay(*c->last_graph);
+        cached_graph & cg = *c->last_graph;
+        if (c->step_tail && cg.tail_ok) {
+            cg.last_use = c->tick;
+            cg.seen++;
+            c->st.graph_key_host_ns += std::chrono::duration_cast<std::chrono::nanoseconds>(std::chrono::steady_clock::now() - t_enter).count();
+            c->st.fa_form = cg.fa_form;
+            c->follow = &cg;
+            c->parked.store(&cg, std::memory_order_release);
+            g_parked_count.fetch_add(1, std::memory_order_release);
+            return GGML_STATUS_SUCCESS;
+        }
+        return replay(cg);
     }
     {
         bool handled = false;
@@ -2461,9 +2628,11 @@
         if (c->graphs.size() > 64) {
             for (auto jt = c->graphs.begin(); jt != c->graphs.end();) {
                 if (jt->second.last_use + 256 < c->tick) {
+                    drop_tail(jt->second);
                     if (jt->second.exec) (void) hipGraphExecDestroy(jt->second.exec);
                     if (jt->second.graph) (void) hipGraphDestroy(jt->second.graph);
                     if (c->last_graph == &jt->second) c->last_graph = nullptr;
+                    if (c->follow == &jt->second) c->follow = nullptr;
                     jt = c->graphs.erase(jt);
                     c->st.graph_evictions++;
                 } else {
@@ -2482,6 +2651,7 @@
     cached_graph * const prev = early ? c->last_graph : nullptr;
     cg.n_nodes = g->n_nodes;
     c->last_graph = &cg;
+    c->follow = &cg;
     if (cg.exec) return replay(cg);
     cg.last_use = c->tick;
     cg.seen++;
@@ -2550,6 +2720,7 @@
             (void) hipGraphExecDestroy(prev->exec);
             c->st.graph_exec_update_failures++;
         }
+        drop_tail(*prev);
         prev->exec = nullptr;
         if (prev->graph) (void) hipGraphDestroy(prev->graph);
         prev->graph = nullptr;
@@ -2564,9 +2735,11 @@
         return run_nodes(c, g, wp) ? GGML_STATUS_SUCCESS : GGML_STATUS_FAILED;
     }
     c->st.graph_exec_update_ns += now_ns() - t_mark;
+    drop_tail(cg);
     cg.graph = graph;
     cg.exec = exec;
     cg.allreduces = red_captured;
+    cg.tail_ok = !has_split && !tp_active(c) && red_captured == 0;
     c->st.graph_captures++;
     c->st.graph_early_captures += early ? 1 : 0;
     if (shadow) {
diff --git a/llama_box_amd/csrc/kernels.h b/llama_box_amd/csrc/kernels.h
--- a/llama_box_amd/csrc/kernels.h
+++ b/llama_box_amd/csrc/kernels.h
@@ -225,6 +225,8 @@
 void launch_clamp(hipStream_t s, const tdesc & src, const tdesc & dst, float lo, float hi);
 void launch_upload_multi(hipStream_t s, const upload_batch & b);
 void launch_upload_small(hipStream_t s, void * dst, const void * pinned_src, size_t n);
+struct upload_small_node { hipKernelNodeParams p; char * dst; const char * src; size_t n; int vec; void * args[4]; };
+void upload_small_node_params(upload_small_node & nd, void * dst, const void * src, size_t n);
 void launch_copy2d(hipStream_t s, void * dst, size_t dpitch, const void * src, size_t spitch, size_t width, size_t height);
 void launch_rebase_row_index(hipStream_t s, int64_t * dst, const int64_t * src, int64_t n_tok, int64_t full, int64_t ext, int64_t o0, int64_t n_ctx);
 struct reduce_parts { const float * part[GGML_MI355X_MAX_DEVICES]; int n; };
diff --git a/llama_box_amd/csrc/ops.hip b/llama_box_amd/csrc/ops.hip
--- a/llama_box_amd/csrc/ops.hip
+++ b/llama_box_amd/csrc/ops.hip
@@ -990,11 +990,29 @@
         if (i < n) dst[i] = src[i];
     }
 }
+static inline int upload_small_vec(const void * dst, const void * src, size_t n) {
+    const uintptr_t al = (uintptr_t) dst | (uintptr_t) src | (uintptr_t) n;
+    return (al & 15) == 0 ? 16 : ((al & 3) == 0 ? 4 : 1);
+}
 void launch_upload_small(hipStream_t s, void * dst, const void * pinned_src, size_t n) {
-    const uintptr_t al = (uintptr_t) dst | (uintptr_t) pinned_src | (uintptr_t) n;
-    const int vec = (al & 15) == 0 ? 16 : ((al & 3) == 0 ? 4 : 1);
+    const int vec = upload_small_vec(dst, pinned_src, n);
     const size_t items = (n + vec - 1) / vec;
     hipLaunchKernelGGL(k_upload_small, dim3((unsigned) ((items + 255) / 256)), dim3(256), 0, s, (char *) dst, (const char *) pinned_src, n, vec);
+}
+void upload_small_node_params(upload_small_node & nd, void * dst, const void * src, size_t n) {
+    nd.dst = (char *) dst;
+    nd.src = (const char *) src;
+    nd.n = n;
+    nd.vec = upload_small_vec(dst, src, n);
+    const size_t items = (n + nd.vec - 1) / nd.vec;
+    nd.args[0] = &nd.dst; nd.args[1] = &nd.src; nd.args[2] = &nd.n; nd.args[3] = &nd.vec;
+    nd.p = hipKernelNodeParams{};
+    nd.p.func = (void *) k_upload_small;
+    nd.p.gridDim = dim3((unsigned) ((items + 255) / 256));
+    nd.p.blockDim = dim3(256);
+    nd.p.sharedMemBytes = 0;
+    nd.p.kernelParams = nd.args;
+    nd.p.extra = nullptr;
 }
 
 __global__ void __launch_bounds__(256) k_upload_multi(const upload_batch b) {
diff --git a/llama_box_amd/csrc/tp_inproc.cpp b/llama_box_amd/csrc/tp_inproc.cpp
--- a/llama_box_amd/csrc/tp_inproc.cpp
+++ b/llama_box_amd/csrc/tp_inproc.cpp
@@ -984,6 +984,8 @@
         std::unique_lock<std::mutex> lk(E->turn_m);
         E->turn_cv.wait(lk, [&] { return E->turn == my; });
     }
+    const bool tail_was = w->step_tail;
+    w->step_tail = false;
     const enum ggml_status st = graph_compute(w, &P->graph[d]);
     if (dbg_order && E->threaded) {
         std::lock_guard<std::mutex> lk(E->turn_m);
@@ -991,6 +993,7 @@
         E->turn_cv.notify_all();
     }
     w->opt.graphs = graphs_was;
+    w->step_tail = tail_was;
     return st;
 }
 static void worker_main(ip_engine * E, int d) {
```
